# jeong0982/gkr

Hardware: AMD Instinct MI355X
Metric: BN254-Fr sumcheck field-ops/sec @ 2^20 vars (higher is better)
Workload: dtype u32x8

## Files before the change

### gkr_amd/_native.py

```python

import ctypes
import os

_HERE = os.path.dirname(os.path.abspath(__file__))
LIB_PATH = os.environ.get("GKR_AMD_LIB") or os.path.join(_HERE, "lib", "libgkr_amd.so")

GKR_OK = 0
GKR_ERR_INVALID = 1
GKR_ERR_NON_CANONICAL = 2
GKR_ERR_NO_DEVICE = 3
GKR_ERR_HIP = 4
GKR_ERR_NOMEM = 5
GKR_ERR_DEGENERATE = 6
GKR_ERR_UNSUPPORTED = 7

GKR_VERIFY_OK, GKR_VERIFY_SHAPE, GKR_VERIFY_NON_CANONICAL = 0, 1, 2
GKR_VERIFY_ROUND_SUM, GKR_VERIFY_CHALLENGE, GKR_VERIFY_EVALUATION = 4, 5, 10

GKR_TRANSCRIPT_DEVICE = 0
GKR_TRANSCRIPT_HOST = 1

SYMBOLS = [
    "gkr_strerror", "gkr_version", "gkr_ctx_create", "gkr_ctx_create_multi", "gkr_ctx_device_count", "gkr_ctx_destroy", "gkr_last_error",
    "gkr_ctx_set_transcript", "gkr_ctx_set_host_threads", "gkr_ctx_set_option", "gkr_ctx_get_option", "gkr_option_count", "gkr_option_name", "gkr_option_doc", "gkr_option_env", "gkr_host_help_while", "gkr_host_accounting", "gkr_host_accounting_read", "gkr_prove_many", "gkr_ctx_device_name", "gkr_ctx_profile", "gkr_ctx_profile_get", "gkr_ctx_profile_samples",
    "gkr_ctx_profile_reset", "gkr_mimc7_multi_hash", "gkr_mimc7_hash", "gkr_mimc7_constant",
    "gkr_selftest_mul", "gkr_selftest_wide_sum", "gkr_selftest_fold", "gkr_selftest_dot", "gkr_selftest_hash8", "gkr_selftest_host_pass", "gkr_selftest_host_prod_pass", "gkr_selftest_host_tail", "gkr_selftest_pass_schedule", "gkr_selftest_line_restriction", "gkr_selftest_seg_item", "gkr_devtest_field", "gkr_devtest_lazy", "gkr_devtest_reduce", "gkr_devtest_lanes", "gkr_sumcheck_mle", "gkr_sumcheck_mle_batch_device",
    "gkr_mle_eval_batch_device", "gkr_sumcheck_mle_verify_batch_device", "gkr_sumcheck_mle_verify",
    "gkr_sumcheck_layer", "gkr_sumcheck_layer_sharded", "gkr_sumcheck_layer_device", "gkr_resident_layer_create", "gkr_resident_layer_sumcheck", "gkr_resident_layer_sumcheck_wdev", "gkr_resident_layer_free", "gkr_exchange_limbs", "gkr_resident_layer_sumcheck_dev", "gkr_exchange_limbs_mle", "gkr_sumcheck_mle_sharded_dev", "gkr_exchange_rccl_unique_id", "gkr_exchange_rccl_create", "gkr_exchange_rccl_dev",
    "gkr_exchange_rccl_calls", "gkr_exchange_rccl_destroy", "gkr_exchange_rccl_error", "gkr_fr_widen", "gkr_fr_narrow", "gkr_predicate_tables", "gkr_layer_eval", "gkr_proof_sizes", "gkr_prove", "gkr_prove_batch",
    "gkr_layer_from_wires", "gkr_values_from_terms", "gkr_terms_from_coeffs", "gkr_prove_wires", "gkr_verify",
    "gkr_verify_prepare", "gkr_verify_prepared", "gkr_verify_circuit_free", "gkr_verify_device", "gkr_mimc7_multi_hash_device",
    "gkr_circom_meta", "gkr_circom_input_json", "gkr_circom_verifier_source", "gkr_circom_inject",
    "gkr_r1cs_parse", "gkr_r1cs_build", "gkr_r1cs_info", "gkr_r1cs_export", "gkr_r1cs_serialize", "gkr_r1cs_free",
    "gkr_wtns_parse", "gkr_wtns_serialize", "gkr_r1cs_compile", "gkr_layered_count", "gkr_layered_circuit",
    "gkr_layered_input_layer", "gkr_layered_input_values", "gkr_layered_free",
    "gkr_device_alloc", "gkr_device_free", "gkr_device_upload", "gkr_device_download",
    "gkr_device_fill_table", "gkr_device_fill_shard", "gkr_device_synchronize", "gkr_ubench_ceilings", "gkr_ubench_host_hash",
    "gkr_layer_session_open", "gkr_layer_session_open_tables", "gkr_layer_session_dep", "gkr_layer_session_rounds",
    "gkr_layer_session_sums", "gkr_layer_session_bind", "gkr_layer_session_tail", "gkr_layer_session_close",
    "gkr_mle_session_open", "gkr_mle_session_sums", "gkr_mle_session_bind", "gkr_mle_session_value",
    "gkr_mle_session_close", "gkr_device_tables_differ",
]


class CircuitDesc(ctypes.Structure):
    _fields_ = [
        ("depth", ctypes.c_uint32),
        ("k", ctypes.POINTER(ctypes.c_uint32)),
        ("gate_type", ctypes.POINTER(ctypes.c_void_p)),
        ("left", ctypes.POINTER(ctypes.c_void_p)),
        ("right", ctypes.POINTER(ctypes.c_void_p)),
    ]


class ProofBuf(ctypes.Structure):
    _fields_ = [(n, ctypes.c_void_p) for n in
                ("sumcheck_coeffs", "sumcheck_len", "sumcheck_r", "q", "q_len", "z", "r", "d_coeffs", "input_coeffs")]


class ProveItem(ctypes.Structure):
    _fields_ = [("circuit", ctypes.c_void_p), ("input_values", ctypes.c_void_p), ("batch", ctypes.c_int),
                ("require_zero_output", ctypes.c_int), ("outs", ctypes.c_void_p), ("status", ctypes.c_int)]


ALLREDUCE_DEV_FN = ctypes.CFUNCTYPE(ctypes.c_int, ctypes.c_void_p, ctypes.c_size_t, ctypes.c_void_p)


class ExchangeDev(ctypes.Structure):
    _fields_ = [("fn", ALLREDUCE_DEV_FN), ("user", ctypes.c_void_p), ("d_limbs", ctypes.c_void_p), ("capacity", ctypes.c_size_t)]


class R1csInfo(ctypes.Structure):
    _fields_ = [("n_wires", ctypes.c_uint32), ("n_pub_out", ctypes.c_uint32), ("n_pub_in", ctypes.c_uint32),
                ("n_prv_in", ctypes.c_uint32), ("n_labels", ctypes.c_uint64), ("n_constraints", ctypes.c_size_t),
                ("n_terms", ctypes.c_size_t)]


class ProofSizes(ctypes.Structure):
    _fields_ = [(n, ctypes.c_size_t) for n in ("rounds", "q_slots", "z_values", "d_coeffs", "input_coeffs")]


_lib = None


def lib():
    global _lib
    if _lib is None:
        if not os.path.exists(LIB_PATH):
            raise ImportError(
                "gkr_amd: %s is missing -- build it with `make -C gkr_amd/csrc` "
                "(or __graft_entry__.build()); there is no fallback path" % LIB_PATH)
        L = ctypes.CDLL(LIB_PATH)
        L.gkr_strerror.restype = ctypes.c_char_p
        L.gkr_version.restype = ctypes.c_char_p
        L.gkr_last_error.restype = ctypes.c_char_p
        L.gkr_last_error.argtypes = [ctypes.c_void_p]
        L.gkr_resident_layer_free.restype = None
        L.gkr_resident_layer_free.argtypes = [ctypes.c_void_p, ctypes.c_void_p]
        L.gkr_exchange_limbs.restype = ctypes.c_size_t
        L.gkr_exchange_limbs.argtypes = [ctypes.c_int]
        L.gkr_host_help_while.restype = ctypes.c_long
        L.gkr_host_help_while.argtypes = [ctypes.c_void_p]
        L.gkr_host_accounting.restype = ctypes.c_int
        L.gkr_host_accounting.argtypes = [ctypes.c_int]
        L.gkr_host_accounting_read.restype = ctypes.c_int
        L.gkr_host_accounting_read.argtypes = [ctypes.POINTER(ctypes.c_double), ctypes.c_size_t]
        L.gkr_ctx_destroy.restype = None
        L.gkr_ctx_destroy.argtypes = [ctypes.c_void_p]
        for fn in (L.gkr_layer_session_close, L.gkr_mle_session_close, L.gkr_verify_circuit_free):
            fn.restype = None
            fn.argtypes = [ctypes.c_void_p, ctypes.c_void_p]
        for fn in (L.gkr_r1cs_free, L.gkr_layered_free):
            fn.restype = None
            fn.argtypes = [ctypes.c_void_p]
        _lib = L
    return _lib
```

### gkr_amd/csrc/capi_internal.h

```cpp
#pragma once
#include <hip/hip_runtime.h>
#include <sched.h>
#include <stdio.h>
#include <stdlib.h>
#include <string.h>

#include <algorithm>
#include <chrono>
#include <condition_variable>
#include <map>
#include <memory>
#include <mutex>
#include <string>
#include <thread>
#include <vector>

#include "../../include/gkr_amd.h"
#include "fr64.h"
#include "host_cpus.h"
#include "hostpool.h"
#include "kernels.h"
#include "options.h"
#include "gate_seg.h"
#include "keccak.h"
// ... 426 lines not shown
    std::atomic<uint64_t> pieces{0}, piece_ns{0}, piece_pass_ns{0}, lanes[17] = {};
    std::atomic<bool> on{false};
};
inline HostAccountTotals& host_account_totals() {
    static HostAccountTotals t;
    return t;
}
inline bool accounting_on() { return host_account_totals().on.load(std::memory_order_relaxed); }
inline void account_piece(int transcripts, double pass_us, double total_us) {
    HostAccountTotals& t = host_account_totals();
    t.pieces.fetch_add(1, std::memory_order_relaxed);
    t.piece_ns.fetch_add((uint64_t)(total_us * 1e3), std::memory_order_relaxed);
    t.piece_pass_ns.fetch_add((uint64_t)(pass_us * 1e3), std::memory_order_relaxed);
    t.lanes[transcripts < 1 ? 1 : (transcripts > 16 ? 16 : transcripts)].fetch_add(1, std::memory_order_relaxed);
}
inline double now_us_dbg() { return std::chrono::duration<double, std::micro>(std::chrono::steady_clock::now().time_since_epoch()).count(); }

inline bool help_enabled() {
    static const bool on = !gkr::process_switch("GKR_NO_HELP");
    return on;
}
static void run_pieces(gkr::SpinPool* pool, const std::function<bool()>* work, bool several, int priority = 0) {
    auto run = [&] {
        if (pool)
            pool->run_now(work);
        else
            while ((*work)()) {
            }
    };
    const bool dbg = gkr::debug_timing() || accounting_on();
    const double t0 = dbg ? now_us_dbg() : 0.0;
    if (several && help_enabled()) {
        gkr::HelpBoard::Posted posted(work, priority);
        run();
    } else {
        run();
    }
    if (dbg) t_account.own_pieces_us += now_us_dbg() - t0;
}

template <typename Rec>
inline int wait_records(gkr_ctx* ctx, const volatile Rec* recs, int count, uint32_t ticket) {
    const auto t0 = std::chrono::steady_clock::now();
    const bool help = help_enabled();
    auto last_progress = t0;
    for (int b = 0; b < count; ++b) {
        uint32_t spins = 0, helped = 0;
        while (__atomic_load_n(&recs[b].seq, __ATOMIC_ACQUIRE) != ticket) {
            const bool dbg = gkr::debug_timing() || accounting_on();
            const double th0 = dbg ? now_us_dbg() : 0.0;
            const bool did_help = help && gkr::HelpBoard::instance().help();
            if (!did_help) GKR_CPU_RELAX();
            if (dbg) (did_help ? t_account.helped_us : t_account.spin_us) += now_us_dbg() - th0;
            if (did_help ? (++helped & 0x3F) == 0 : (++spins & 0xFFFF) == 0) {
                hipError_t q = hipStreamQuery(ctx->stream);
                if (q != hipSuccess && q != hipErrorNotReady) return ctx->hip_fail(q, "stream failed while waiting for a round");
                if (std::chrono::steady_clock::now() - last_progress > std::chrono::seconds(30)) {
                    if (q == hipSuccess && __atomic_load_n(&recs[b].seq, __ATOMIC_ACQUIRE) == ticket) break;
                    return ctx->fail(GKR_ERR_HIP, "timed out waiting for the device to publish a round");
                }
            }
        }
        if (spins | helped) last_progress = std::chrono::steady_clock::now();
    }
    return GKR_OK;
}

constexpr int kMaxGroups = 32;
constexpr int kMleShardTailLog2 = 6;

#define WS(ctx, slot, type, count, ptr) \
    HIP_TRY(ctx, (ctx)->workspace(slot, (size_t)(count) * sizeof(type), reinterpret_cast<void**>(&(ptr))))

inline int mle_pass_rounds(int m, int n, int jmax) {
    int j = m < jmax ? m : jmax;
    if (((size_t)1 << m) > gkr::kSmallPassEntries && m != n && j > m - 6) j = m - 6;
    if (jmax > 3 && (m - j == 10 || m - j == 11) && m - 12 >= 1) j = m - 12;
    return j < 1 ? 1 : j;
}

inline void write_round_output(gkr_fr* out_coeffs, uint32_t* out_len, gkr_fr* out_r, size_t row, const void* c0, const void* c1, uint32_t ln,
                               const void* r) {
    memset(&out_coeffs[row * 2], 0, 32);
    if (ln == 2) memcpy(&out_coeffs[row * 2], c1, 32);
    memcpy(&out_coeffs[row * 2 + 1], c0, 32);
    out_len[row] = ln;
    memcpy(&out_r[row], r, 32);
}
struct GroupHandoff {
    int b0 = 0, nb = 0;
    int state = 0;
    uint32_t ticket = 0;
    std::atomic<uint64_t> claim{0};
    std::atomic<int> done{0};
    template <typename Rec>
    bool records_landed(const Rec* rec) const {
        for (int i = nb - 1; i >= 0; --i)
            if (__atomic_load_n(&rec[b0 + i].seq, __ATOMIC_ACQUIRE) != ticket) return false;
        return true;
    }
    void open(uint32_t generation) {
        done.store(0, std::memory_order_relaxed);
        claim.store((uint64_t)generation << 32, std::memory_order_release);
        state = 1;
    }
    uint32_t open_generation() const {
        const uint64_t c = claim.load(std::memory_order_acquire);
        return (uint32_t)c < (uint32_t)nb ? (uint32_t)(c >> 32) : 0u;
    }
    bool try_claim(uint32_t chunk, uint32_t* first, uint32_t* take, uint32_t* generation = nullptr) {
        uint64_t c = claim.load(std::memory_order_acquire);
        while ((c >> 32) != 0 && (uint32_t)c < (uint32_t)nb) {
            const uint32_t left = (uint32_t)nb - (uint32_t)c, t = left < chunk ? left : chunk;
            if (!claim.compare_exchange_weak(c, c + t, std::memory_order_acq_rel)) continue;
            *first = (uint32_t)c;
            *take = t;
            if (generation) *generation = (uint32_t)(c >> 32);
            return true;
        }
        return false;
    }
    void finish(uint32_t count) { done.fetch_add((int)count, std::memory_order_release); }
    bool all_done() {
        if (done.load(std::memory_order_acquire) != nb) return false;
        claim.store(0, std::memory_order_release);
        return true;
    }
};
struct HandoffWatch {
    gkr_ctx* ctx;
    hipStream_t s;
    std::string unit;
    std::chrono::steady_clock::time_point t0 = std::chrono::steady_clock::now();
    uint32_t idle = 0;
    int progressed() {
        idle = 0;
        t0 = std::chrono::steady_clock::now();
        if (hipError_t le = hipGetLastError(); le != hipSuccess) return ctx->hip_fail(le, ("launch of a sumcheck " + unit).c_str());
        return GKR_OK;
    }
    int idled() {
        GKR_CPU_RELAX();
        if ((++idle & 0xFFFF) != 0) return GKR_OK;
        const hipError_t q = hipStreamQuery(s);
        if (q != hipSuccess && q != hipErrorNotReady) return ctx->hip_fail(q, ("stream failed during a sumcheck " + unit).c_str());
        if (std::chrono::steady_clock::now() - t0 > std::chrono::seconds(60))
            return ctx->fail(GKR_ERR_HIP, "timed out waiting for the device to publish a " + unit);
        return GKR_OK;
    }
};

void host_pass_scalar(const uint64_t* sums, size_t sums_row_words, int count, int J, const uint32_t* final_len, uint64_t (*c0)[16][4],
                      uint64_t (*c1)[16][4], uint64_t (*r)[16][4], uint32_t (*len)[16], uint64_t* weights, size_t w_row_words);
struct MleTailArgs {
    int n_total = 0, round_offset = 0;
    const uint32_t* dep_last = nullptr;
};
int run_mle_batch_passes(gkr_ctx* ctx, const Fr* d_tables, int n, int batch, gkr_fr* out_coeffs, uint32_t* out_len, gkr_fr* out_r,
                         const MleTailArgs* tail = nullptr);
int run_mle_batch(gkr_ctx* ctx, const Fr* d_tables, int n, int batch, gkr_fr* out_coeffs, uint32_t* out_len, gkr_fr* out_r);
void host_tail_pass(gkr::h64::F* tables, size_t stride, uint32_t m, uint32_t jp, const gkr::h64::F* weights, uint32_t J, gkr::h64::F* rec);
void host_tail_pass_scalar(gkr::h64::F* tables, size_t stride, uint32_t m, uint32_t jp, const gkr::h64::F* weights, uint32_t J, gkr::h64::F* rec);
void host_prod_pass_scalar(const uint64_t* recs, size_t rec_row_words, int count, int J, const uint32_t (*vec_len)[16], uint64_t (*c2)[16][4],
                           uint64_t (*lin)[16][4], uint64_t (*c0)[16][4], uint64_t (*r)[16][4], uint64_t* weights, size_t w_row_words);
struct LayerShardArgs {
    uint64_t gate_base = 0, gate_count = 0;
    gkr_allreduce_fn allreduce = nullptr;
    void* user = nullptr;
    const gkr_exchange_dev* dev = nullptr;
};
struct LayerGroup {
    const gkr::GateSet* d_sets = nullptr;
    gkr::GatePlanCounts plan_counts{};
};
int run_layer_batch(gkr_ctx* ctx, int batch, int k_i, int k, const uint8_t* d_gt, const uint32_t* d_l, const uint32_t* d_r, const gkr_fr* z,
                    const Fr* d_W, gkr_fr* const* out_coeffs, uint32_t* const* out_len, gkr_fr* const* out_r, const LayerShardArgs* shard = nullptr,
                    GateLists* cached = nullptr, const LayerGroup* group = nullptr);
int build_cached_gate_lists(gkr_ctx* ctx, int k_i, int k, const uint8_t* d_gt, const uint32_t* d_l, const uint32_t* d_r, GateLists* cached);
int check_layer_args(gkr_ctx* ctx, int k_i, int k_next, const uint8_t* gt, const uint32_t* l, const uint32_t* r, const gkr_fr* z);
int upload_gates(gkr_ctx* ctx, size_t gates, const uint8_t* gt, const uint32_t* l, const uint32_t* r, DevBuf<uint8_t>& dgt, DevBuf<uint32_t>& dl,
                 DevBuf<uint32_t>& dr);
int run_layer_dense(gkr_ctx* ctx, int batch, int k_i, int k, const uint8_t* d_gt, const uint32_t* d_l, const uint32_t* d_r, const gkr_fr* z,
                    const Fr* d_W, gkr_fr* const* out_coeffs, uint32_t* const* out_len, gkr_fr* const* out_r);
bool verify_device_hash_wanted(size_t rows);
int verify_hash_rows_device(gkr_ctx* ctx, const uint32_t* d_rows, const uint32_t* d_len, size_t n, gkr::VerifyHashSlot* d_slots, hipStream_t s);
void mobius_msb(std::vector<gkr::h64::F>& c, int k);
void line_restriction(const std::vector<gkr::h64::F>& vals, const std::vector<gkr::h64::F>& coeffs, int k, const gkr_fr* b, const gkr_fr* c,
                      gkr_fr* out, uint32_t* out_len);
int check_circuit(gkr_ctx* ctx, const gkr_circuit_desc* c);

}
```

### gkr_amd/csrc/capi_mle_passes.hip

```cpp
#include "capi_internal.h"

namespace gkr_host {

void host_pass_scalar(const uint64_t* sums, size_t sums_row_words, int count, int J, const uint32_t* final_len,
                             uint64_t (*c0)[16][4], uint64_t (*c1)[16][4], uint64_t (*r)[16][4], uint32_t (*len)[16],
                             uint64_t* weights, size_t w_row_words) {
    using gkr::h64::F;
    const F* cts = host_mimc_constants64();
    const F one_m = gkr::h64::to_mont(F{{1, 0, 0, 0}});
    for (int k = 0; k < count; ++k) {
        F S[gkr::kMleMaxSub], rm[gkr::kMlePassMaxRounds];
        memcpy(S, sums + (size_t)k * sums_row_words, sizeof(F) << J);
        for (int t = 0; t < J; ++t) {
            const int half = 1 << (J - t - 1);
            F lo = S[0], hi = S[half];
            for (int b = 1; b < half; ++b) {
                lo = gkr::h64::add(lo, S[b]);
                hi = gkr::h64::add(hi, S[half + b]);
            }
            const F d = gkr::h64::sub(hi, lo);
            const uint32_t ln = (final_len && t == J - 1) ? final_len[k] : (gkr::h64::is_zero(d) ? 1u : 2u);
            const F vec[2] = {d, lo};
            const F rc = host_multi_hash(vec + (2 - ln), (int)ln, cts);
            memcpy(c0[t][k], &lo, 32);
            memcpy(c1[t][k], &d, 32);
            memcpy(r[t][k], &rc, 32);
            len[t][k] = ln;
            rm[t] = gkr::h64::to_mont(rc);
            for (int b = 0; b < half; ++b) S[b] = gkr::h64::add(S[b], gkr::h64::mont_mul(gkr::h64::sub(S[half + b], S[b]), rm[t]));
        }
        if (!weights) continue;
        F* w = reinterpret_cast<F*>(weights + (size_t)k * w_row_words);
        F tmp[gkr::kMleMaxSub];
        tmp[0] = one_m;
        int cur = 1;
        for (int t = 0; t < J; ++t) {
            const F nr = gkr::h64::sub(one_m, rm[t]);
            for (int b = cur; b-- > 0;) {
                tmp[2 * b + 1] = gkr::h64::mont_mul(tmp[b], rm[t]);
                tmp[2 * b] = gkr::h64::mont_mul(tmp[b], nr);
            }
            cur <<= 1;
        }
        memcpy(w, tmp, sizeof(F) << J);
    }
}

struct MlePassTables {
    const Fr* input = nullptr;
    size_t in_stride = 0;
    Fr* work = nullptr;
    size_t work_len = 0;
    gkr::MleSubPartial* partials = nullptr;
    unsigned char* plans = nullptr;
    Fr* h_w = nullptr;
    gkr::MleHostRecSub* h_rec = nullptr;
    gkr::MleHostRecSub* rec = nullptr;
    uint32_t* arrivals = nullptr;
    Fr* h_tail = nullptr;
};
static int mle_pass_tables(gkr_ctx* ctx, const std::string& prefix, const Fr* input, size_t len, size_t work_len, int batch, MlePassTables& T) {
    T.input = input;
    T.in_stride = len;
    T.work_len = work_len;
    WS(ctx, (prefix + ".work").c_str(), Fr, (size_t)batch * (work_len ? work_len : 1), T.work);
    WS(ctx, (prefix + ".partials").c_str(), gkr::MleSubPartial, (size_t)batch * gkr::kMaxBlocksPerTable, T.partials);
    WS(ctx, (prefix + ".plans").c_str(), unsigned char, (size_t)batch * gkr::mle_fold_plan_bytes(), T.plans);
    HIP_TRY(ctx, ctx->pinned_host((prefix + ".rec").c_str(), sizeof(gkr::MleHostRecSub) * batch, reinterpret_cast<void**>(&T.h_rec)));
    HIP_TRY(ctx, ctx->pinned_host((prefix + ".w").c_str(), sizeof(Fr) * gkr::kMleMaxSub * batch, reinterpret_cast<void**>(&T.h_w)));
    T.rec = T.h_rec;
    return GKR_OK;
}

constexpr double kFusedPublishBytes = 64.0 * 1024 * 1024;
constexpr uint32_t kFusedPublishBlocks = 256;
constexpr size_t kArrivalCounters = 4096;
static int mle_arrival_counters(gkr_ctx* ctx, size_t len, MlePassTables& T) {
    if (gkr::opt(gkr::OPT_no_fused_reduce) != 0 || (double)len * 32.0 > kFusedPublishBytes) return GKR_OK;
    WS(ctx, "mlep.arrivals", uint32_t, kArrivalCounters, T.arrivals);
    if (ctx->mle_arrivals_zeroed != T.arrivals) {
        HIP_TRY(ctx, hipMemsetAsync(T.arrivals, 0, sizeof(uint32_t) * kArrivalCounters, ctx->stream));
        ctx->mle_arrivals_zeroed = T.arrivals;
    }
    return GKR_OK;
}
static bool fused_publish(const MlePassTables& T, int b0, int nb, uint32_t nblk, double bytes_read, uint32_t ticket, int jout, gkr::MlePublish& pub) {
    if (!T.arrivals || (size_t)(b0 + nb) > kArrivalCounters || bytes_read > kFusedPublishBytes || (uint64_t)nblk * nb > kFusedPublishBlocks || nblk > 128u)
        return false;
    pub.rec = T.rec + b0;
    pub.arrivals = T.arrivals + b0;
    pub.ticket = ticket;
    pub.jout = (uint32_t)jout;
    return true;
}

constexpr uint32_t kMleTailLog2 = 7;
struct MlePassPolicy {
    const char* row = nullptr;
    int plan_event = -1;
    Fr* export_tail = nullptr;
};
static void queue_sub_reduce(gkr_ctx* ctx, const MlePassTables& T, int b0, int nb, uint32_t nblk, int jout, uint32_t ticket, hipStream_t st) {
    Timed t(ctx, "mle_sub_reduce", 0.0, st, true);
    gkr::launch_mle_sub_reduce(T.partials + (size_t)b0 * gkr::kMaxBlocksPerTable, nblk, (uint32_t)jout, nb, T.rec + b0, ticket, st);
}
static void queue_pass0(gkr_ctx* ctx, const MlePassTables& T, int b0, int nb, int jout, uint32_t ticket, hipStream_t st, const MlePassPolicy& P) {
    const size_t len = T.in_stride;
    const Fr* src = T.input + (size_t)b0 * len;
    const double bytes = (double)nb * len * 32.0;
    if (len <= gkr::kSmallPassEntries) {
        Timed t(ctx, "mle_pass_small", bytes, st, true);
        gkr::launch_mle_multifold_small(0, src, len, nullptr, 0, (uint32_t)len, (uint32_t)jout, nb, T.h_w + (size_t)b0 * gkr::kMleMaxSub, T.rec + b0, ticket, st);
        return;
    }
    const uint32_t nblk = gkr::mle_pass_blocks((uint32_t)len, (uint32_t)jout, nb);
    gkr::MlePublish pub;
    const bool fused = fused_publish(T, b0, nb, nblk, bytes, ticket, jout, pub);
    {
        Timed t(ctx, P.row, bytes, st, fused);
        gkr::launch_mle_sub_sums(src, len, (uint32_t)len, nb, nblk, T.partials + (size_t)b0 * gkr::kMaxBlocksPerTable, st, fused ? &pub : nullptr);
    }
    if (!fused) queue_sub_reduce(ctx, T, b0, nb, nblk, jout, ticket, st);
}
static void queue_fold(gkr_ctx* ctx, const MlePassTables& T, int b0, int nb, bool from_input, int m_src, int jin, int jout, uint32_t ticket,
                       hipStream_t st, const MlePassPolicy& P) {
    const size_t src_len = (size_t)1 << m_src, S = src_len >> jin;
    const Fr* src = from_input ? T.input + (size_t)b0 * T.in_stride : T.work + (size_t)b0 * T.work_len;
    const size_t src_stride = from_input ? T.in_stride : T.work_len;
    Fr* dst = T.work + (size_t)b0 * T.work_len;
    const Fr* w = T.h_w + (size_t)b0 * gkr::kMleMaxSub;
    const double bytes = (double)nb * ((double)src_len + (double)S) * 32.0;
    if (S <= gkr::kSmallPassEntries) {
        Timed t(ctx, "mle_pass_small", bytes, st, true);
        gkr::launch_mle_multifold_small(jin, src, src_stride, dst, T.work_len, (uint32_t)S, (uint32_t)jout, nb, w, T.rec + b0, ticket, st, P.export_tail,
                                        1u << kMleTailLog2);
        return;
    }
    const uint32_t nblk = gkr::mle_multifold_blocks((uint32_t)S, (uint32_t)jout, nb);
    unsigned char* plan = T.plans + (size_t)b0 * gkr::mle_fold_plan_bytes();
    if (gkr::mle_multifold_uses_mfma((uint32_t)S, nblk)) {
        if (P.plan_event < 0) {
            gkr::launch_mle_fold_plan(jin, w, plan, nb, st);
        } else {
            {
                Timed t(ctx, "mle_fold_plan", 0.0, ctx->aux, true);
                gkr::launch_mle_fold_plan(jin, w, plan, nb, ctx->aux);
            }
            (void)hipEventRecord(ctx->aux_events[P.plan_event], ctx->aux);
            (void)hipStreamWaitEvent(st, ctx->aux_events[P.plan_event], 0);
        }
    }
    gkr::MlePublish pub;
    const bool fused = fused_publish(T, b0, nb, nblk, (double)nb * (double)src_len * 32.0, ticket, jout, pub);
    {
        Timed t(ctx, P.row, bytes, st, fused);
        gkr::launch_mle_multifold(jin, src, src_stride, dst, T.work_len, (uint32_t)S, nb, nblk, w, plan, T.partials + (size_t)b0 * gkr::kMaxBlocksPerTable, st,
                                  fused ? &pub : nullptr);
    }
    if (!fused) queue_sub_reduce(ctx, T, b0, nb, nblk, jout, ticket, st);
}

struct MleSchedule {
    int jmax = 0, j_first = 0;
    int n_dev = 0;
    int groups = 0, depth = 0;
    int bound[kMaxGroups + 1];
    uint32_t chunk[kMaxGroups];
    bool tail_on = false;
};
static MleSchedule mle_schedule(int n, int batch, int hash_threads, bool is_tail, const gkr::Options& o) {
    MleSchedule sc;
    const double len = (double)((size_t)1 << n);
    const int jcap = o.v[gkr::OPT_no_mfma_fold] ? 3 : gkr::kMlePassMaxRounds;
    const int jwant = o.v[gkr::OPT_rounds_per_pass] > 0 ? (int)o.v[gkr::OPT_rounds_per_pass] : jcap;
    sc.jmax = jwant > jcap ? jcap : jwant;
    sc.j_first = mle_pass_rounds(n, n, sc.jmax);
    const long long dp = o.v[gkr::OPT_device_hash_percent];
    const int dev_percent = dp < 0 ? 0 : (dp > 90 ? 90 : (int)dp);
    if (dev_percent > 0 && !is_tail && batch >= 64 && sc.j_first >= 1) {
        sc.n_dev = (int)((long long)batch * dev_percent / 100) & ~7;
        if (batch - sc.n_dev < 16) sc.n_dev = (batch - 16) & ~7;
        if (sc.n_dev < 8) sc.n_dev = 0;
    }
    const int host_batch = batch - sc.n_dev;
    const double batch_bytes = (double)host_batch * len * 32.0;
    int want_groups = (int)(batch_bytes / (4.0 * 1024 * 1024 * 1024));
    want_groups = want_groups < 4 ? 4 : (want_groups > 8 ? (batch_bytes > 96.0 * 1024 * 1024 * 1024 ? 16 : 8) : want_groups);
    const bool small_tables = n <= 17 && host_batch >= 256;
    if (small_tables) want_groups = 16;
    if (hash_threads <= 3 && host_batch >= 256 && want_groups < 16) want_groups = 16;
    int group_size = host_batch >= 128 ? (host_batch + want_groups - 1) / want_groups : (host_batch >= 16 ? (host_batch + 1) / 2 : host_batch);
    if (sc.n_dev && hash_threads <= 3 && host_batch >= 256) group_size = 64;
    if (o.v[gkr::OPT_group_size] > 0) group_size = (int)o.v[gkr::OPT_group_size];
    sc.groups = (host_batch + group_size - 1) / group_size;
    if (sc.groups > kMaxGroups) sc.groups = kMaxGroups;
    const long long forced = o.v[gkr::OPT_hash_chunk];
    for (int g = 0; g <= sc.groups; ++g) sc.bound[g] = sc.n_dev + (int)((long long)host_batch * g / sc.groups);
    for (int g = 0; g < sc.groups; ++g) {
        const int nb = sc.bound[g + 1] - sc.bound[g], per = (nb + hash_threads - 1) / hash_threads;
        sc.chunk[g] = forced == 8 || forced == 16 ? (uint32_t)forced : (nb >= 32 * hash_threads ? 16u : (uint32_t)(per <= 8 ? 8 : (per <= 16 ? per : 16)));
    }
    sc.depth = o.v[gkr::OPT_pass_queue_depth] > 0 ? (int)o.v[gkr::OPT_pass_queue_depth] : (small_tables ? 4 : 2);
    sc.tail_on = o.v[gkr::OPT_host_tail_log2] >= 0 && sc.n_dev == 0 && batch <= (o.v[gkr::OPT_host_tail_max_batch] > 0 ? o.v[gkr::OPT_host_tail_max_batch] : 8);
    return sc;
}

namespace {
struct PassGroup : GroupHandoff {
    int m = 0;
    int j = 0;
    int round0 = 0;
    int pass = 0, index = 0;
    hipStream_t chain = nullptr;
    bool on_host = false;
};
struct MlePassClock {
    const bool on = gkr::debug_timing();
    const std::chrono::steady_clock::time_point t0 = std::chrono::steady_clock::now();
    double a = 0, b = 0, c = 0, d = 0, e = 0;
    std::atomic<uint64_t> busy_ns{0};
    double us() const { return std::chrono::duration<double, std::micro>(std::chrono::steady_clock::now() - t0).count(); }
    void report(int threads) const {
        if (!on) return;
        fprintf(stderr,
                "[gkr timing] setup %.0f us, first launches %.0f, loop %.0f, end_session %.0f, sync %.0f, drain %.0f; hashing %.0f us "
                "over %d threads = %.0f%% of the loop\n",
                a, b - a, c - b, d - c, e - d, us() - e, busy_ns.load() * 1e-3, threads, busy_ns.load() * 1e-3 / ((c - b) * threads) * 100.0);
    }
};

struct MlePassRun {
    gkr_ctx* ctx;
    const int n, batch;
    const MleTailArgs* tail;
    gkr_fr* out_coeffs;
    uint32_t* out_len;
    gkr_fr* out_r;
    MleSchedule sc;
    MlePassTables T;
    hipStream_t s = nullptr, late = nullptr, chain = nullptr;
    std::vector<PassGroup> grp;
    std::vector<uint32_t> dep_last;
    int next_first = 0;
    gkr_fr *stage_c = nullptr, *stage_r = nullptr;
    uint32_t* stage_len = nullptr;
    MlePassClock clock;

    int rounds_for(int m) const { return mle_pass_rounds(m, n, sc.jmax); }
    void advance(PassGroup& G, int jin) {
        G.m -= jin;
        G.round0 += jin;
        G.j = rounds_for(G.m);
        G.ticket = ++ctx->ticket;
    }
    void launch_first(PassGroup& G) {
        G.ticket = ++ctx->ticket;
        MlePassPolicy P;
        P.row = G.chain ? "mle_sub_sums_dev" : "mle_sub_sums";
        queue_pass0(ctx, T, G.b0, G.nb, G.j, G.ticket, G.chain ? G.chain : s, P);
    }
    void launch_next_first() {
        if (next_first < sc.groups) launch_first(grp[next_first++]);
    }
    void launch_fold(PassGroup& G, int jin) {
        const int m_src = G.m;
        const bool from_input = m_src == n;
        hipStream_t st = G.chain ? G.chain : ((!from_input && m_src <= 16) ? late : s);
        advance(G, jin);
        MlePassPolicy P;
        P.row = G.chain ? "mle_multifold_dev" : (st == s ? "mle_multifold" : "mle_multifold_late");
        if (!gkr::opt(gkr::OPT_plan_main) && st == s && sc.groups != 1) P.plan_event = G.index;
        G.on_host = sc.tail_on && !G.chain && G.m <= (int)kMleTailLog2 && G.m - G.j > 0;
        if (G.on_host) P.export_tail = T.h_tail + ((size_t)G.b0 << kMleTailLog2);
        queue_fold(ctx, T, G.b0, G.nb, from_input, m_src, jin, G.j, G.ticket, st, P);
    }
    void host_fold(PassGroup& G, int jin) {
        using gkr::h64::F;
        advance(G, jin);
        const size_t S = (size_t)1 << G.m, nsub = (size_t)1 << G.j, sub = S >> G.j;
        for (int b = G.b0; b < G.b0 + G.nb; ++b) {
            F* tab = reinterpret_cast<F*>(T.h_tail + ((size_t)b << kMleTailLog2));
            const F* w = reinterpret_cast<const F*>(T.h_w + (size_t)b * gkr::kMleMaxSub);
            for (size_t i = 0; i < S; ++i) {
                gkr::h64::Wide acc = gkr::h64::wide_zero();
                for (size_t t = 0; t < ((size_t)1 << jin); ++t) gkr::h64::wide_mac(acc, tab[t * S + i], w[t]);
                tab[i] = gkr::h64::wide_reduce(acc);
            }
            F* sums = reinterpret_cast<F*>(T.h_rec[b].sums);
            for (size_t a = 0; a < nsub; ++a) {
                F v = tab[a * sub];
                for (size_t i = 1; i < sub; ++i) v = gkr::h64::add(v, tab[a * sub + i]);
                sums[a] = v;
            }
            __atomic_store_n(&T.h_rec[b].seq, G.ticket, __ATOMIC_RELEASE);
        }
    }
    void process_chunk(const PassGroup& G, int b_first, int count) {
        static const bool scalar_book = gkr::process_switch("GKR_HOST_PASS_SCALAR");
        const int J = G.j, n_out = tail ? tail->n_total : n, r_off = tail ? tail->round_offset : 0;
        uint64_t c0[gkr::kMlePassMaxRounds][16][4], c1[gkr::kMlePassMaxRounds][16][4], r[gkr::kMlePassMaxRounds][16][4];
        uint32_t ln[gkr::kMlePassMaxRounds][16], final_len[16];
        const bool final_pass = G.round0 + J == n;
        for (int i = 0; i < count; ++i) {
            if (G.round0 == 0) dep_last[b_first + i] = tail && tail->dep_last ? tail->dep_last[b_first + i] : T.h_rec[b_first + i].dep;
            final_len[i] = dep_last[b_first + i] ? 2u : 1u;
        }
        static_assert(sizeof(gkr::MleHostRecSub) % 8 == 0, "hand-off records are addressed in 64-bit words");
        const uint64_t* sums = reinterpret_cast<const uint64_t*>(T.h_rec[b_first].sums);
        uint64_t* weights = G.m - J > 0 ? reinterpret_cast<uint64_t*>(T.h_w + (size_t)b_first * gkr::kMleMaxSub) : nullptr;
        (host_ifma_ready() && count >= 3 && !scalar_book ? gkr::gkr_ifma_pass : host_pass_scalar)(
            sums, sizeof(gkr::MleHostRecSub) / 8, count, J, final_pass ? final_len : nullptr, c0, c1, r, ln, weights, 4 * gkr::kMleMaxSub);
        for (int i = 0; i < count; ++i)
            for (int t = 0; t < J; ++t)
                write_round_output(out_coeffs, out_len, out_r, (size_t)(b_first + i) * n_out + r_off + G.round0 + t, c0[t][i], c1[t][i], ln[t][i], r[t][i]);
    }
    bool try_work() {
        for (;;) {
            int best = -1;
            uint32_t best_gen = 0;
            for (int g = 0; g < sc.groups; ++g)
                if (const uint32_t gen = grp[g].open_generation(); gen && (best < 0 || gen < best_gen)) best = g, best_gen = gen;
            if (best < 0) return false;
            PassGroup& G = grp[best];
            uint32_t first, take;
            if (!G.try_claim(sc.chunk[best], &first, &take)) continue;
            const double t_in = clock.on ? clock.us() : 0.0;
            process_chunk(G, G.b0 + (int)first, (int)take);
            G.finish(take);
            if (clock.on) clock.busy_ns.fetch_add((uint64_t)((clock.us() - t_in) * 1e3), std::memory_order_relaxed);
            return true;
        }
    }
    int queue_device_chain() {
        const int n_dev = sc.n_dev;
        HIP_TRY(ctx, ctx->chain_stream(&chain));
        uint32_t* dep_dev = nullptr;
        WS(ctx, "mlep.dev_dep", uint32_t, (size_t)n_dev, dep_dev);
        HIP_TRY(ctx, ctx->pinned_host("mlep.stage_c", sizeof(gkr_fr) * 2 * (size_t)n_dev * n, reinterpret_cast<void**>(&stage_c)));
        HIP_TRY(ctx, ctx->pinned_host("mlep.stage_r", sizeof(gkr_fr) * (size_t)n_dev * n, reinterpret_cast<void**>(&stage_r)));
        HIP_TRY(ctx, ctx->pinned_host("mlep.stage_len", sizeof(uint32_t) * (size_t)n_dev * n, reinterpret_cast<void**>(&stage_len)));
        PassGroup dev;
        dev.nb = n_dev;
        dev.m = n;
        dev.j = sc.j_first;
        dev.index = sc.groups;
        dev.chain = chain;
        launch_first(dev);
        for (bool first = true;; first = false) {
            const int J = dev.j;
            {
                Timed t(ctx, "mle_pass_hash_dev", 0.0, chain);
                gkr::launch_mle_pass_hash_lanes(T.rec, (uint32_t)n_dev, (uint32_t)J, (uint32_t)dev.round0, (uint32_t)n, dev.round0 + J == n, first, ctx->d_cts,
                                                dep_dev, dev.m - J > 0 ? T.h_w : nullptr, reinterpret_cast<Fr*>(stage_c), stage_len,
                                                reinterpret_cast<Fr*>(stage_r), chain);
            }
            if (dev.m - J <= 0) return GKR_OK;
            launch_fold(dev, J);
        }
    }
    bool step(PassGroup& G, int& active) {
        if (G.state == 0 && G.records_landed(T.h_rec)) {
            G.open((uint32_t)++G.pass);
            return true;
        }
        if (G.state != 1 || !G.all_done()) return false;
        if (G.m - G.j > 0) {
            const bool first_fold = G.m == n;
            if (G.on_host)
                host_fold(G, G.j);
            else
                launch_fold(G, G.j);
            G.state = 0;
            if (first_fold) launch_next_first();
        } else {
            G.state = 2;
            --active;
            launch_next_first();
        }
        return true;
    }
    int loop() {
        int rc = GKR_OK, active = sc.groups;
        HandoffWatch watch{ctx, s, "pass"};
        while (active > 0 && rc == GKR_OK) {
            bool progress = false;
            for (int g = 0; g < next_first; ++g) progress |= step(grp[g], active);
            if (progress)
                rc = watch.progressed();
            else if (!try_work())
                rc = watch.idled();
        }
        return rc;
    }
};
}

int run_mle_batch_passes(gkr_ctx* ctx, const Fr* d_tables, int n, int batch, gkr_fr* out_coeffs, uint32_t* out_len, gkr_fr* out_r,
                         const MleTailArgs* tail) {
    MlePassRun R{ctx, n, batch, tail, out_coeffs, out_len, out_r};
    const size_t len = (size_t)1 << n;
    hipStream_t s = R.s = R.late = ctx->stream;
    gkr::SpinPool* pool = ctx->host_pool();
    const gkr::Options* o = gkr::current_options();
    const MleSchedule& sc = R.sc = mle_schedule(n, batch, pool->workers() + 1, tail != nullptr, o ? *o : gkr::default_options());
    if (int rc = mle_pass_tables(ctx, "mlep", d_tables, len, len >> sc.j_first, batch, R.T)) return rc;
    if (int rc = mle_arrival_counters(ctx, len, R.T)) return rc;
    HIP_TRY(ctx, ctx->aux_stream(sc.groups));
    if (sc.tail_on) HIP_TRY(ctx, ctx->pinned_host("mlep.tail", sizeof(Fr) * ((size_t)batch << kMleTailLog2), reinterpret_cast<void**>(&R.T.h_tail)));
    if (!gkr::opt(gkr::OPT_no_late_stream) && sc.groups > 1) HIP_TRY(ctx, ctx->late_stream(&R.late));
    R.dep_last = std::vector<uint32_t>(batch, 0);
    R.grp = std::vector<PassGroup>(sc.groups);
    for (int g = 0; g < sc.groups; ++g) {
        PassGroup& G = R.grp[g];
        G.index = g;
        G.b0 = sc.bound[g];
        G.nb = sc.bound[g + 1] - sc.bound[g];
        G.m = n;
        G.j = sc.j_first;
    }
    const std::function<bool()> try_work = [&R] { return R.try_work(); };
    R.clock.a = R.clock.us();
    gkr::SpinPool::Session session(pool, &try_work);
    R.launch_next_first();
    if (sc.n_dev)
        if (int rc = R.queue_device_chain()) return rc;
    while (R.next_first < sc.groups && R.next_first < sc.depth) R.launch_next_first();
    R.clock.b = R.clock.us();
    const int rc = R.loop();
    R.clock.c = R.clock.us();
    session.close();
    if (rc) {
        (void)hipStreamSynchronize(s);
        if (R.late != s) (void)hipStreamSynchronize(R.late);
        if (R.chain) (void)hipStreamSynchronize(R.chain);
        ctx->mle_arrivals_zeroed = nullptr;
        return rc;
    }
    R.clock.d = R.clock.us();
    HIP_TRY(ctx, hipGetLastError());
    HIP_TRY(ctx, hipStreamSynchronize(s));
    if (R.late != s) HIP_TRY(ctx, hipStreamSynchronize(R.late));
    if (sc.n_dev) {
        HIP_TRY(ctx, hipStreamSynchronize(R.chain));
        memcpy(out_coeffs, R.stage_c, sizeof(gkr_fr) * 2 * (size_t)sc.n_dev * n);
        memcpy(out_r, R.stage_r, sizeof(gkr_fr) * (size_t)sc.n_dev * n);
        memcpy(out_len, R.stage_len, sizeof(uint32_t) * (size_t)sc.n_dev * n);
    }
    R.clock.e = R.clock.us();
    if (ctx->pending.size() > 8192) ctx->drain_events();
    R.clock.report(pool->workers() + 1);
    return GKR_OK;
}

namespace {
struct MleShardRun {
    gkr_ctx* ctx;
    const gkr_exchange_dev* exchange;
    const int n, batch;
    gkr_fr* out_coeffs;
    uint32_t* out_len;
    gkr_fr* out_r;
    MlePassTables T;
    uint32_t* h_fail = nullptr;
    std::vector<uint32_t> dep_last;
    gkr::SpinPool* pool = nullptr;
    int rc = GKR_OK;
    uint32_t exchanges = 0;

    long long* limbs() const { return reinterpret_cast<long long*>(exchange->d_limbs); }
    void hook_failed(int arc) {
        if (arc && !rc) rc = ctx->fail(GKR_ERR_INVALID, "the device sum-over-ranks hook failed (status " + std::to_string(arc) + ")");
    }
    bool some_rank_failed() const { return __atomic_load_n(h_fail, __ATOMIC_ACQUIRE) != 0; }
    void exchange_sums(int J, uint32_t ticket) {
        hipStream_t s = ctx->stream;
        Timed t(ctx, "exchange", 0.0);
        gkr::launch_mle_xwiden(T.rec, (uint32_t)J, (uint32_t)batch, rc ? 1u : 0u, limbs(), s);
        const int arc = exchange->fn(exchange->user, (size_t)batch * (((size_t)1 << J) + 2) * 8, static_cast<void*>(s));
        gkr::launch_mle_xnarrow(limbs(), (uint32_t)J, (uint32_t)batch, T.h_rec, ticket, h_fail, s);
        ++exchanges;
        hook_failed(arc);
    }
    void gather_tail(const Fr* rest, size_t stride, int m, int lp, int shard, Fr* d_tail) {
        hipStream_t s = ctx->stream;
        Timed t(ctx, "exchange", 0.0);
        gkr::launch_mle_gather_widen(rest, stride, (uint32_t)m, (uint32_t)lp, (uint32_t)shard, rc ? 1u : 0u, (uint32_t)batch, limbs(), s);
        const int arc = exchange->fn(exchange->user, ((size_t)batch << (m + lp)) * 8 + 8, static_cast<void*>(s));
        gkr::launch_mle_gather_narrow(limbs(), (uint32_t)(m + lp), (uint32_t)batch, d_tail, h_fail, s);
        ++exchanges;
        hook_failed(arc);
    }
    void rounds_chunk(int first, int J, int round0) {
        const int count = batch - first < 16 ? batch - first : 16;
        uint64_t c0[gkr::kMlePassMaxRounds][16][4], c1[gkr::kMlePassMaxRounds][16][4], r[gkr::kMlePassMaxRounds][16][4];
        uint32_t ln[gkr::kMlePassMaxRounds][16];
        (host_ifma_ready() && count >= 3 ? gkr::gkr_ifma_pass : host_pass_scalar)(
            reinterpret_cast<const uint64_t*>(T.h_rec[first].sums), sizeof(gkr::MleHostRecSub) / 8, count, J, nullptr, c0, c1, r, ln,
            reinterpret_cast<uint64_t*>(T.h_w + (size_t)first * gkr::kMleMaxSub), 4 * gkr::kMleMaxSub);
        for (int i = 0; i < count; ++i) {
            if (round0 == 0) dep_last[first + i] = T.h_rec[first + i].dep;
            for (int t = 0; t < J; ++t)
                write_round_output(out_coeffs, out_len, out_r, (size_t)(first + i) * n + round0 + t, c0[t][i], c1[t][i], ln[t][i], r[t][i]);
        }
    }
    void host_rounds(int J, int round0) {
        std::atomic<int> next{0};
        const std::function<bool()> work_fn = [&]() -> bool {
            const int first = next.fetch_add(16, std::memory_order_relaxed);
            if (first < batch) rounds_chunk(first, J, round0);
            return first < batch;
        };
        gkr::SpinPool::Session session(pool, nullptr);
        run_pieces(pool, &work_fn, batch > 16);
    }
    void pass(bool pass0, bool from_input, int m_src, int jin, int J, int round0) {
        const uint32_t ticket = ++ctx->ticket;
        if (!rc) {
            MlePassPolicy P;
            P.row = pass0 ? "mle_sub_sums" : "mle_multifold";
            if (pass0)
                queue_pass0(ctx, T, 0, batch, J, ticket, ctx->stream, P);
            else
                queue_fold(ctx, T, 0, batch, from_input, m_src, jin, J, ticket, ctx->stream, P);
            if (hipError_t le = hipGetLastError(); le != hipSuccess) rc = ctx->hip_fail(le, "launch of a sumcheck pass");
        }
        exchange_sums(J, ticket);
        if (!rc) rc = wait_records(ctx, T.h_rec, batch, ticket);
        if (!rc && some_rank_failed()) rc = ctx->fail(GKR_ERR_HIP, "another rank failed during the sumcheck");
        if (!rc) host_rounds(J, round0);
    }
};
}

}

extern "C" {

size_t gkr_exchange_limbs_mle(int n, int log2_shards, int batch) {
    if (n < 2 || log2_shards < 0 || log2_shards > 16 || n - log2_shards < 1 || n - log2_shards > GKR_MAX_MLE_N || batch < 1) return 0;
    const int nl = n - log2_shards, t = nl < kMleShardTailLog2 ? nl : kMleShardTailLog2;
    const size_t per_pass = (size_t)batch * (gkr::kMleMaxSub + 2) * 8, gather = ((size_t)batch << (t + log2_shards)) * 8 + 8;
    return per_pass > gather ? per_pass : gather;
}

int gkr_sumcheck_mle_sharded_dev(gkr_ctx* ctx, const void* d_shards, int n, int log2_shards, int shard, int batch,
                                 const gkr_exchange_dev* exchange, gkr_fr* out_coeffs, uint32_t* out_len, gkr_fr* out_r,
                                 uint32_t* out_exchanges) {
    if (!ctx) return GKR_ERR_INVALID;
    if (!d_shards || !exchange || !exchange->fn || !exchange->d_limbs || !out_coeffs || !out_len || !out_r || batch < 1 || batch > 65535)
        return ctx->fail(GKR_ERR_INVALID, "null pointer or batch out of range [1, 65535]");
    const int lp = log2_shards, nl = n - lp;
    if (lp < 0 || lp > 16 || shard < 0 || shard >= (1 << lp)) return ctx->fail(GKR_ERR_INVALID, "shard must be in [0, 2^log2_shards), log2_shards in [0, 16]");
    if (n < 2 || nl < 1 || nl > GKR_MAX_MLE_N) return ctx->fail(GKR_ERR_INVALID, "n >= 2 and 1 <= n - log2_shards <= GKR_MAX_MLE_N needed");
    if (ctx->transcript != GKR_TRANSCRIPT_HOST) return ctx->fail(GKR_ERR_INVALID, "a sumcheck split over ranks needs the host transcript");
    if (exchange->capacity < gkr_exchange_limbs_mle(n, lp, batch)) return ctx->fail(GKR_ERR_INVALID, "the exchange buffer is smaller than gkr_exchange_limbs_mle(n, log2_shards, batch) int64");
    GKR_ENTER(ctx);
    hipStream_t s = ctx->stream;
    const size_t len = (size_t)1 << nl;
    const int t_stop = nl < kMleShardTailLog2 ? nl : kMleShardTailLog2;
    const int jmax = gkr::opt(gkr::OPT_no_mfma_fold) ? 3 : gkr::kMlePassMaxRounds;
// ... 50 lines not shown
```

### gkr_amd/csrc/gkr_capi.hip

```cpp
#include "capi_internal.h"


extern "C" {

const char* gkr_strerror(int status) {
    switch (status) {
        case GKR_OK: return "ok";
        case GKR_ERR_INVALID: return "invalid argument";
        case GKR_ERR_NON_CANONICAL: return "field element is not canonical (>= r)";
        case GKR_ERR_NO_DEVICE: return "no gfx950 device available";
        case GKR_ERR_HIP: return "HIP runtime error";
        case GKR_ERR_NOMEM: return "out of memory";
        case GKR_ERR_DEGENERATE: return "degenerate sumcheck (v == 0)";
        case GKR_ERR_UNSUPPORTED: return "R1CS shape the reference's compiler does not support";
        default: return "unknown status";
    }
}

const char* gkr_version(void) { return "gkr_amd 0.1 (gfx950)"; }

int gkr_ctx_create(int device_id, gkr_ctx** out) {
    if (!out) return GKR_ERR_INVALID;
    *out = nullptr;
    int count = 0;
// ... 196 lines not shown
int gkr_ctx_device_name(const gkr_ctx* ctx, char* buf, size_t len) {
    if (!ctx || !buf || !len) return GKR_ERR_INVALID;
    snprintf(buf, len, "%s", ctx->name);
    return GKR_OK;
}

int gkr_ctx_profile(gkr_ctx* ctx, int enable) {
    if (!ctx) return GKR_ERR_INVALID;
    ctx->profile = enable < 0 ? 0 : (enable > 2 ? 2 : enable);
    return GKR_OK;
}

int gkr_ctx_profile_get(gkr_ctx* ctx, const char* kernel, uint64_t* launches, double* total_ms, double* bytes) {
    if (!ctx || !kernel) return GKR_ERR_INVALID;
    ctx->drain_events();
    auto it = ctx->prof.find(kernel);
    ProfileRow r = it == ctx->prof.end() ? ProfileRow() : it->second;
    if (launches) *launches = r.launches;
    if (total_ms) *total_ms = r.total_ms;
    if (bytes) *bytes = r.bytes;
    return GKR_OK;
}

int gkr_ctx_profile_samples(gkr_ctx* ctx, const char* kernel, double* ms, double* bytes, size_t capacity, size_t* count) {
    if (!ctx || !kernel || !count) return GKR_ERR_INVALID;
    ctx->drain_events();
    auto it = ctx->prof.find(kernel);
    const size_t n = it == ctx->prof.end() ? 0 : it->second.samples.size();
    *count = n;
    for (size_t i = 0; i < n && i < capacity; ++i) {
        if (ms) ms[i] = it->second.samples[i].first;
        if (bytes) bytes[i] = it->second.samples[i].second;
    }
    return GKR_OK;
}

int gkr_ctx_profile_reset(gkr_ctx* ctx) {
    if (!ctx) return GKR_ERR_INVALID;
    ctx->drain_events();
    ctx->prof.clear();
    return GKR_OK;
}


int gkr_mimc7_multi_hash(const gkr_fr* arr, size_t n, const gkr_fr* key, gkr_fr* out) {
    if ((!arr && n) || !out) return GKR_ERR_INVALID;
    if (!all_canonical(arr, n) || (key && !all_canonical(key, 1))) return GKR_ERR_NON_CANONICAL;
    const Fr* cts = host_mimc_constants();
    Fr r = key ? gkr::to_mont(to_dev(*key)) : gkr::fr_zero();
    for (size_t i = 0; i < n; ++i) {
        Fr a = gkr::to_mont(to_dev(arr[i]));
        Fr h = gkr::mimc7_hash_mont(a, r, cts);
        r = gkr::fr_add(gkr::fr_add(r, a), h);
    }
    *out = to_abi(gkr::from_mont(r));
    return GKR_OK;
}

int gkr_mimc7_hash(const gkr_fr* x, const gkr_fr* k, gkr_fr* out) {
    if (!x || !k || !out) return GKR_ERR_INVALID;
    if (!all_canonical(x, 1) || !all_canonical(k, 1)) return GKR_ERR_NON_CANONICAL;
    Fr h = gkr::mimc7_hash_mont(gkr::to_mont(to_dev(*x)), gkr::to_mont(to_dev(*k)), host_mimc_constants());
    *out = to_abi(gkr::from_mont(h));
    return GKR_OK;
}

int gkr_mimc7_constant(int i, gkr_fr* out) {
    if (i < 0 || i >= gkr::kMimcRounds || !out) return GKR_ERR_INVALID;
    *out = to_abi(gkr::from_mont(host_mimc_constants()[i]));
    return GKR_OK;
}

int gkr_selftest_mul(const gkr_fr* a, const gkr_fr* b, gkr_fr* out) {
    if (!a || !b || !out) return GKR_ERR_INVALID;
    if (!all_canonical(a, 1) || !all_canonical(b, 1)) return GKR_ERR_NON_CANONICAL;
    *out = to_abi(gkr::fr_mul(to_dev(*a), to_dev(*b)));
    return GKR_OK;
}

int gkr_selftest_fold(const gkr_fr* lo, const gkr_fr* hi, const gkr_fr* r, gkr_fr* out) {
    if (!lo || !hi || !r || !out) return GKR_ERR_INVALID;
    if (!all_canonical(lo, 1) || !all_canonical(hi, 1) || !all_canonical(r, 1)) return GKR_ERR_NON_CANONICAL;
    const gkr::FixedMul T = gkr::make_fixed_mul(to_dev(*r));
    gkr::FixedMul T64;
    gkr::h64::F r64;
    memcpy(&r64, r, 32);
    gkr::h64::make_fixed_mul(r64, T64.w);
    if (memcmp(&T, &T64, sizeof T) != 0) return GKR_ERR_INVALID;
    const Fr single = gkr::fr_fold_fixed(to_dev(*lo), to_dev(*hi), T);
    Fr y0, y1;
    gkr::fr_fold_fixed2(to_dev(*lo), to_dev(*hi), to_dev(*hi), to_dev(*lo), T, y0, y1);
    if (!gkr::fr_eq(y0, single) || !gkr::fr_eq(y1, gkr::fr_fold_fixed(to_dev(*hi), to_dev(*lo), T))) return GKR_ERR_INVALID;
    *out = to_abi(single);
    return GKR_OK;
}

int gkr_selftest_pass_schedule(int n, int mfma, uint32_t* rounds, size_t capacity, size_t* passes) {
    if (n < 1 || n > 40 || !passes) return GKR_ERR_INVALID;
    const int jmax = mfma ? gkr::kMlePassMaxRounds : 3;
    size_t count = 0;
    for (int m = n; m > 0;) {
        const int j = mle_pass_rounds(m, n, jmax);
        if (rounds && count < capacity) rounds[count] = (uint32_t)j;
        ++count;
        m -= j;
    }
    *passes = count;
    return (rounds && count > capacity) ? GKR_ERR_NOMEM : GKR_OK;
}

int gkr_selftest_host_pass(const gkr_fr* sums, int count, int J, const uint32_t* final_len, gkr_fr* c0, gkr_fr* c1, uint32_t* len,
                           gkr_fr* r, gkr_fr* w, int* used_ifma) {
    using gkr::h64::F;
    if (!sums || !c0 || !c1 || !len || !r || !w || count < 1 || count > kHashChunkMax || J < 1 || J > gkr::kMlePassMaxRounds)
        return GKR_ERR_INVALID;
    static_assert(gkr::kMleMaxSub == 32 && kHashChunkMax == 16, "shapes of the self-test's arrays");
    if (!all_canonical(sums, (size_t)count * 32)) return GKR_ERR_NON_CANONICAL;
    if (final_len)
        for (int k = 0; k < count; ++k)
            if (final_len[k] != 1 && final_len[k] != 2) return GKR_ERR_INVALID;
    struct Out {
        uint64_t c0[gkr::kMlePassMaxRounds][16][4], c1[gkr::kMlePassMaxRounds][16][4], r[gkr::kMlePassMaxRounds][16][4];
        uint32_t len[gkr::kMlePassMaxRounds][16];
        std::vector<F> w;
    } a, b;
    a.w.assign((size_t)count * 32, F{{0, 0, 0, 0}});
    host_pass_scalar(reinterpret_cast<const uint64_t*>(sums), 4 * 32, count, J, final_len, a.c0, a.c1, a.r, a.len, &a.w[0].l[0], 4 * 32);
    const bool ifma = host_ifma_ready();
    if (used_ifma) *used_ifma = ifma ? 1 : 0;
    if (ifma) {
        b.w.assign((size_t)count * 32, F{{0, 0, 0, 0}});
        gkr::gkr_ifma_pass(reinterpret_cast<const uint64_t*>(sums), 4 * 32, count, J, final_len, b.c0, b.c1, b.r, b.len, &b.w[0].l[0], 4 * 32);
        for (int t = 0; t < J; ++t)
            for (int k = 0; k < count; ++k)
                if (memcmp(a.c0[t][k], b.c0[t][k], 32) || memcmp(a.c1[t][k], b.c1[t][k], 32) || memcmp(a.r[t][k], b.r[t][k], 32) ||
                    a.len[t][k] != b.len[t][k])
                    return GKR_ERR_INVALID;
        if (memcmp(a.w.data(), b.w.data(), sizeof(F) * a.w.size()) != 0) return GKR_ERR_INVALID;
    }
    for (int t = 0; t < J; ++t)
        for (int k = 0; k < count; ++k) {
            memcpy(&c0[(size_t)t * count + k], a.c0[t][k], 32);
            memcpy(&c1[(size_t)t * count + k], a.c1[t][k], 32);
            memcpy(&r[(size_t)t * count + k], a.r[t][k], 32);
            len[(size_t)t * count + k] = a.len[t][k];
        }
    for (size_t i = 0; i < a.w.size(); ++i) {
        const F wc = gkr::h64::from_mont(a.w[i]);
        memcpy(&w[i], &wc, 32);
    }
    return GKR_OK;
}

int gkr_selftest_host_prod_pass(const gkr_fr* recs, int count, int J, const uint32_t* vec_len, gkr_fr* c2, gkr_fr* lin, gkr_fr* c0,
                                gkr_fr* r, gkr_fr* w, int* used_ifma) {
    using gkr::h64::F;
    if (!recs || !vec_len || !c2 || !lin || !c0 || !r || !w || count < 1 || count > kHashChunkMax || J < 1 || J > gkr::kProdMaxJ)
        return GKR_ERR_INVALID;
    if (!all_canonical(recs, (size_t)count * gkr::kProdRecValues)) return GKR_ERR_NON_CANONICAL;
    uint32_t vl[gkr::kProdMaxJ][16] = {};
    for (int t = 0; t < J; ++t)
        for (int k = 0; k < count; ++k) {
            vl[t][k] = vec_len[(size_t)t * count + k];
            if (vl[t][k] != 2 && vl[t][k] != 3) return GKR_ERR_INVALID;
        }
    struct Out {
        uint64_t c2[gkr::kProdMaxJ][16][4], lin[gkr::kProdMaxJ][16][4], c0[gkr::kProdMaxJ][16][4], r[gkr::kProdMaxJ][16][4];
        F w[16][8];
    } a, b;
    memset(&a, 0, sizeof a);
    memset(&b, 0, sizeof b);
    host_prod_pass_scalar(reinterpret_cast<const uint64_t*>(recs), 4 * gkr::kProdRecValues, count, J, vl, a.c2, a.lin, a.c0, a.r, &a.w[0][0].l[0], 32);
    const bool ifma = host_ifma_ready();
    if (used_ifma) *used_ifma = ifma ? 1 : 0;
    if (ifma) {
        gkr::gkr_ifma_prod_pass(reinterpret_cast<const uint64_t*>(recs), 4 * gkr::kProdRecValues, count, J, vl, b.c2, b.lin, b.c0, b.r, &b.w[0][0].l[0], 32);
        for (int t = 0; t < J; ++t)
            for (int k = 0; k < count; ++k)
                if (memcmp(a.c2[t][k], b.c2[t][k], 32) || memcmp(a.lin[t][k], b.lin[t][k], 32) || memcmp(a.c0[t][k], b.c0[t][k], 32) ||
                    memcmp(a.r[t][k], b.r[t][k], 32))
                    return GKR_ERR_INVALID;
        for (int k = 0; k < count; ++k)
            if (memcmp(a.w[k], b.w[k], sizeof(F) << J) != 0) return GKR_ERR_INVALID;
    }
    for (int t = 0; t < J; ++t)
        for (int k = 0; k < count; ++k) {
            memcpy(&c2[(size_t)t * count + k], a.c2[t][k], 32);
            memcpy(&lin[(size_t)t * count + k], a.lin[t][k], 32);
            memcpy(&c0[(size_t)t * count + k], a.c0[t][k], 32);
            memcpy(&r[(size_t)t * count + k], a.r[t][k], 32);
        }
    for (int k = 0; k < count; ++k)
        for (int bb = 0; bb < 8; ++bb) {
            const F wc = bb < (1 << J) ? gkr::h64::from_mont(a.w[k][bb]) : F{{0, 0, 0, 0}};
            memcpy(&w[(size_t)k * 8 + bb], &wc, 32);
        }
    return GKR_OK;
}

int gkr_selftest_host_tail(const gkr_fr* tables, int m, int jp, const gkr_fr* weights, int J, gkr_fr* rec, int* used_ifma) {
    using gkr::h64::F;
    if (!tables || !rec || m < 0 || m > 12 || jp < 0 || jp > gkr::kProdMaxJ || jp > m || J < 1 || J > gkr::kProdMaxJ || J > m - jp || (jp && !weights))
        return GKR_ERR_INVALID;
    const size_t len = (size_t)1 << m;
    if (!all_canonical(tables, 3 * len) || (jp && !all_canonical(weights, (size_t)1 << jp))) return GKR_ERR_NON_CANONICAL;
    std::vector<F> t(3 * len);
    memcpy(t.data(), tables, sizeof(F) * 3 * len);
    for (size_t i = 0; i < len; ++i) t[i] = gkr::h64::to_mont(t[i]);
    F w[8] = {};
    for (int b = 0; jp && b < (1 << jp); ++b) {
        memcpy(&w[b], &weights[b], sizeof(F));
        w[b] = gkr::h64::to_mont(w[b]);
    }
    F out[gkr::kProdRecValues] = {};
    const bool ifma = host_ifma_ready();
    if (used_ifma) *used_ifma = ifma ? 1 : 0;
    if (ifma) {
        std::vector<F> t2(t);
        F out2[gkr::kProdRecValues] = {};
        gkr::gkr_ifma_tail_pass(&t2[0].l[0], len, (uint32_t)m, (uint32_t)jp, &w[0].l[0], (uint32_t)J, &out2[0].l[0]);
        host_tail_pass_scalar(t.data(), len, (uint32_t)m, (uint32_t)jp, w, (uint32_t)J, out);
        const size_t folded = (size_t)1 << (m - jp);
        for (int tb = 0; tb < 3; ++tb)
            if (memcmp(&t[(size_t)tb * len], &t2[(size_t)tb * len], folded * sizeof(F)) != 0) return GKR_ERR_INVALID;
        const int n = 1 << J;
        for (int a = 0; a < n; ++a) {
            if (memcmp(&out[a * 8], &out2[a * 8], sizeof(F) * n) != 0) return GKR_ERR_INVALID;
            if (memcmp(&out[64 + a], &out2[64 + a], sizeof(F)) != 0) return GKR_ERR_INVALID;
        }
    } else {
        host_tail_pass_scalar(t.data(), len, (uint32_t)m, (uint32_t)jp, w, (uint32_t)J, out);
    }
    memcpy(rec, out, sizeof out);
    return GKR_OK;
}

int gkr_selftest_hash8(const gkr_fr* vecs, const uint32_t* len, gkr_fr* out, int* used_ifma) {
    if (!vecs || !len || !out) return GKR_ERR_INVALID;
    if (!all_canonical(vecs, 24)) return GKR_ERR_NON_CANONICAL;
    for (int k = 0; k < 8; ++k)
        if (len[k] > 3) return GKR_ERR_INVALID;
    const bool ifma = host_ifma_ready();
    if (used_ifma) *used_ifma = ifma ? 1 : 0;
    if (ifma) {
        uint64_t v[8][3][4], o[8][4];
        memcpy(v, vecs, sizeof v);
        gkr::gkr_ifma_multi_hash8(v, len, 3, o);
        memcpy(out, o, sizeof o);
        uint64_t v16[16][3][4], o16[16][4];
        uint32_t len16[16];
        for (int k = 0; k < 8; ++k) {
            memcpy(v16[k], v[k], sizeof v[k]);
            memcpy(v16[15 - k], v[k], sizeof v[k]);
            len16[k] = len16[15 - k] = len[k];
        }
        gkr::gkr_ifma_multi_hash16(v16, len16, 3, o16);
        for (int k = 0; k < 8; ++k)
            if (memcmp(o16[k], o[k], 32) != 0 || memcmp(o16[15 - k], o[k], 32) != 0) return GKR_ERR_INVALID;
    } else {
        const gkr::h64::F* cts = host_mimc_constants64();
        for (int k = 0; k < 8; ++k) {
            gkr::h64::F v[3];
            memcpy(v, vecs + 3 * k, 96);
            const gkr::h64::F r = host_multi_hash(v + (3 - len[k]), (int)len[k], cts);
            memcpy(&out[k], &r, 32);
        }
    }
    return GKR_OK;
}

int gkr_ubench_host_hash(int len, double* us_per_hash_lanes16, double* us_per_hash_scalar) {
    if (len < 1 || len > 3 || !us_per_hash_lanes16 || !us_per_hash_scalar) return GKR_ERR_INVALID;
    uint64_t v16[16][3][4], o16[16][4];
    uint32_t len16[16];
    for (int k = 0; k < 16; ++k) {
        len16[k] = (uint32_t)len;
        for (int e = 0; e < 3; ++e)
            for (int j = 0; j < 4; ++j) v16[k][e][j] = j == 3 ? 0x0123456789abcdefull >> 4 : 0x9E3779B97F4A7C15ull * (uint64_t)(k * 12 + e * 4 + j + 1);
    }
    auto now = [] { return std::chrono::steady_clock::now(); };
    *us_per_hash_lanes16 = 0.0;
    if (host_ifma_ready()) {
        double best = 1e30;
        for (int rep = 0; rep < 5; ++rep) {
            const auto t0 = now();
            for (int i = 0; i < 64; ++i) {
                gkr::gkr_ifma_multi_hash16(v16, len16, 3, o16);
                memcpy(v16[i & 15][2], o16[(i + 1) & 15], 32);
            }
            const double us = std::chrono::duration<double, std::micro>(now() - t0).count() / (64.0 * 16.0);
            if (us < best) best = us;
        }
        *us_per_hash_lanes16 = best;
    }
    const gkr::h64::F* cts = host_mimc_constants64();
    gkr::h64::F v[3];
    memcpy(v, v16[0], 96);
    double best = 1e30;
    for (int rep = 0; rep < 5; ++rep) {
        const auto t0 = now();
        for (int i = 0; i < 32; ++i) v[2] = host_multi_hash(v + (3 - len), len, cts);
        const double us = std::chrono::duration<double, std::micro>(now() - t0).count() / 32.0;
        if (us < best) best = us;
    }
    *us_per_hash_scalar = best;
    return GKR_OK;
// ... 217 lines not shown
```

### gkr_amd/csrc/kernels.h

```cpp
#pragma once
#include <hip/hip_runtime.h>
#include <stddef.h>
#include <stdint.h>

#include "fr32.h"

namespace gkr {

constexpr uint32_t kMaxBlocksPerTable = 2048;
constexpr uint32_t kMaxLayerBlocks = 2048;

struct MlePartial {
    Acc<9> lo, hi;
    uint32_t dep, pad;
};

struct LayerBatch {
    uint32_t batch;
    uint32_t pstride;
    size_t tstride, wstride;
};
inline LayerBatch single_layer() { return LayerBatch{1u, 0u, 0, 0}; }

struct LayerPartial {
    Acc<9> c0, g1, c2;
    uint32_t pad;
};

struct MleHostRec {
    Fr c0, c1;
    uint32_t dep, seq;
    uint32_t pad[14];
};
struct LayerHostRec {
    Fr c0, g1, c2;
    uint32_t seq;
    uint32_t pad[7];
};
static_assert(sizeof(MleHostRec) == 128 && sizeof(LayerHostRec) == 128, "hand-off records are one 128-byte line");

constexpr int kProdMaxJ = 3;
constexpr int kProdRecValues = 72;
struct ProdPassRec {
    Fr v[kProdRecValues];
    uint32_t seq;
    uint32_t pad[7];
};
static_assert(sizeof(ProdPassRec) == kProdRecValues * 32 + 32, "product-pass record layout");
constexpr uint32_t kProdTile = 8, kProdTileWide = 32;
inline uint32_t prod_pass_tile(uint32_t S) { return S >= 1024u ? kProdTileWide : kProdTile; }
inline uint32_t prod_pass_blocks(uint32_t S) { return S <= kProdTile ? 1u : S / prod_pass_tile(S); }
inline uint32_t prod_pass_max_blocks(uint32_t k) {
    uint32_t m = 1;
    for (uint32_t l = 0; l < k; ++l) m = prod_pass_blocks(1u << l) > m ? prod_pass_blocks(1u << l) : m;
    return m;
}
inline size_t prod_pass_scratch_values(uint32_t k) { return ((size_t)prod_pass_max_blocks(k) + 64u) * kProdRecValues; }
constexpr uint32_t kProdFuseBlocks = 64;
constexpr uint32_t kProdFoldMinM = 17;
size_t prod_fold_plan_bytes();
void launch_prod_pass(Fr* W, Fr* X, Fr* Y, uint32_t m_in, uint32_t jp, const Fr* weights, uint32_t J, Fr* partials, uint32_t wstride,
                      ProdPassRec* rec, uint32_t ticket, uint32_t batch, hipStream_t s, uint32_t* arrivals = nullptr, void* fold_plans = nullptr,
                      Fr* tail = nullptr, uint32_t tail_stride = 0);
void launch_prod_c_setup(const Fr* Wb, uint32_t jp, const Fr* weights, const Fr* A, const Fr* M, Fr* X, Fr* Y, uint32_t k, uint32_t wstride,
                         uint32_t batch, hipStream_t s);

constexpr uint32_t kSmallFoldQuarter = 2048;
void launch_mle_fold_sum_small(const Fr* src, size_t src_stride, Fr* dst, size_t dst_stride, uint32_t q, uint32_t batch,
                               const FixedMul* rtab, MleHostRec* host_rec, uint32_t ticket, hipStream_t s);
void launch_mle_round_reduce(const MlePartial* partials, uint32_t nblk, uint32_t batch, MleHostRec* host_rec,
                             uint32_t ticket, hipStream_t s);

struct MleSubPartial {
    Acc<9> sum;
    uint32_t dep, pad[2];
};
constexpr int kMlePassMaxRounds = 5;
constexpr int kMleMaxSub = 1 << kMlePassMaxRounds;
struct MleHostRecSub {
    Fr sums[kMleMaxSub];
    uint32_t dep, seq;
    uint32_t pad[14];
};
static_assert(sizeof(MleHostRecSub) == 1088, "hand-off record layout");
struct MlePublish {
    MleHostRecSub* rec = nullptr;
    uint32_t* arrivals = nullptr;
    uint32_t ticket = 0, jout = 0;
};
constexpr uint32_t kSmallPassEntries = 512;
uint32_t mle_pass_blocks(uint32_t items, uint32_t jout, uint32_t batch);
uint32_t mle_multifold_blocks(uint32_t S, uint32_t jout, uint32_t batch);
bool mle_multifold_uses_mfma(uint32_t S, uint32_t nblk);
void launch_mle_sub_sums(const Fr* tables, size_t stride, uint32_t len, uint32_t batch, uint32_t nblk, MleSubPartial* partials,
                         hipStream_t s, const MlePublish* publish = nullptr);
void launch_mle_sub_reduce(const MleSubPartial* partials, uint32_t nblk, uint32_t jout, uint32_t batch, MleHostRecSub* host_rec,
                           uint32_t ticket, hipStream_t s);
size_t mle_fold_plan_bytes();
void launch_mle_fold_plan(int jin, const Fr* weights, void* plans, uint32_t batch, hipStream_t s);
void launch_mle_multifold(int jin, const Fr* src, size_t src_stride, Fr* dst, size_t dst_stride, uint32_t S, uint32_t batch,
                          uint32_t nblk, const Fr* weights, const void* plans, MleSubPartial* partials, hipStream_t s,
                          const MlePublish* publish = nullptr);
void launch_mle_pass_hash_lanes(const MleHostRecSub* rec, uint32_t count, uint32_t J, uint32_t round0, uint32_t n_out, bool final_pass,
                                bool first_pass, const Fr* cts, uint32_t* dep_last, Fr* weights, Fr* out_coeffs, uint32_t* out_len, Fr* out_r,
                                hipStream_t s);
void launch_mle_multifold_small(int jin, const Fr* src, size_t src_stride, Fr* dst, size_t dst_stride, uint32_t S, uint32_t jout,
                                uint32_t batch, const Fr* weights, MleHostRecSub* host_rec, uint32_t ticket, hipStream_t s, Fr* tail = nullptr, uint32_t tail_stride = 0);
void launch_layer_round_reduce(const LayerPartial* partials, uint32_t nblk, LayerHostRec* host_rec, uint32_t ticket,
                               LayerBatch lb, hipStream_t s);
void launch_fold_small(Fr* W, uint32_t hw, const FixedMul* rtab, LayerBatch lb, hipStream_t s);
struct GateSpan {
    uint64_t base, count;
};
uint32_t gate_lists_lds_blocks(uint64_t gates, uint32_t k);
size_t gate_lists_lds_scratch_words(uint64_t gates, uint32_t k);
inline size_t gate_list_words(uint64_t gates) { return 2 * (size_t)gates + 1; }
struct GateSegs {
    uint32_t shift = 0;
    uint32_t runs = 0;
    uint32_t run_base = 0;
    uint32_t bound = 0;
    uint32_t half_bound = 0;
    uint32_t groups = 0;
    uint32_t nb = 0;
    uint64_t packed_half = 0;
    uint32_t* words = nullptr;
    uint2* items() const { return reinterpret_cast<uint2*>(words); }
    uint32_t* order() const { return words + 2 * (size_t)bound; }
    uint32_t* bucket_begin() const { return order() + bound; }
    uint32_t* group_len() const { return bucket_begin() + 2 * (size_t)nb + 2; }
    uint32_t* group_off() const { return group_len() + 2 * (size_t)groups; }
    uint32_t* packed() const { return group_off() + 2 * (size_t)groups + 2; }
};
uint32_t gate_seg_shift(GateSpan span, uint32_t k_i, uint32_t k);
size_t gate_segs_words(GateSpan span, uint32_t k_i, uint32_t k);
size_t gate_segs_scratch_words(GateSpan span, uint32_t k_i, uint32_t k);
size_t gate_seg_partial_elems(GateSpan span, uint32_t k_i, uint32_t k);
void launch_gate_lists(GateSpan span, uint32_t k_i, uint32_t k, const uint8_t* gate_type, const uint32_t* left, const uint32_t* right,
                       uint32_t* counts, uint32_t* offsets, uint32_t* cursor, uint32_t* block_sums, uint32_t* list, uint32_t* bad,
                       uint32_t* lds_scratch, GateSegs* segs, uint32_t* seg_scratch, hipStream_t s);
struct GateSet {
    const uint32_t* offsets;
    const uint32_t* cursor;
    const uint32_t* list;
    const uint32_t* plan;
    const uint8_t* gate_type;
    const uint32_t* left;
    const uint32_t* right;
    uint64_t pad;
};
static_assert(sizeof(GateSet) == 64, "one cache line per proof");
void launch_gate_uv(GateSpan span, uint32_t k_i, uint32_t k, const uint32_t* offsets, const uint32_t* cursor, const uint32_t* list,
                    const Fr* e_hi, const Fr* e_lo_mont, uint32_t kl, const Fr* W, Fr* U, Fr* V, LayerBatch lb, const GateSegs* segs,
                    Fr* partials, hipStream_t s, const GateSet* sets = nullptr);
struct CPhaseFuse {
    const Fr* Wb = nullptr;
    const Fr* weights = nullptr;
    Fr* X = nullptr;
    Fr* Y = nullptr;
    uint32_t jp = 0;
};
bool launch_gate_rows(GateSpan span, uint32_t k_i, uint32_t k, const uint32_t* offsets, const uint32_t* cursor, const uint32_t* list,
                      const Fr* e_hi, const Fr* e_lo_mont, uint32_t kl, const Fr* eq_mont, Fr* A_row, Fr* M_row, LayerBatch lb,
                      const GateSegs* segs, Fr* partials, hipStream_t s, const CPhaseFuse* fuse = nullptr, const GateSet* sets = nullptr);
void launch_fill_table(Fr* table, size_t count, uint64_t seed, hipStream_t s);
void launch_fill_shard(Fr* shard_table, size_t count, uint32_t lp, uint32_t shard, uint64_t seed, hipStream_t s);
void launch_exchange_widen(const Fr* a, const Fr* b, uint32_t each, const uint32_t* flag, uint32_t local_flag, long long* limbs, hipStream_t s);
void launch_exchange_narrow(const long long* limbs, Fr* a, Fr* b, uint32_t each, uint32_t* flag_out, hipStream_t s);
void launch_ubench_copy(const void* in, void* out, size_t bytes, hipStream_t s);
void launch_ubench_read(const void* in, void* out, size_t bytes, hipStream_t s);
void launch_ubench_modmul(Fr* io, uint32_t entries_pow2, uint32_t waves, int reps, hipStream_t s);

uint32_t mle_blocks_per_table(uint32_t items, uint32_t batch);
void launch_mle_sum_first(const Fr* tables, size_t stride, uint32_t h, uint32_t batch, uint32_t nblk,
                          MlePartial* partials, hipStream_t s);
void launch_mle_fold_sum(const Fr* src, size_t src_stride, Fr* dst, size_t dst_stride, uint32_t q, uint32_t batch,
                         uint32_t nblk, const FixedMul* rtab, uint32_t r_stride, MlePartial* partials, hipStream_t s);
void launch_mle_round_hash(const MlePartial* partials, uint32_t nblk, uint32_t round, uint32_t n, uint32_t batch,
                           const Fr* cts, Fr* out_coeffs, uint32_t* out_len, Fr* out_r, FixedMul* rtab,
                           uint32_t* dep_last, hipStream_t s);

void launch_layer_eval(uint32_t gates, const uint8_t* gate_type, const uint32_t* left, const uint32_t* right,
                       const Fr* prev, Fr* out, uint32_t batch, uint32_t prev_stride, hipStream_t s, const GateSet* sets = nullptr);
void launch_copy_words(const void* src, void* dst, size_t words, hipStream_t s);
void launch_copy_rows(const void* src, size_t src_stride_words, void* dst, size_t dst_stride_words, uint32_t words, uint32_t rows, hipStream_t s);
void launch_eq_table(const Fr* points, uint32_t stride, uint32_t first, uint32_t nvars, Fr* out, bool montgomery, uint32_t batch,
                     hipStream_t s, const CPhaseFuse* wu_job = nullptr, Fr* wu_out = nullptr, uint32_t wstride = 0);
void launch_layer_prologue(const Fr* points, uint32_t k_i, uint32_t kh, uint32_t kl, Fr* e_hi, Fr* e_lo, const Fr* W, Fr* Wb, Fr* Wc,
                           uint32_t k, uint32_t* dep, uint32_t* host_dep, uint32_t batch, hipStream_t s, uint32_t* wide_bits = nullptr);
enum class LinePart { all, prepare, finish };
void launch_line_restriction(const Fr* W, uint32_t k, const Fr* bc, Fr* scratch, uint32_t* deg_scratch, Fr* bcm, Fr* out, uint32_t* out_len,
                             uint32_t batch, hipStream_t s, LinePart part = LinePart::all);

constexpr uint32_t kWideMinK = 13;
size_t gate_plan_words(uint64_t gates, uint32_t k);
size_t gate_plan_partial_elems(uint64_t gates, uint32_t k);
void launch_gate_plan(GateSpan span, uint32_t k, const uint32_t* offsets, const uint32_t* cursor, const uint32_t* list, uint32_t* plan, hipStream_t s);
struct GateEq {
    const Fr* E;
    const Fr* e_hi;
    const Fr* e_lo_mont;
    uint32_t kl;
};
constexpr uint32_t kGateEqTableMaxKi = 20;
struct GatePlanCounts {
    uint32_t hdr[2][8];
    bool known;
};
size_t gate_plan_arrive_words(uint64_t gates, uint32_t k);
void gate_plan_counts_offsets(uint64_t gates, uint32_t k, size_t* half1_word_offset);
void launch_gate_uv_wide(GateSpan span, uint32_t k_i, uint32_t k, const uint32_t* plan, const GateEq& eq, const Fr* W, Fr* U, Fr* V, LayerBatch lb, Fr* partials,
                         uint32_t* arrive, hipStream_t s, const GateSet* sets = nullptr, const GatePlanCounts* counts = nullptr);
struct WideCFuse {
    const Fr* wu = nullptr;
    Fr* X = nullptr;
    Fr* Y = nullptr;
};
void launch_gate_rows_wide(GateSpan span, uint32_t k_i, uint32_t k, const uint32_t* plan, const GateEq& eq, const Fr* eq_mont, Fr* A_row, Fr* M_row, LayerBatch lb,
                           Fr* partials, uint32_t* arrive, hipStream_t s, const GateSet* sets = nullptr, const GatePlanCounts* counts = nullptr,
                           const WideCFuse* fuse = nullptr);
void launch_eq_outer(const Fr* e_hi, const Fr* e_lo_mont, uint32_t k_i, uint32_t kl, Fr* E, uint32_t batch, hipStream_t s);
void launch_exclusive_scan(const uint32_t* in, uint32_t* out, uint32_t* block_sums, size_t n, hipStream_t s);
void launch_check_canonical(const Fr* t, size_t n, uint32_t* flag, hipStream_t s);
void launch_depends_wide(const Fr* W, uint32_t k, uint32_t* bits, uint32_t* dep, uint32_t* host_dep, uint32_t batch, hipStream_t s, bool bits_preset = false);
void launch_mobius(Fr* tables, uint32_t k, size_t stride, uint32_t batch, hipStream_t s);
void launch_line_setup_wide(const Fr* W, uint32_t k, Fr* scratch, uint32_t* maxdeg_scratch, uint32_t batch, hipStream_t s);

void launch_mle_xwiden(const MleHostRecSub* rec, uint32_t J, uint32_t batch, uint32_t local_fail, long long* limbs, hipStream_t s);
void launch_mle_xnarrow(const long long* limbs, uint32_t J, uint32_t batch, MleHostRecSub* host_rec, uint32_t ticket, uint32_t* fail_out,
                        hipStream_t s);
void launch_mle_gather_widen(const Fr* src, size_t stride, uint32_t t, uint32_t lp, uint32_t shard, uint32_t local_fail, uint32_t batch,
                             long long* limbs, hipStream_t s);
void launch_mle_gather_narrow(const long long* limbs, uint32_t tn, uint32_t batch, Fr* tail, uint32_t* fail_out, hipStream_t s);
void launch_to_mont(const Fr* in, Fr* out, uint32_t count, hipStream_t s);
void launch_depends(const Fr* W, uint32_t k, uint32_t* dep, uint32_t batch, hipStream_t s);
void launch_predicate_scatter(uint32_t k_i, uint32_t k_next, const uint8_t* gate_type, const uint32_t* left,
                              const uint32_t* right, const Fr* e_hi, const Fr* e_lo_mont, uint32_t kl,
                              unsigned long long* wideA, unsigned long long* wideM, uint32_t* bad, uint32_t log_p,
                              uint32_t shard, hipStream_t s);
void launch_to_mont_strided(const Fr* in, Fr* out, uint32_t count, uint32_t stride, uint32_t offset, hipStream_t s);
void launch_tables_differ(const Fr* a, const Fr* b, size_t count, uint32_t* flag, hipStream_t s);
void launch_fold_pair(const Fr* src, Fr* dst, const FixedMul* rtab, hipStream_t s);
void launch_predicate_sorted(uint32_t k_i, uint32_t k_next, const uint8_t* gate_type, const uint32_t* left,
                             const uint32_t* right, const Fr* e_hi, const Fr* e_lo_mont, uint32_t kl, uint32_t log_p,
                             uint32_t shard, size_t ncells, uint32_t* counts, uint32_t* offsets, uint32_t* cursor,
                             uint32_t* block_sums, uint32_t* list, uint32_t* bad, Fr* out_A, Fr* out_M, uint32_t batch,
                             hipStream_t s);
void launch_predicate_normalise(const unsigned long long* wide, Fr* out, size_t cells, hipStream_t s);

void launch_verify_pack(const uint8_t* gate_type, const uint32_t* left, const uint32_t* right, uint32_t gates, uint32_t k, uint2* packed,
                        uint32_t* bad, hipStream_t s);
struct VerifyLayer {
    const uint2* gates;
    const Fr* e_hi;
    const Fr* e_lo;
// ... 38 lines not shown
```

### gkr_amd/csrc/kernels.hip

```cpp
#include <hip/hip_runtime.h>
#include <stdlib.h>

#include <atomic>

#include "kernels.h"
#include "options.h"
#include "dev_util.h"
#include "gate_seg.h"
#include "mfma_fold.h"
#include "mfma_cross.h"
#include "mimc7.h"

namespace gkr {


__device__ __forceinline__ uint64_t mix64(uint64_t z) {
    z = (z ^ (z >> 30)) * 0xBF58476D1CE4E5B9ULL;
    z = (z ^ (z >> 27)) * 0x94D049BB133111EBULL;
    return z ^ (z >> 31);
}

__global__ void k_fill_table(Fr* table, size_t count, uint64_t seed) {
    for (size_t i = blockIdx.x * (size_t)blockDim.x + threadIdx.x; i < count; i += (size_t)gridDim.x * blockDim.x) {
        Fr f;
// ... 149 lines not shown
            Fr x[8];
#pragma unroll
            for (int b = 0; b < 8; ++b) x[b] = load_fr(s + (size_t)(q * 8 + b) * S + i);
            Lazy17 t;
            weighted_sum_s<8>(x, w + q * 8, t);
            y = fr_add(y, lazy_reduce_k8(t));
        }
        return y;
    }
}

__device__ __forceinline__ void mle_total_and_publish(const MleSubPartial* __restrict__ p, uint32_t nblk, uint32_t jout,
                                                      MleHostRecSub* __restrict__ r, uint32_t ticket) {
    __shared__ uint32_t s_pdep;
    __shared__ Acc<10> s_tot[kMleMaxSub], s_wave[16];
    const uint32_t T = blockDim.x, t = threadIdx.x, lane = t & 63u;
    const uint32_t nsub = 1u << jout, per = nblk > T ? nblk / T : 1u, eff = nblk / per, bps = (nblk >> jout) / per;
    if (t == 0) s_pdep = 0;
    __syncthreads();
    Acc<10> tot = acc_zero<10>();
    uint32_t dep = 0;
    if (t < eff) {
        for (uint32_t i = 0; i < per; ++i) {
            acc_add_acc(tot, p[(size_t)t * per + i].sum);
            dep |= p[(size_t)t * per + i].dep;
        }
    }
    if (__any(dep) && lane == 0) atomicOr(&s_pdep, 1u);
    const uint32_t seg = bps < 64u ? bps : 64u;
    for (uint32_t off = seg >> 1; off >= 1u; off >>= 1) {
        Acc<10> o;
#pragma unroll
        for (int l = 0; l < 10; ++l) o.l[l] = __shfl_down(tot.l[l], off, 64);
        acc_add_acc(tot, o);
    }
    if (bps <= 64u) {
        if (t < eff && (t & (seg - 1u)) == 0) s_tot[t / seg] = tot;
        __syncthreads();
    } else {
        if (t < eff && lane == 0) s_wave[t >> 6] = tot;
        __syncthreads();
        if (t < nsub) {
            Acc<10> a = acc_zero<10>();
            for (uint32_t w = 0; w < (bps >> 6); ++w) acc_add_acc(a, s_wave[t * (bps >> 6) + w]);
            s_tot[t] = a;
        }
    }
    if (t < nsub) r->sums[t] = acc_reduce(s_tot[t]);
    __syncthreads();
    if (t == 0) {
        r->dep = s_pdep;
        __hip_atomic_store(&r->seq, ticket, __ATOMIC_RELEASE, __HIP_MEMORY_SCOPE_SYSTEM);
    }
}

__device__ __forceinline__ void mle_publish_from_last_block(const MleSubPartial* __restrict__ partials, const MlePublish& pub) {
    __shared__ uint32_t s_last;
    const uint32_t b = blockIdx.y, nblk = gridDim.x;
    if (threadIdx.x == 0) {
        __threadfence();
        s_last = atomicAdd(pub.arrivals + b, 1u) == nblk - 1u ? 1u : 0u;
    }
    __syncthreads();
    if (!s_last) return;
    __threadfence();
    if (threadIdx.x == 0) pub.arrivals[b] = 0u;
    mle_total_and_publish(partials + (size_t)b * nblk, nblk, pub.jout, pub.rec + b, pub.ticket);
}

__global__ void __launch_bounds__(256) k_mle_sub_sums(const Fr* __restrict__ tables, size_t table_stride, uint32_t len,
                                                      MleSubPartial* __restrict__ partials, MlePublish pub) {
    __shared__ Acc<9> smem[4];
    __shared__ uint32_t s_dep;
    const Fr* t = tables + (size_t)blockIdx.y * table_stride;
    const uint32_t chunk = len / gridDim.x;
    const uint32_t begin = blockIdx.x * chunk, end = begin + chunk;
    Acc<9> acc[1] = {acc_zero<9>()};
    uint32_t dep = 0;
    if (threadIdx.x == 0) s_dep = 0;
    __syncthreads();
    for (uint32_t i = begin + threadIdx.x; i < end; i += blockDim.x) {
        const Fr x = load_fr(t + i);
        acc_add_fr(acc[0], x);
        uint32_t d = 0;
#pragma unroll
        for (int k = 0; k < 8; ++k) d |= x.l[k] ^ (uint32_t)__builtin_amdgcn_mov_dpp((int)x.l[k], 0xB1, 0xF, 0xF, true);
        dep |= d;
    }
    if (dep) atomicOr(&s_dep, 1u);
    block_sum<9, 1>(acc, smem);
    if (threadIdx.x == 0) {
        MleSubPartial* p = partials + (size_t)blockIdx.y * gridDim.x + blockIdx.x;
        p->sum = acc[0];
        p->dep = s_dep;
    }
    if (pub.arrivals) mle_publish_from_last_block(partials, pub);
}

template <int JIN>
__global__ void __launch_bounds__(256) k_mle_multifold(const Fr* __restrict__ src, size_t src_stride, Fr* __restrict__ dst,
                                                       size_t dst_stride, uint32_t S, const Fr* __restrict__ weights,
                                                       MleSubPartial* __restrict__ partials, MlePublish pub) {
    __shared__ Acc<9> smem[4];
    const Fr* s = src + (size_t)blockIdx.y * src_stride;
    Fr* d = dst + (size_t)blockIdx.y * dst_stride;
    const Fr* w = weights + (size_t)blockIdx.y * kMleMaxSub;
    const uint32_t chunk = S / gridDim.x;
    const uint32_t begin = blockIdx.x * chunk, end = begin + chunk;
    Acc<9> acc[1] = {acc_zero<9>()};
    for (uint32_t i = begin + threadIdx.x; i < end; i += blockDim.x) {
        const Fr y = multifold_entry<JIN>(s, S, i, w);
        store_fr(d + i, y);
        acc_add_fr(acc[0], y);
    }
    block_sum<9, 1>(acc, smem);
    if (threadIdx.x == 0) {
        MleSubPartial* p = partials + (size_t)blockIdx.y * gridDim.x + blockIdx.x;
        p->sum = acc[0];
        p->dep = 0;
    }
    if (pub.arrivals) mle_publish_from_last_block(partials, pub);
}

template <int JIN>
__global__ void __launch_bounds__(1024) k_mle_fold_plan(const Fr* __restrict__ weights, MfmaFoldPlan* __restrict__ plans) {
    __shared__ __attribute__((aligned(16))) unsigned char digits[32 * 32 * (1 << JIN)];
    mfma_plan_block<JIN>(weights + (size_t)blockIdx.x * kMleMaxSub, plans + blockIdx.x, digits);
}

template <int JIN>
__global__ void __launch_bounds__(256) k_mle_multifold_mfma(const Fr* __restrict__ src, size_t src_stride, Fr* __restrict__ dst,
                                                            size_t dst_stride, uint32_t S, const MfmaFoldPlan* __restrict__ plans,
                                                            MleSubPartial* __restrict__ partials, MlePublish pub) {
    __shared__ Acc<9> smem[4];
    __shared__ __attribute__((aligned(16))) unsigned char digits[JIN > 2 ? 32 * 32 * (1 << JIN) : 16];
    const Fr* s = src + (size_t)blockIdx.y * src_stride;
    Fr* d = dst + (size_t)blockIdx.y * dst_stride;
    const uint32_t chunk = S / gridDim.x;
    const uint32_t begin = blockIdx.x * chunk;
    Acc<9> acc[1] = {acc_zero<9>()};
    mfma_multifold_block<JIN>(s, d, S, plans + blockIdx.y, begin, begin + chunk, blockIdx.x * 5u + blockIdx.y * 3u, acc[0], digits);
    block_sum<9, 1>(acc, smem);
    if (threadIdx.x == 0) {
        MleSubPartial* p = partials + (size_t)blockIdx.y * gridDim.x + blockIdx.x;
        p->sum = acc[0];
        p->dep = 0;
    }
    if (pub.arrivals) mle_publish_from_last_block(partials, pub);
}

__global__ void __launch_bounds__(512) k_mle_sub_reduce(const MleSubPartial* __restrict__ partials, uint32_t nblk,
                                                        uint32_t jout, MleHostRecSub* __restrict__ host_rec, uint32_t ticket) {
    mle_total_and_publish(partials + (size_t)blockIdx.x * nblk, nblk, jout, host_rec + blockIdx.x, ticket);
}

__global__ void __launch_bounds__(256) k_mle_sums_small(const Fr* __restrict__ src, size_t src_stride, uint32_t S, uint32_t jout,
                                                        MleHostRecSub* __restrict__ host_rec, uint32_t ticket) {
    const uint32_t b = blockIdx.x;
    const Fr* tbl = src + (size_t)b * src_stride;
    const uint32_t sub = S >> jout, nsub = 1u << jout;
    MleHostRecSub* r = host_rec + b;
    uint32_t dep = 0;
    __shared__ Acc<9> s_part[256];
    const uint32_t tps = 256u >> jout, sb = threadIdx.x / tps, rr = threadIdx.x % tps;
    Acc<9> acc = acc_zero<9>();
    for (uint32_t i = rr; i < sub; i += tps) {
        const Fr x = load_fr(tbl + (size_t)sb * sub + i);
        acc_add_fr(acc, x);
        dep |= fr_eq(x, load_fr(tbl + (((size_t)sb * sub + i) ^ 1u))) ? 0u : 1u;
    }
    s_part[threadIdx.x] = acc;
    __syncthreads();
    for (uint32_t step = tps >> 1; step >= 1u; step >>= 1) {
        if (rr < step) {
            Acc<9> mine = s_part[threadIdx.x];
            acc_add_acc(mine, s_part[threadIdx.x + step]);
            s_part[threadIdx.x] = mine;
        }
        __syncthreads();
    }
    if (threadIdx.x < nsub) r->sums[threadIdx.x] = acc_reduce(s_part[threadIdx.x * tps]);
    dep = __syncthreads_or(dep);
    if (threadIdx.x == 0) {
        r->dep = dep ? 1u : 0u;
        __hip_atomic_store(&r->seq, ticket, __ATOMIC_RELEASE, __HIP_MEMORY_SCOPE_SYSTEM);
    }
}

__global__ void __launch_bounds__(1024) k_mle_multifold_small(const Fr* __restrict__ src, size_t src_stride, Fr* __restrict__ dst,
                                                              size_t dst_stride, uint32_t S, uint32_t jin, uint32_t jout,
                                                              const Fr* __restrict__ weights, MleHostRecSub* __restrict__ host_rec,
                                                              uint32_t ticket, Fr* __restrict__ tail, uint32_t tail_stride) {
    __shared__ Fr s_w[kMleMaxSub];
    __shared__ Fr s_y[1024];
    __shared__ Acc<9> s_part[kMleMaxSub];
    const uint32_t b = blockIdx.x;
    const Fr* s = src + (size_t)b * src_stride;
    Fr* d = dst + (size_t)b * dst_stride;
    const uint32_t nterm = 1u << jin;
    if (threadIdx.x < nterm * 8u)
        s_w[threadIdx.x >> 3].l[threadIdx.x & 7u] = reinterpret_cast<const uint32_t*>(weights + (size_t)b * kMleMaxSub)[threadIdx.x];
    __syncthreads();
    const uint32_t items = S << jin, per = items > 1024u ? items >> 10 : 1u, groups = nterm / per;
    const uint32_t i = threadIdx.x & (S - 1u), q = threadIdx.x / S;
    if (q < groups) {
        Lazy17 acc = lazy_zero();
        for (uint32_t t = 0; t < per; ++t) {
            const uint32_t term = q * per + t;
            lazy_mac_v(acc, load_fr(s + (size_t)term * S + i), s_w[term]);
        }
        s_y[q * S + i] = lazy_reduce(acc);
    }
    __syncthreads();
    Fr y;
    if (threadIdx.x < S) {
        Acc<9> tot = acc_zero<9>();
        for (uint32_t g = 0; g < groups; ++g) acc_add_fr(tot, s_y[g * S + threadIdx.x]);
        y = acc_reduce(tot);
        store_fr(d + threadIdx.x, y);
        if (tail) store_fr(tail + (size_t)b * tail_stride + threadIdx.x, y);
    }
    if (tail) __threadfence_system();
    __syncthreads();
    if (threadIdx.x < S) s_y[threadIdx.x] = y;
    __syncthreads();
    const uint32_t nsub = 1u << jout, sub = S >> jout;
    uint32_t tps = 1024u >> jout;
    if (tps > sub) tps = sub;
    const uint32_t sb = threadIdx.x / tps, rr = threadIdx.x % tps;
    MleHostRecSub* r = host_rec + b;
    const bool mine = sb < nsub;
    Acc<9> acc = acc_zero<9>();
    if (mine)
        for (uint32_t k = rr; k < sub; k += tps) acc_add_fr(acc, s_y[sb * sub + k]);
    const uint32_t within = tps < 64u ? tps : 64u;
    for (uint32_t off = within >> 1; off >= 1u; off >>= 1) {
        Acc<9> o;
#pragma unroll
        for (int l = 0; l < 9; ++l) o.l[l] = __shfl_down(acc.l[l], off, 64);
        acc_add_acc(acc, o);
    }
    if (tps > 64u) {
        __shared__ Acc<9> s_wave[16];
        if (mine && (threadIdx.x & 63u) == 0) s_wave[threadIdx.x >> 6] = acc;
        __syncthreads();
        if (threadIdx.x < nsub) {
            Acc<9> tot = acc_zero<9>();
            for (uint32_t w = 0; w < (tps >> 6); ++w) acc_add_acc(tot, s_wave[threadIdx.x * (tps >> 6) + w]);
            s_part[threadIdx.x] = tot;
        }
    } else if (mine && rr == 0) {
        s_part[sb] = acc;
    }
    __syncthreads();
    if (threadIdx.x < nsub) r->sums[threadIdx.x] = acc_reduce(s_part[threadIdx.x]);
    __syncthreads();
    if (threadIdx.x == 0) {
        r->dep = 0u;
        __hip_atomic_store(&r->seq, ticket, __ATOMIC_RELEASE, __HIP_MEMORY_SCOPE_SYSTEM);
    }
}

__global__ void __launch_bounds__(256) k_mle_fold_sum_small(const Fr* __restrict__ src, size_t src_stride,
                                                            Fr* __restrict__ dst, size_t dst_stride, uint32_t q,
                                                            const FixedMul* __restrict__ rtab,
                                                            MleHostRec* __restrict__ host_rec, uint32_t ticket) {
    __shared__ Acc<9> smem[4 * 2];
    const uint32_t b = blockIdx.x;
    const Fr* s = src + (size_t)b * src_stride;
    Fr* d = dst + (size_t)b * dst_stride;
    const FixedMul T = rtab[b];
    Acc<9> acc[2] = {acc_zero<9>(), acc_zero<9>()};
    for (uint32_t i = threadIdx.x; i < q; i += blockDim.x) {
        Fr x0 = load_fr(s + i), x1 = load_fr(s + i + 2 * (size_t)q);
        Fr x2 = load_fr(s + i + q), x3 = load_fr(s + i + 3 * (size_t)q);
        Fr y0 = fr_fold_fixed(x0, x1, T);
        Fr y1 = fr_fold_fixed(x2, x3, T);
        store_fr(d + i, y0);
        store_fr(d + i + q, y1);
        acc_add_fr(acc[0], y0);
        acc_add_fr(acc[1], y1);
    }
    block_sum<9, 2>(acc, smem);
    if (threadIdx.x == 0) {
        Fr c0 = acc_reduce(acc[0]);
        Fr c1 = fr_sub(acc_reduce(acc[1]), c0);
        MleHostRec* r = host_rec + b;
        r->c0 = c0;
        r->c1 = c1;
        r->dep = 0;
        __hip_atomic_store(&r->seq, ticket, __ATOMIC_RELEASE, __HIP_MEMORY_SCOPE_SYSTEM);
    }
}

__global__ void __launch_bounds__(64) k_mle_round_reduce(const MlePartial* __restrict__ partials, uint32_t nblk,
                                                         MleHostRec* __restrict__ host_rec, uint32_t ticket) {
    const uint32_t b = blockIdx.x;
    const MlePartial* p = partials + (size_t)b * nblk;
    Acc<10> lo = acc_zero<10>(), hi = acc_zero<10>();
    uint32_t dep = 0;
    for (uint32_t i = threadIdx.x; i < nblk; i += 64) {
        acc_add_acc(lo, p[i].lo);
        acc_add_acc(hi, p[i].hi);
        dep |= p[i].dep;
    }
    lo = wave_sum(lo);
// ... 1567 lines not shown
            uint32_t *cnt = seg_scratch, *off = cnt + a, *asums = off + a, *lh = asums + ablocks + 1, *ls = lh + b, *bsums = ls + b,
                     *csums = bsums + bblocks + 1;
            segs->shift = p.shift;
            segs->runs = p.runs;
            segs->run_base = p.run_base;
            segs->bound = p.bound;
            segs->half_bound = p.half_bound;
            segs->groups = p.groups;
            segs->nb = 1u << k;
            segs->packed_half = p.packed_half;
            const dim3 sg((unsigned)((a + 255) / 256));
            hipLaunchKernelGGL(k_seg_count, sg, dim3(256), 0, s, starts, hist, lblocks, p.m, p.runs, p.nseg, cnt);
            hipLaunchKernelGGL(k_scan_blocks, dim3(ablocks), dim3(256), 0, s, cnt, off, asums, a);
            hipLaunchKernelGGL(k_scan_sums, dim3(1), dim3(1024), 0, s, asums, ablocks);
            hipLaunchKernelGGL(k_scan_add, dim3(ablocks), dim3(256), 0, s, off, (uint32_t*)nullptr, asums, a);
            hipLaunchKernelGGL(k_seg_fill, sg, dim3(256), 0, s, starts, hist, lblocks, p.m, p.runs, p.nseg, off, segs->items(), segs->bucket_begin());
            const uint32_t per = (p.bound + p.len_blocks - 1) / p.len_blocks;
            hipLaunchKernelGGL(k_seg_len_hist, dim3(p.len_blocks), dim3(256), 0, s, segs->items(), segs->bucket_begin(), 1u << k, per, lh);
            hipLaunchKernelGGL(k_scan_blocks, dim3(bblocks), dim3(256), 0, s, lh, ls, bsums, b);
            hipLaunchKernelGGL(k_scan_sums, dim3(1), dim3(1024), 0, s, bsums, bblocks);
            hipLaunchKernelGGL(k_scan_add, dim3(bblocks), dim3(256), 0, s, ls, (uint32_t*)nullptr, bsums, b);
            hipLaunchKernelGGL(k_seg_len_fill, dim3(p.len_blocks), dim3(256), 0, s, segs->items(), segs->bucket_begin(), 1u << k, per, ls, segs->order());
            const size_t c = 2 * (size_t)p.groups + 1;
            const uint32_t cblocks = (uint32_t)((c + kScanPerBlock - 1) / kScanPerBlock);
            hipLaunchKernelGGL(k_seg_group_len, dim3((unsigned)((c + 255) / 256)), dim3(256), 0, s, segs->items(), segs->order(), segs->bucket_begin(),
                               1u << k, p.groups, segs->group_len());
            hipLaunchKernelGGL(k_scan_blocks, dim3(cblocks), dim3(256), 0, s, segs->group_len(), segs->group_off(), csums, c);
            hipLaunchKernelGGL(k_scan_sums, dim3(1), dim3(1024), 0, s, csums, cblocks);
            hipLaunchKernelGGL(k_scan_add, dim3(cblocks), dim3(256), 0, s, segs->group_off(), (uint32_t*)nullptr, csums, c);
            hipLaunchKernelGGL(k_seg_pack, dim3((2 * p.groups + 3) / 4), dim3(256), 0, s, segs->items(), segs->order(), segs->bucket_begin(), 1u << k, p.groups,
                               segs->group_len(), segs->group_off(), list, list + gate_list_words(gates), (uint32_t)span.base, p.shift,
                               segs->packed());
        }
        return;
    }
    const uint32_t gblocks = blocks_for(gates, 4096);
    const uint32_t sblocks = (uint32_t)((n + kScanPerBlock - 1) / kScanPerBlock);
    hipLaunchKernelGGL(k_gate_count, dim3(gblocks), dim3(256), 0, s, gates, k, gate_type, left, right, counts, bad);
    hipLaunchKernelGGL(k_scan_blocks, dim3(sblocks), dim3(256), 0, s, counts, offsets, block_sums, n);
    hipLaunchKernelGGL(k_scan_sums, dim3(1), dim3(1024), 0, s, block_sums, sblocks);
    hipLaunchKernelGGL(k_scan_add, dim3(sblocks), dim3(256), 0, s, offsets, cursor, block_sums, n);
    hipLaunchKernelGGL(k_gate_fill, dim3(gblocks), dim3(256), 0, s, gates, k, gate_type, left, right, cursor, list, list + gate_list_words(gates));
}

static uint32_t device_cus() {
    static std::atomic<uint32_t> cus[64];
    int dev = 0;
    if (hipGetDevice(&dev) != hipSuccess) return 256u;
    std::atomic<uint32_t>& slot = cus[dev & 63];
    uint32_t n = slot.load(std::memory_order_relaxed);
    if (!n) {
        hipDeviceProp_t prop;
        n = (hipGetDeviceProperties(&prop, dev) == hipSuccess && prop.multiProcessorCount >= 1) ? (uint32_t)prop.multiProcessorCount : 256u;
        slot.store(n, std::memory_order_relaxed);
    }
    return n;
}
template <bool ROWS, bool LDS_T>
static void launch_seg_pass_t(const GateSegs& g, uint32_t k, const Fr* e_lo_mont, const Fr* T, Fr* X, Fr* Y, LayerBatch lb, hipStream_t s) {
    const uint32_t tlen = 1u << k;
    const size_t lds = LDS_T ? (size_t)tlen * sizeof(Fr) : 0;
    static std::atomic<uint64_t> attr_set{0};
    int dev = 0;
    (void)hipGetDevice(&dev);
    if (LDS_T && !((attr_set.load(std::memory_order_relaxed) >> (dev & 63)) & 1u)) {
        if (hipFuncSetAttribute(reinterpret_cast<const void*>(&k_seg_pass<ROWS, LDS_T>), hipFuncAttributeMaxDynamicSharedMemorySize, 160 * 1024) != hipSuccess) {
            (void)hipGetLastError();
            launch_seg_pass_t<ROWS, false>(g, k, e_lo_mont, T, X, Y, lb, s);
            return;
        }
        attr_set.fetch_or((uint64_t)1 << (dev & 63), std::memory_order_relaxed);
    }
    const uint32_t blocks = LDS_T ? device_cus() : 4 * device_cus();
    hipLaunchKernelGGL((k_seg_pass<ROWS, LDS_T>), dim3(blocks, lb.batch), dim3(LDS_T ? 1024 : 256), lds, s, g.items(), g.order(), g.bucket_begin(),
                       g.nb, g.groups, g.group_len(), g.group_off(), g.packed(), e_lo_mont, g.shift, T, tlen,
                       (uint32_t)lb.wstride, X, Y, g.half_bound);
}
static void launch_seg_pass(bool rows, const GateSegs& g, uint32_t k, const Fr* e_lo_mont, const Fr* T, Fr* X, Fr* Y, LayerBatch lb, hipStream_t s) {
    const bool no_lds = opt(OPT_gate_segments_no_lds) != 0;
    const bool lds_t = !no_lds && ((size_t)sizeof(Fr) << k) <= 128 * 1024;
    if (rows)
        lds_t ? launch_seg_pass_t<true, true>(g, k, e_lo_mont, T, X, Y, lb, s) : launch_seg_pass_t<true, false>(g, k, e_lo_mont, T, X, Y, lb, s);
    else
        lds_t ? launch_seg_pass_t<false, true>(g, k, e_lo_mont, T, X, Y, lb, s) : launch_seg_pass_t<false, false>(g, k, e_lo_mont, T, X, Y, lb, s);
}

void launch_exclusive_scan(const uint32_t* in, uint32_t* out, uint32_t* block_sums, size_t n, hipStream_t s) {
    const uint32_t sblocks = (uint32_t)((n + kScanPerBlock - 1) / kScanPerBlock);
    hipLaunchKernelGGL(k_scan_blocks, dim3(sblocks), dim3(256), 0, s, in, out, block_sums, n);
    hipLaunchKernelGGL(k_scan_sums, dim3(1), dim3(1024), 0, s, block_sums, sblocks);
    hipLaunchKernelGGL(k_scan_add, dim3(sblocks), dim3(256), 0, s, out, (uint32_t*)nullptr, block_sums, n);
}

static uint32_t bucket_threads(uint64_t gates, uint32_t k) { return (gates >> k) > 64u ? 256u : 64u; }

void launch_gate_uv(GateSpan span, uint32_t k_i, uint32_t k, const uint32_t* offsets, const uint32_t* cursor, const uint32_t* list,
                    const Fr* e_hi, const Fr* e_lo_mont, uint32_t kl, const Fr* W, Fr* U, Fr* V, LayerBatch lb, const GateSegs* segs,
                    Fr* partials, hipStream_t s, const GateSet* sets) {
    if (segs && segs->shift && partials && !sets) {
        Fr *X = partials, *Y = partials + (size_t)segs->half_bound * lb.batch;
        launch_seg_pass(false, *segs, k, e_lo_mont, W, X, Y, lb, s);
        hipLaunchKernelGGL(k_seg_combine, dim3(((1u << k) + 1u) / 2u, lb.batch), dim3(64), 0, s, segs->items(), segs->bucket_begin(), 0u, 1u << k, X, Y,
                           segs->half_bound, e_hi, k_i - segs->shift, segs->run_base, U, V, (uint32_t)lb.wstride, CPhaseFuse{});
        return;
    }
    hipLaunchKernelGGL(k_gate_uv, dim3(1u << k, lb.batch), dim3(bucket_threads(span.count, k)), 0, s, offsets, cursor, list,
                       list + gate_list_words(span.count), e_hi, e_lo_mont, kl, k_i - kl, W, U, V, (uint32_t)lb.wstride, (uint32_t)span.base, sets);
}

bool launch_gate_rows(GateSpan span, uint32_t k_i, uint32_t k, const uint32_t* offsets, const uint32_t* cursor, const uint32_t* list,
                      const Fr* e_hi, const Fr* e_lo_mont, uint32_t kl, const Fr* eq_mont, Fr* A_row, Fr* M_row, LayerBatch lb,
                      const GateSegs* segs, Fr* partials, hipStream_t s, const CPhaseFuse* fuse, const GateSet* sets) {
    if (segs && segs->shift && partials && !sets) {
        Fr *X = partials, *Y = partials + (size_t)segs->half_bound * lb.batch;
        launch_seg_pass(true, *segs, k, e_lo_mont, eq_mont, X, Y, lb, s);
        hipLaunchKernelGGL(k_seg_combine, dim3(((1u << k) + 1u) / 2u, lb.batch), dim3(64), 0, s, segs->items(), segs->bucket_begin(), 1u << k, 1u << k, X, Y,
                           segs->half_bound, e_hi, k_i - segs->shift, segs->run_base, A_row, M_row, (uint32_t)lb.wstride, fuse ? *fuse : CPhaseFuse{});
        return fuse != nullptr;
    }
    hipLaunchKernelGGL(k_gate_rows, dim3(1u << k, lb.batch), dim3(bucket_threads(span.count, k)), 0, s, offsets, cursor, list,
                       list + gate_list_words(span.count), e_hi, e_lo_mont, kl, k_i - kl, eq_mont, A_row, M_row, k, (uint32_t)lb.wstride,
                       (uint32_t)span.base, sets);
    return false;
}

void launch_predicate_normalise(const unsigned long long* wide, Fr* out, size_t cells, hipStream_t s) {
    hipLaunchKernelGGL(k_predicate_normalise, dim3(blocks_for(cells, 4096)), dim3(256), 0, s, wide, out, cells);
}

void launch_mle_fold_sum_small(const Fr* src, size_t src_stride, Fr* dst, size_t dst_stride, uint32_t q, uint32_t batch,
                               const FixedMul* rtab, MleHostRec* host_rec, uint32_t ticket, hipStream_t s) {
    hipLaunchKernelGGL(k_mle_fold_sum_small, dim3(batch), dim3(256), 0, s, src, src_stride, dst, dst_stride, q, rtab,
                       host_rec, ticket);
}

uint32_t mle_pass_blocks(uint32_t items, uint32_t jout, uint32_t batch) {
    uint32_t want = mle_blocks_per_table(items, batch);
    uint32_t b = 1u << jout;
    while (b < want && b * 2 <= items && b * 2 <= kMaxBlocksPerTable) b <<= 1;
    if (b > items) b = items;
    return b;
}

void launch_mle_sub_sums(const Fr* tables, size_t stride, uint32_t len, uint32_t batch, uint32_t nblk, MleSubPartial* partials,
                         hipStream_t s, const MlePublish* publish) {
    hipLaunchKernelGGL(k_mle_sub_sums, dim3(nblk, batch), dim3(256), 0, s, tables, stride, len, partials, publish ? *publish : MlePublish{});
}

void launch_mle_sub_reduce(const MleSubPartial* partials, uint32_t nblk, uint32_t jout, uint32_t batch, MleHostRecSub* host_rec,
                           uint32_t ticket, hipStream_t s) {
    hipLaunchKernelGGL(k_mle_sub_reduce, dim3(batch), dim3(512), 0, s, partials, nblk, jout, host_rec, ticket);
}

bool mle_multifold_uses_mfma(uint32_t S, uint32_t nblk) {
    const bool off = opt(OPT_no_mfma_fold) != 0;
    return !off && nblk > 0 && S % nblk == 0 && (S / nblk) % 64u == 0;
}

size_t mle_fold_plan_bytes() { return sizeof(MfmaFoldPlan); }

void launch_mle_fold_plan(int jin, const Fr* weights, void* plans, uint32_t batch, hipStream_t s) {
    MfmaFoldPlan* pl = static_cast<MfmaFoldPlan*>(plans);
    if (jin == 1)
        hipLaunchKernelGGL(k_mle_fold_plan<1>, dim3(batch), dim3(64), 0, s, weights, pl);
    else if (jin == 2)
        hipLaunchKernelGGL(k_mle_fold_plan<2>, dim3(batch), dim3(128), 0, s, weights, pl);
    else if (jin == 3)
        hipLaunchKernelGGL(k_mle_fold_plan<3>, dim3(batch), dim3(256), 0, s, weights, pl);
    else if (jin == 4)
        hipLaunchKernelGGL(k_mle_fold_plan<4>, dim3(batch), dim3(512), 0, s, weights, pl);
    else
        hipLaunchKernelGGL(k_mle_fold_plan<5>, dim3(batch), dim3(1024), 0, s, weights, pl);
}

void launch_mle_multifold(int jin, const Fr* src, size_t src_stride, Fr* dst, size_t dst_stride, uint32_t S, uint32_t batch,
                          uint32_t nblk, const Fr* weights, const void* plans, MleSubPartial* partials, hipStream_t s,
                          const MlePublish* publish) {
    dim3 grid(nblk, batch);
    const MlePublish pub = publish ? *publish : MlePublish{};
    if (mle_multifold_uses_mfma(S, nblk)) {
        const MfmaFoldPlan* pl = static_cast<const MfmaFoldPlan*>(plans);
        if (jin == 1)
            hipLaunchKernelGGL(k_mle_multifold_mfma<1>, grid, dim3(256), 0, s, src, src_stride, dst, dst_stride, S, pl, partials, pub);
        else if (jin == 2)
            hipLaunchKernelGGL(k_mle_multifold_mfma<2>, grid, dim3(256), 0, s, src, src_stride, dst, dst_stride, S, pl, partials, pub);
        else if (jin == 3)
            hipLaunchKernelGGL(k_mle_multifold_mfma<3>, grid, dim3(256), 0, s, src, src_stride, dst, dst_stride, S, pl, partials, pub);
        else if (jin == 4)
            hipLaunchKernelGGL(k_mle_multifold_mfma<4>, grid, dim3(256), 0, s, src, src_stride, dst, dst_stride, S, pl, partials, pub);
        else
            hipLaunchKernelGGL(k_mle_multifold_mfma<5>, grid, dim3(256), 0, s, src, src_stride, dst, dst_stride, S, pl, partials, pub);
        return;
    }
    if (jin == 1)
        hipLaunchKernelGGL(k_mle_multifold<1>, grid, dim3(256), 0, s, src, src_stride, dst, dst_stride, S, weights, partials, pub);
    else if (jin == 2)
        hipLaunchKernelGGL(k_mle_multifold<2>, grid, dim3(256), 0, s, src, src_stride, dst, dst_stride, S, weights, partials, pub);
    else
        hipLaunchKernelGGL(k_mle_multifold<3>, grid, dim3(256), 0, s, src, src_stride, dst, dst_stride, S, weights, partials, pub);
}

uint32_t mle_multifold_blocks(uint32_t S, uint32_t jout, uint32_t batch) {
    const bool off = opt(OPT_no_mfma_fold) != 0;
    if (off) return mle_pass_blocks(S, jout, batch);
    const uint32_t target = opt(OPT_fold_blocks) > 0 ? (uint32_t)opt(OPT_fold_blocks) : 65536u;
    const uint32_t mc = (uint32_t)opt(OPT_fold_min_chunk);
    const uint32_t min_chunk = mc >= 64u && (mc & (mc - 1u)) == 0 ? mc : 256u;
    uint32_t b = 1u << jout;
    while ((uint64_t)b * batch < target && S / (2u * b) >= min_chunk && 2u * b <= kMaxBlocksPerTable) b <<= 1;
    if (b > S) b = S;
    return b;
}

void launch_mle_multifold_small(int jin, const Fr* src, size_t src_stride, Fr* dst, size_t dst_stride, uint32_t S, uint32_t jout,
                                uint32_t batch, const Fr* weights, MleHostRecSub* host_rec, uint32_t ticket, hipStream_t s, Fr* tail, uint32_t tail_stride) {
    dim3 grid(batch);
    if (jin == 0)
        hipLaunchKernelGGL(k_mle_sums_small, grid, dim3(256), 0, s, src, src_stride, S, jout, host_rec, ticket);
    else
        hipLaunchKernelGGL(k_mle_multifold_small, grid, dim3(1024), 0, s, src, src_stride, dst, dst_stride, S, (uint32_t)jin, jout, weights,
                           host_rec, ticket, tail, tail_stride);
}

void launch_mle_round_reduce(const MlePartial* partials, uint32_t nblk, uint32_t batch, MleHostRec* host_rec,
                             uint32_t ticket, hipStream_t s) {
    hipLaunchKernelGGL(k_mle_round_reduce, dim3(batch), dim3(64), 0, s, partials, nblk, host_rec, ticket);
}


}
```

### gkr_amd/csrc/mfma_fold.h

```cpp
#pragma once
#include "fr32.h"

namespace gkr {

constexpr int kMfmaMaxJ = 5;

#if defined(__HIP_DEVICE_COMPILE__) || defined(__HIPCC__)

typedef int mf_v4i __attribute__((ext_vector_type(4)));
typedef int mf_v16i __attribute__((ext_vector_type(16)));
typedef uint32_t mf_v2u __attribute__((ext_vector_type(2)));
typedef uint32_t mf_v4u __attribute__((ext_vector_type(4)));

__constant__ const uint32_t kMfmaColumnBias[kMfmaMaxJ][32] = {
    {0x2000f3, 0x2000a9, 0x2000e0, 0x2000af, 0x2000bc, 0x2000a4, 0x20007a, 0x20007a, 0x200093, 0x20009f, 0x200035,
     0x2000d6, 0x200006, 0x200035, 0x20007d, 0x20004d, 0x2000d7, 0x20003f, 0x2000fc, 0x200030, 0x20009b, 0x200087,
     0x200017, 0x2000d2, 0x200026, 0x200072, 0x2000b6, 0x200064, 0x200095, 0x20002d, 0x2000e0, 0x200006},
    {0x4000e6, 0x400053, 0x4000c1, 0x40005f, 0x400079, 0x400049, 0x4000f5, 0x4000f4, 0x400026, 0x40003f, 0x40006b,
     0x4000ac, 0x40000d, 0x40006a, 0x4000fa, 0x40009a, 0x4000ae, 0x40007f, 0x4000f8, 0x400061, 0x400036, 0x40000f,
     0x40002f, 0x4000a4, 0x40004d, 0x4000e4, 0x40006c, 0x4000c9, 0x40002a, 0x40005b, 0x4000c0, 0x40000d},
    {0x8000cc, 0x8000a7, 0x800082, 0x8000bf, 0x8000f2, 0x800092, 0x8000ea, 0x8000e9, 0x80004d, 0x80007e, 0x8000d6,
     0x800058, 0x80001b, 0x8000d4, 0x8000f4, 0x800035, 0x80005d, 0x8000ff, 0x8000f0, 0x8000c3, 0x80006c, 0x80001e,
     0x80005e, 0x800048, 0x80009b, 0x8000c8, 0x8000d9, 0x800092, 0x800055, 0x8000b6, 0x800080, 0x80001b},
    {0x1000097, 0x100004f, 0x1000005, 0x100008f, 0x1000051, 0x1000030, 0x10000f3, 0x100008f, 0x100000a, 0x100008c, 0x10000f3,
     0x1000037, 0x10000ee, 0x10000bf, 0x10000b5, 0x1000043, 0x100005d, 0x10000a6, 0x1000060, 0x1000006, 0x1000023, 0x10000f7,
     0x100006b, 0x10000d8, 0x100000c, 0x10000f1, 0x1000081, 0x1000044, 0x1000038, 0x100001e, 0x100009d, 0x1000006},
    {0x200002e, 0x200009f, 0x200000a, 0x200001e, 0x20000a3, 0x2000060, 0x20000e6, 0x200001f, 0x2000015, 0x2000018, 0x20000e7,
     0x200006f, 0x20000dc, 0x200007f, 0x200006b, 0x2000087, 0x20000ba, 0x200004c, 0x20000c1, 0x200000c, 0x2000046, 0x20000ee,
     0x20000d7, 0x20000b0, 0x2000019, 0x20000e2, 0x2000003, 0x2000089, 0x2000070, 0x200003c, 0x200003a, 0x200000d}};

__device__ __forceinline__ Fr mf_reduce_274(const uint32_t (&l)[9]) {
    constexpr uint32_t p[8] = GKR_MOD_LIMBS;
    constexpr uint32_t mu = 0xa948e8c4u;
    const uint64_t t1 = (uint64_t)l[7] * mu, t2 = (uint64_t)l[8] * mu;
    const uint32_t q = (uint32_t)((t2 + (t1 >> 32)) >> 29);
    uint32_t r[8];
    uint64_t prod = 0;
    uint32_t borrow = 0;
#pragma unroll
    for (int i = 0; i < 8; ++i) {
        prod += (uint64_t)q * p[i];
        const uint32_t s = (uint32_t)prod;
        prod >>= 32;
        const uint64_t d = (uint64_t)l[i] - s - borrow;
        r[i] = (uint32_t)d;
        borrow = (uint32_t)(d >> 63);
    }
    return cond_sub_mod(r);
}

struct alignas(16) MfmaFoldPlan {
    unsigned char digits[32 * 32 * (1 << kMfmaMaxJ)];
    int32_t start[2][16];
};

template <int JIN>
__device__ __forceinline__ void mfma_plan_block(const Fr* __restrict__ w_mont, MfmaFoldPlan* __restrict__ plan,
                                                unsigned char* lds ) {
    constexpr int NB = 1 << JIN;
    constexpr int K = 32 * NB;
    const uint32_t tid = threadIdx.x, lane = tid & 63u, c = lane & 31u, h = lane >> 5;
    __shared__ uint32_t w_lds[8 * NB];
    for (uint32_t i = tid; i < (uint32_t)(8 * NB); i += blockDim.x) w_lds[i] = reinterpret_cast<const uint32_t*>(w_mont)[i];
    __syncthreads();
    for (uint32_t row = tid; row < (uint32_t)K; row += blockDim.x) {
        const uint32_t b = row >> 5, j = row & 31u;
        Fr sh = fr_zero(), wb;
        sh.l[j >> 2] = 1u << (8u * (j & 3u));
#pragma unroll
        for (int i = 0; i < 8; ++i) wb.l[i] = w_lds[b * 8u + (uint32_t)i];
        const Fr R = mont_mul(wb, sh);
        uint32_t carry = 0;
        const uint32_t base = ((b * 2u + (j >> 4)) * 32u) * 16u + (j & 15u);
#pragma unroll
        for (int m = 0; m < 32; ++m) {
            uint32_t v = ((R.l[m >> 2] >> (8 * (m & 3))) & 0xffu) + carry;
            carry = (v + 128u) >> 8;
            lds[base + (uint32_t)m * 16u] = (unsigned char)v;
        }
    }
    __syncthreads();
    for (uint32_t i = tid; i < (uint32_t)(32 * K / 16); i += blockDim.x)
        reinterpret_cast<mf_v4u*>(plan->digits)[i] = reinterpret_cast<const mf_v4u*>(lds)[i];
    if (tid < 64u) {
        mf_v16i t = {0, 0, 0, 0, 0, 0, 0, 0, 0, 0, 0, 0, 0, 0, 0, 0};
        const mf_v4i x64 = {0x40404040, 0x40404040, 0x40404040, 0x40404040};
#pragma unroll
        for (int b = 0; b < NB; ++b) {
            const mf_v4i wf = *reinterpret_cast<const mf_v4i*>(lds + ((b * 2 + h) * 32 + c) * 16);
            t = __builtin_amdgcn_mfma_i32_32x32x32_i8(wf, x64, t, 0, 0, 0);
        }
        if (c == 0) {
#pragma unroll
            for (int r = 0; r < 16; ++r)
                plan->start[h][r] = 2 * t[r] + (int)kMfmaColumnBias[JIN - 1][(r & 3) + 8 * (r >> 2) + 4 * h];
        }
    }
}

__device__ __forceinline__ Fr mf_finish(const mf_v16i& a0, const mf_v16i& a1) {
    uint64_t ev[4], od[4];
#pragma unroll
    for (int g = 0; g < 4; ++g) {
        const uint64_t v0 = (uint64_t)(uint32_t)a0[4 * g] + ((uint64_t)(uint32_t)a0[4 * g + 1] << 8) +
                            ((uint64_t)(uint32_t)a0[4 * g + 2] << 16) + ((uint64_t)(uint32_t)a0[4 * g + 3] << 24);
        const uint64_t v1 = (uint64_t)(uint32_t)a1[4 * g] + ((uint64_t)(uint32_t)a1[4 * g + 1] << 8) +
                            ((uint64_t)(uint32_t)a1[4 * g + 2] << 16) + ((uint64_t)(uint32_t)a1[4 * g + 3] << 24);
        const mf_v2u lo = __builtin_amdgcn_permlane32_swap((uint32_t)v0, (uint32_t)v1, false, false);
        const mf_v2u hi = __builtin_amdgcn_permlane32_swap((uint32_t)(v0 >> 32), (uint32_t)(v1 >> 32), false, false);
        ev[g] = (uint64_t)lo.x | ((uint64_t)hi.x << 32);
        od[g] = (uint64_t)lo.y | ((uint64_t)hi.y << 32);
    }
    uint32_t l[9];
    uint64_t run = 0;
#pragma unroll
    for (int g = 0; g < 4; ++g) {
        run += ev[g];
        l[2 * g] = (uint32_t)run;
        run >>= 32;
        run += od[g];
        l[2 * g + 1] = (uint32_t)run;
        run >>= 32;
    }
    l[8] = (uint32_t)run;
    return mf_reduce_274(l);
}

template <int JIN, class Sink>
__device__ __forceinline__ void mfma_multifold_stream(const Fr* __restrict__ s, uint32_t S, const MfmaFoldPlan* __restrict__ plan,
                                                      uint32_t begin, uint32_t end, uint32_t rot, unsigned char* lds, Sink&& sink) {
    constexpr int NB = 1 << JIN;
    constexpr int KS = NB < 8 ? NB : 8;
    constexpr int NST = NB / KS;
    constexpr bool kRegs = NB <= 4;
    const uint32_t tid = threadIdx.x, lane = tid & 63u, c = lane & 31u, h = lane >> 5;
    mf_v4i wf[kRegs ? NB : 1];
    if constexpr (kRegs) {
#pragma unroll
        for (int b = 0; b < NB; ++b) wf[b] = *reinterpret_cast<const mf_v4i*>(plan->digits + ((b * 2 + h) * 32 + c) * 16);
    } else {
        for (uint32_t i = tid; i < (uint32_t)(32 * 32 * NB / 16); i += blockDim.x)
            reinterpret_cast<mf_v4u*>(lds)[i] = reinterpret_cast<const mf_v4u*>(plan->digits)[i];
        __syncthreads();
    }
    mf_v16i init;
#pragma unroll
    for (int r = 0; r < 16; ++r) init[r] = plan->start[h][r];

    const uint32_t wave = __builtin_amdgcn_readfirstlane(tid >> 6);
    auto load_stage = [&](uint32_t e0, int stage, mf_v4u (&x)[2][KS]) {
        const uint32_t voff = c * 32u + 16u * h;
        const Fr* tile = s + e0;
#pragma unroll
        for (int k = 0; k < KS; ++k) {
#if defined(MF_STREAM_PAD)
            const char* base = reinterpret_cast<const char*>(tile + (size_t)(stage * KS + k) * (S + MF_STREAM_PAD));
#else
            const char* base = reinterpret_cast<const char*>(tile + (size_t)(stage * KS + k) * S);
#endif
#pragma unroll
            for (int t = 0; t < 2; ++t)
                x[t][k] = __builtin_nontemporal_load(reinterpret_cast<const mf_v4u*>(base + voff + 1024u * t));
        }
    };
    auto mac_stage = [&](int stage, const mf_v4u (&x)[2][KS], mf_v16i& a0, mf_v16i& a1) {
#pragma unroll
        for (int k = 0; k < KS; ++k) {
            mf_v4i w;
            if constexpr (kRegs)
                w = wf[stage * KS + k];
            else
                w = *reinterpret_cast<const mf_v4i*>(lds + (((stage * KS + k) * 2 + h) * 32 + c) * 16);
            const mf_v4u f0 = x[0][k] ^ 0x80808080u, f1 = x[1][k] ^ 0x80808080u;
            a0 = __builtin_amdgcn_mfma_i32_32x32x32_i8(w, (mf_v4i)f0, a0, 0, 0, 0);
            a1 = __builtin_amdgcn_mfma_i32_32x32x32_i8(w, (mf_v4i)f1, a1, 0, 0, 0);
        }
    };
    auto store_entry = [&](uint32_t e0, const mf_v16i& a0, const mf_v16i& a1) { sink(e0, h, c, mf_finish(a0, a1)); };

    const uint32_t span = end - begin;
    const uint32_t iters = (span + 255u) / 256u;
    const uint32_t woff = wave * 64u;
    if (woff >= span) return;
    uint32_t cur = rot % iters;
    auto next_pos = [&]() {
        cur = cur + 1u == iters ? 0u : cur + 1u;
        return begin + cur * 256u + woff;
    };
    mf_v4u xa[2][KS], xb[2][KS];
    uint32_t e0 = begin + cur * 256u + woff;
    load_stage(e0, 0, xa);
    if constexpr (NST == 1) {
        for (uint32_t it = 0; it < iters; it += 2u) {
            const bool more1 = it + 1u < iters;
            const uint32_t e1 = next_pos();
            if (more1) load_stage(e1, 0, xb);
            {
                mf_v16i a0 = init, a1 = init;
                mac_stage(0, xa, a0, a1);
                store_entry(e0, a0, a1);
            }
            __builtin_amdgcn_sched_barrier(0);
            if (!more1) break;
            const bool more2 = it + 2u < iters;
            e0 = next_pos();
            if (more2) load_stage(e0, 0, xa);
            {
                mf_v16i a0 = init, a1 = init;
                mac_stage(0, xb, a0, a1);
                store_entry(e1, a0, a1);
            }
            __builtin_amdgcn_sched_barrier(0);
        }
    } else {
        for (uint32_t it = 0; it < iters; ++it) {
            const bool more = it + 1u < iters;
            const uint32_t e1 = next_pos();
            mf_v16i a0 = init, a1 = init;
#pragma unroll
            for (int st = 0; st < NST; st += 2) {
                load_stage(e0, st + 1, xb);
                mac_stage(st, xa, a0, a1);
                __builtin_amdgcn_sched_barrier(0);
                if (st + 2 < NST)
                    load_stage(e0, st + 2, xa);
                else if (more)
                    load_stage(e1, 0, xa);
                mac_stage(st + 1, xb, a0, a1);
                __builtin_amdgcn_sched_barrier(0);
            }
            store_entry(e0, a0, a1);
            e0 = e1;
        }
    }
}

template <int JIN>
__device__ __forceinline__ void mfma_multifold_block(const Fr* __restrict__ s, Fr* __restrict__ d, uint32_t S,
                                                     const MfmaFoldPlan* __restrict__ plan, uint32_t begin, uint32_t end,
                                                     uint32_t rot, Acc<9>& acc_out, unsigned char* lds) {
    mfma_multifold_stream<JIN>(s, S, plan, begin, end, rot, lds, [&](uint32_t e0, uint32_t h, uint32_t c, const Fr& y) {
        mf_v4u* o = reinterpret_cast<mf_v4u*>(d + e0 + 32u * h + c);
        const mf_v4u y0 = {y.l[0], y.l[1], y.l[2], y.l[3]}, y1 = {y.l[4], y.l[5], y.l[6], y.l[7]};
        __builtin_nontemporal_store(y0, o);
        __builtin_nontemporal_store(y1, o + 1);
        acc_add_fr(acc_out, y);
    });
}

#endif

}
```

### gkr_amd/csrc/mimc_ifma.cpp

```cpp
#include <immintrin.h>
#include <stdint.h>
#include <string.h>

#include "mimc_ifma.h"

namespace gkr {
namespace ifma {

typedef unsigned __int128 u128;
static const uint64_t M52 = (1ULL << 52) - 1;

struct V {
    __m512i l[5];
};

static void to52(const uint64_t x[4], uint64_t o[5]) {
    o[0] = x[0] & M52;
    o[1] = ((x[0] >> 52) | (x[1] << 12)) & M52;
    o[2] = ((x[1] >> 40) | (x[2] << 24)) & M52;
    o[3] = ((x[2] >> 28) | (x[3] << 36)) & M52;
    o[4] = x[3] >> 16;
}
static void from52(const uint64_t l[5], uint64_t x[4]) {
    x[0] = l[0] | (l[1] << 52);
// ... 572 lines not shown
        }
        uint64_t* base = weights + (size_t)8 * w * w_row_words;
        for (int b = 0; b < cur; ++b) scatter8(wv[b], base + 4 * (size_t)b, off_w[w], valid[w]);
    }
}

template <int W>
static void prod_pass_w(const uint64_t* recs, size_t rec_row_words, int count, int J, const uint32_t (*vec_len)[16], uint64_t (*c2)[16][4],
                        uint64_t (*lin)[16][4], uint64_t (*c0)[16][4], uint64_t (*r)[16][4], uint64_t* weights, size_t w_row_words) {
    const V r2 = splat(g_r2_52), one = splat(g_one52);
    V zero;
    for (int i = 0; i < 5; ++i) zero.l[i] = _mm512_setzero_si512();
    V M[W][64], SY[W][8], rm[3][W];
    __m512i off_in[W], off_out[W], off_w[W];
    __mmask8 valid[W];
    int cnt[W];
    const int n = 1 << J;
    for (int w = 0; w < W; ++w) {
        cnt[w] = count - 8 * w < 0 ? 0 : (count - 8 * w > 8 ? 8 : count - 8 * w);
        valid[w] = (__mmask8)((1u << cnt[w]) - 1);
        off_in[w] = lane_offsets(rec_row_words, cnt[w]);
        off_out[w] = lane_offsets(4, cnt[w]);
        off_w[w] = lane_offsets(w_row_words, cnt[w]);
        const uint64_t* base = recs + (size_t)(cnt[w] ? 8 * w : 0) * rec_row_words;
        for (int a = 0; a < n; ++a) {
            for (int b = 0; b < n; ++b) M[w][a * 8 + b] = gather8(base + 4 * (size_t)(a * 8 + b), off_in[w]);
            SY[w][a] = gather8(base + 4 * (size_t)(64 + a), off_in[w]);
        }
    }
    for (int t = 0; t < J; ++t) {
        const int half = 1 << (J - t - 1);
        V vc2[W], vlin[W], vc0[W], a[W], acc[W], h[W];
        __mmask8 three[W];
        unsigned any_three = 0;
        for (int w = 0; w < W; ++w) {
            V p00 = M[w][0], p01 = M[w][half], p10 = M[w][half * 8], p11 = M[w][half * 8 + half], s0 = SY[w][0], s1 = SY[w][half];
            for (int x = 1; x < half; ++x) {
                p00 = add_mod(p00, M[w][x * 8 + x]);
                p01 = add_mod(p01, M[w][x * 8 + half + x]);
                p10 = add_mod(p10, M[w][(half + x) * 8 + x]);
                p11 = add_mod(p11, M[w][(half + x) * 8 + half + x]);
                s0 = add_mod(s0, SY[w][x]);
                s1 = add_mod(s1, SY[w][half + x]);
            }
            vc0[w] = add_mod(p00, s0);
            const V g1 = add_mod(p11, s1);
            vc2[w] = sub_mod(add_mod(p11, p00), add_mod(p10, p01));
            vlin[w] = sub_mod(sub_mod(g1, vc0[w]), vc2[w]);
            three[w] = 0;
            for (int k = 0; k < cnt[w]; ++k)
                if (vec_len[t][8 * w + k] == 3) three[w] |= (__mmask8)(1u << k);
            any_three |= three[w];
            scatter8(vc2[w], &c2[t][8 * w][0], off_out[w], valid[w]);
            scatter8(vlin[w], &lin[t][8 * w][0], off_out[w], valid[w]);
            scatter8(vc0[w], &c0[t][8 * w][0], off_out[w], valid[w]);
            acc[w] = zero;
        }
        if (any_three) {
            for (int w = 0; w < W; ++w) a[w] = mont_mul(vc2[w], r2);
            mimc7_hash_w<W>(a, acc, h);
            for (int w = 0; w < W; ++w) {
                const V nr = add_mod(add_mod(acc[w], a[w]), h[w]);
                for (int i = 0; i < 5; ++i) acc[w].l[i] = _mm512_mask_blend_epi64(three[w], acc[w].l[i], nr.l[i]);
            }
        }
        for (int w = 0; w < W; ++w) a[w] = mont_mul(vlin[w], r2);
        mimc7_hash_w<W>(a, acc, h);
        for (int w = 0; w < W; ++w) acc[w] = add_mod(add_mod(acc[w], a[w]), h[w]);
        for (int w = 0; w < W; ++w) a[w] = mont_mul(vc0[w], r2);
        mimc7_hash_w<W>(a, acc, h);
        for (int w = 0; w < W; ++w) {
            rm[t][w] = add_mod(add_mod(acc[w], a[w]), h[w]);
            scatter8(mont_mul(rm[t][w], one), &r[t][8 * w][0], off_out[w], valid[w]);
            const V x = rm[t][w];
            for (int ra = 0; ra < half; ++ra)
                for (int cb = 0; cb < 2 * half; ++cb)
                    M[w][ra * 8 + cb] = add_mod(M[w][ra * 8 + cb], mont_mul(sub_mod(M[w][(half + ra) * 8 + cb], M[w][ra * 8 + cb]), x));
            for (int ra = 0; ra < half; ++ra)
                for (int cb = 0; cb < half; ++cb)
                    M[w][ra * 8 + cb] = add_mod(M[w][ra * 8 + cb], mont_mul(sub_mod(M[w][ra * 8 + half + cb], M[w][ra * 8 + cb]), x));
            for (int ra = 0; ra < half; ++ra) SY[w][ra] = add_mod(SY[w][ra], mont_mul(sub_mod(SY[w][half + ra], SY[w][ra]), x));
        }
    }
    if (!weights) return;
    for (int w = 0; w < W; ++w) {
        if (!cnt[w]) continue;
        V* wv = M[w];
        wv[0] = splat(g_r256_52);
        int cur = 1;
        for (int t = 0; t < J; ++t) {
            for (int b = cur; b-- > 0;) {
                const V hi = mont_mul(wv[b], rm[t][w]);
                wv[2 * b + 1] = hi;
                wv[2 * b] = sub_mod(wv[b], hi);
            }
            cur <<= 1;
        }
        uint64_t* base = weights + (size_t)8 * w * w_row_words;
        for (int b = 0; b < cur; ++b) scatter8(wv[b], base + 4 * (size_t)b, off_w[w], valid[w]);
    }
}

}

void gkr_ifma_prod_pass(const uint64_t* recs, size_t rec_row_words, int count, int J, const uint32_t (*vec_len)[16], uint64_t (*c2)[16][4],
                        uint64_t (*lin)[16][4], uint64_t (*c0)[16][4], uint64_t (*r)[16][4], uint64_t* weights, size_t w_row_words) {
    if (count > 8)
        ifma::prod_pass_w<2>(recs, rec_row_words, count, J, vec_len, c2, lin, c0, r, weights, w_row_words);
    else
        ifma::prod_pass_w<1>(recs, rec_row_words, count, J, vec_len, c2, lin, c0, r, weights, w_row_words);
}

void gkr_ifma_tail_pass(uint64_t* tables, size_t stride, uint32_t m, uint32_t jp, const uint64_t* weights, uint32_t J, uint64_t* rec) {
    using namespace ifma;
    const uint32_t mf = m - jp, len = 1u << mf, nsub = 1u << J, S = len >> J;
    const V c264 = splat(g_r264_52);
    if (jp) {
        V w[8];
        for (uint32_t b = 0; b < (1u << jp); ++b) {
            uint64_t l[5];
            to52(weights + 4 * b, l);
            w[b] = mont_mul(splat(l), c264);
        }
        for (int t = 0; t < 3; ++t) {
            uint64_t* T = tables + (size_t)t * stride * 4;
            for (uint32_t i = 0; i < len; i += 8) {
                const int count = len - i < 8 ? (int)(len - i) : 8;
                const __m512i off = lane_offsets(4, count);
                V acc = mont_mul(gather8(T + (size_t)i * 4, off), w[0]);
                for (uint32_t b = 1; b < (1u << jp); ++b) acc = add_mod(acc, mont_mul(gather8(T + (((size_t)b << mf) + i) * 4, off), w[b]));
                scatter8(acc, T + (size_t)i * 4, off, (__mmask8)((1u << count) - 1u));
            }
        }
    }
    const uint64_t *W = tables, *X = tables + stride * 4, *Y = tables + 2 * stride * 4;
    const __m512i sub_off = lane_offsets((size_t)S * 4, (int)nsub);
    const __mmask8 sub_lanes = (__mmask8)((1u << nsub) - 1u);
    const __m512i rec_off = lane_offsets(4, (int)nsub);
    uint64_t zero52[5] = {0, 0, 0, 0, 0};
    for (uint32_t a = 0; a < nsub; ++a) {
        V acc = splat(zero52);
        for (uint32_t i = 0; i < S; ++i) {
            uint64_t l[5];
            to52(W + ((size_t)a * S + i) * 4, l);
            acc = add_mod(acc, mont_mul(splat(l), gather8(X + (size_t)i * 4, sub_off)));
        }
        scatter8(mont_mul(acc, c264), rec + (size_t)a * 8 * 4, rec_off, sub_lanes);
    }
    V ysum = splat(zero52);
    for (uint32_t i = 0; i < S; ++i) ysum = add_mod(ysum, gather8(Y + (size_t)i * 4, sub_off));
    scatter8(ysum, rec + 64 * 4, rec_off, sub_lanes);
}

void gkr_ifma_pass(const uint64_t* sums, size_t sums_row_words, int count, int J, const uint32_t* final_len, uint64_t (*c0)[16][4],
                   uint64_t (*c1)[16][4], uint64_t (*r)[16][4], uint32_t (*len)[16], uint64_t* weights, size_t w_row_words) {
    if (count > 8)
        ifma::pass_w<2>(sums, sums_row_words, count, J, final_len, c0, c1, r, len, weights, w_row_words);
    else
        ifma::pass_w<1>(sums, sums_row_words, count, J, final_len, c0, c1, r, len, weights, w_row_words);
}

bool gkr_ifma_available() {
#if defined(__x86_64__)
    return __builtin_cpu_supports("avx512f") && __builtin_cpu_supports("avx512ifma");
#else
    return false;
#endif
}

void gkr_ifma_init(const uint64_t (*cts_canonical)[4]) { ifma::init_constants(cts_canonical); }

void gkr_ifma_multi_hash8(const uint64_t (*vec)[3][4], const uint32_t* len, int slots, uint64_t (*out)[4]) {
    using namespace ifma;
    const V r2 = splat(g_r2_52), one = splat(g_one52);
    V r;
    for (int i = 0; i < 5; ++i) r.l[i] = _mm512_setzero_si512();
    for (int s = 0; s < slots; ++s) {
        uint64_t in[8][4];
        __mmask8 active = 0;
        for (int k = 0; k < 8; ++k) {
            memcpy(in[k], vec[k][s], 32);
            if ((uint32_t)(slots - s) <= len[k]) active |= (__mmask8)(1u << k);
        }
        if (!active) continue;
        const V a = mont_mul(load8(in), r2);
        const V h = mimc7_hash(a, r);
        const V nr = add_mod(add_mod(r, a), h);
        for (int i = 0; i < 5; ++i) r.l[i] = _mm512_mask_blend_epi64(active, r.l[i], nr.l[i]);
    }
    store8(mont_mul(r, one), out);
}

void gkr_ifma_multi_hash16(const uint64_t (*vec)[3][4], const uint32_t* len, int slots, uint64_t (*out)[4]) {
    ifma::multi_hash_w<2>(vec, len, slots, out);
}

}
```

### gkr_amd/csrc/mimc_ifma.h

```cpp
#pragma once
#include <stdint.h>

namespace gkr {
bool gkr_ifma_available();
void gkr_ifma_init(const uint64_t (*cts_canonical)[4]);
void gkr_ifma_multi_hash8(const uint64_t (*vec)[3][4], const uint32_t* len, int slots, uint64_t (*out)[4]);
void gkr_ifma_multi_hash16(const uint64_t (*vec)[3][4], const uint32_t* len, int slots, uint64_t (*out)[4]);
void gkr_ifma_pass(const uint64_t* sums, size_t sums_row_words, int count, int J, const uint32_t* final_len, uint64_t (*c0)[16][4],
                   uint64_t (*c1)[16][4], uint64_t (*r)[16][4], uint32_t (*len)[16], uint64_t* weights, size_t w_row_words);
void gkr_ifma_prod_pass(const uint64_t* recs, size_t rec_row_words, int count, int J, const uint32_t (*vec_len)[16], uint64_t (*c2)[16][4],
                        uint64_t (*lin)[16][4], uint64_t (*c0)[16][4], uint64_t (*r)[16][4], uint64_t* weights, size_t w_row_words);
void gkr_ifma_tail_pass(uint64_t* tables, size_t stride, uint32_t m, uint32_t jp, const uint64_t* weights, uint32_t J, uint64_t* rec);
}
```

### gkr_amd/csrc/options.h

```cpp
#pragma once
#include <stdlib.h>
#include <string.h>

namespace gkr {

#define GKR_CONTEXT_OPTIONS(X)                                                                                                       \
                                                                  \
    X(rounds_per_pass, "rounds_per_pass", "GKR_ROUNDS_PER_PASS", 0, "rounds a pass of the plain sumcheck covers (0: 5; 3 without the MFMA fold)") \
    X(no_mfma_fold, "no_mfma_fold", "GKR_NO_MFMA_FOLD", 0, "fold passes on v_mad_u64_u32 instead of int8 MFMA")                      \
    X(no_fused_reduce, "no_fused_reduce", "GKR_NO_FUSED_REDUCE", 0, "latency-bound passes publish through k_mle_sub_reduce instead of from their last block") \
    X(hash_chunk, "hash_chunk", "GKR_HASH_CHUNK", 0, "8 or 16: sumchecks per host hash call (0: 16 when host threads are scarce)")    \
    X(device_hash_percent, "device_hash_percent", "GKR_DEVICE_HASH_PERCENT", 0, "share of a batch of >= 64 plain sumchecks hashed on the device (0..90)") \
    X(group_size, "group_size", "GKR_GROUP_SIZE", 0, "sumchecks per scheduling group of a batch (0: groups of ~4 GiB of tables)")     \
    X(pass_queue_depth, "pass_queue_depth", "GKR_PASS_QUEUE_DEPTH", 0, "groups whose pass 0 is queued up front (0: two)")           \
    X(no_late_stream, "no_late_stream", "GKR_NO_LATE_STREAM", 0, "a group's small late passes stay on the main stream")              \
    X(plan_main, "plan_main", "GKR_PLAN_MAIN", 0, "the fold plan (digit matrix) on the main stream instead of the side stream")       \
    X(mle_per_round, "mle_per_round", "GKR_MLE_PER_ROUND", 0, "one variable per pass (the first schedule; what the device transcript uses)") \
    X(fold_blocks, "fold_blocks", "GKR_FOLD_BLOCKS", 0, "target block count of a fold pass (0: 65536)")                              \
    X(fold_min_chunk, "fold_min_chunk", "GKR_FOLD_MIN_CHUNK", 0, "smallest chunk of entries per fold block (0: 256)")                \
    X(items_per_block, "items_per_block", "GKR_ITEMS_PER_BLOCK", 0, "entries per block of the first pass (0: 1024)")                 \
                                                                \
    X(predicate_atomics, "predicate_atomics", "GKR_PREDICATE_ATOMICS", 0, "dense predicate tables by widened-atomic scatter instead of the counting sort") \
    X(gate_groups_min_k, "gate_groups_min_k", "GKR_GATE_GROUPS_MIN_K", -1, "smallest k_next whose layers take the wide layers' item passes (-1: 13)") \
    X(no_fused_publish, "no_fused_publish", "GKR_NO_FUSED_PUBLISH", 0, "product passes publish through a second launch instead of from their last block") \
    X(gate_sort_global, "gate_sort_global", "GKR_GATE_SORT_GLOBAL", 0, "the gate lists' counting sort with global atomics where the LDS sort applies") \
    X(gate_segments_off, "gate_segments_off", "GKR_GATE_SEGMENTS_OFF", 0, "bucket kernels instead of the segment passes on large layers") \
    X(gate_segments_min_log2, "gate_segments_min_log2", "GKR_GATE_SEGMENTS_MIN_LOG2", 22, "smallest layer (log2 gates) that takes the segment passes") \
    X(gate_segment_log2, "gate_segment_log2", "GKR_GATE_SEGMENT_LOG2", 0, "log2 of the segments' mean length (0: 4)")              \
    X(gate_segments_no_lds, "gate_segments_no_lds", "GKR_GATE_SEGMENTS_NO_LDS", 0, "the segment pass gathers its table from L2 instead of LDS") \
    X(no_mfma_cross, "no_mfma_cross", "GKR_NO_MFMA_CROSS", 0, "wide layers' product passes over tables of 2^15 entries and more on v_mad_u64_u32 instead of int8 MFMA") \
    X(prod_cross_min_log2, "prod_cross_min_log2", "GKR_PROD_CROSS_MIN_LOG2", 0, "smallest tables (log2 entries, at least 13) whose cross sums of a product pass run on the matrix cores (0: 15)") \
    X(prod_fold_min_log2, "prod_fold_min_log2", "GKR_PROD_FOLD_MIN_LOG2", 0, "smallest tables (log2 entries) whose pending fold of a product pass runs on the matrix cores (0: 17)") \
    X(host_tail_log2, "host_tail_log2", "GKR_HOST_TAIL_LOG2", 0, "a phase's product passes over tables of 2^this entries and fewer run on the host (0: 6; -1: none; at most 12)") \
    X(host_tail_max_batch, "host_tail_max_batch", "GKR_HOST_TAIL_MAX_BATCH", 0, "largest batch (proofs advancing together) whose small product passes run on the host (0: 8)") \
    X(line_stepwise, "line_stepwise", "GKR_LINE_STEPWISE", 0, "q_i in its wide-layer form (one launch per variable) at every width")  \
    X(layer_no_fused, "layer_no_fused", "GKR_LAYER_NO_FUSED", 0, "device transcript: separate fold and sum kernels in the b-phase")   \
                                  \
    X(no_circuit_cache, "no_circuit_cache", "GKR_NO_CIRCUIT_CACHE", 0, "do not keep proven circuits' gate arrays and lists on the device between calls") \
    X(prove_many_pieces, "prove_many_pieces", "GKR_PROVE_MANY_PIECES", 0, "gkr_prove_many: cut the costliest items in two until there are this many")      \
    X(prove_many_lockstep, "prove_many_lockstep", "GKR_PROVE_MANY_LOCKSTEP", 1, "gkr_prove_many: items whose circuits share a k list advance in lockstep, one launch per pass for the group (0: one chain per item)") \
    X(lockstep_max_proofs, "lockstep_max_proofs", "GKR_LOCKSTEP_MAX_PROOFS", 0, "most proofs one lockstep group may hold (0: 32 -- beyond that independent chains overlap better)") \
                                                                \
    X(verify_workspace_mb, "verify_workspace_mb", "GKR_VERIFY_WORKSPACE_MB", 0, "gkr_verify_prepared / gkr_sumcheck_mle_verify*: MiB of device workspace a chunk of proofs may take (0: 2048; a chunk is never less than one proof)") \
    X(verify_device_hash_min, "verify_device_hash_min", "GKR_VERIFY_DEVICE_HASH_MIN", 0, "gkr_verify_prepared / gkr_sumcheck_mle_verify*: smallest number of round vectors in a chunk whose challenge hashes run on the device (0: the measured default, capi_verify.hip kVerifyDeviceHashMinRows; -1: never, the host threads hash; 1: always)") \
                         \
    X(mle_eval_mfma_min_n, "mle_eval_mfma_min_n", "GKR_MLE_EVAL_MFMA_MIN_N", 0, "gkr_mle_eval_batch_device / gkr_sumcheck_mle_verify*: smallest n whose tables are evaluated by the streaming matrix-core kernel (0: the default, kernels.h kMleEvalMfmaMinN; never below 11, where the kernel starts to apply; above 24: the one-block kernel up to n = 24, its largest)")

enum OptionId : int {
#define GKR_OPT_ENUM(id, name, env, def, doc) OPT_##id,
    GKR_CONTEXT_OPTIONS(GKR_OPT_ENUM)
#undef GKR_OPT_ENUM
        OPT_COUNT
};

struct OptionInfo {
    const char* name;
    const char* env;
    long long def;
    const char* doc;
};

inline const OptionInfo* option_table() {
    static const OptionInfo table[OPT_COUNT] = {
#define GKR_OPT_ROW(id, name, env, def, doc) {name, env, def, doc},
        GKR_CONTEXT_OPTIONS(GKR_OPT_ROW)
#undef GKR_OPT_ROW
    };
    return table;
}

struct Options {
    long long v[OPT_COUNT];
    static Options from_environment() {
        Options o;
        const OptionInfo* t = option_table();
        for (int i = 0; i < OPT_COUNT; ++i) {
            o.v[i] = t[i].def;
            if (const char* e = getenv(t[i].env)) {
                char* end = nullptr;
                const long long val = strtoll(e, &end, 0);
                o.v[i] = end != e ? val : 1;
            }
        }
        return o;
    }
};

inline int option_index(const char* name) {
    if (!name) return -1;
    const OptionInfo* t = option_table();
    for (int i = 0; i < OPT_COUNT; ++i)
        if (!strcmp(t[i].name, name) || !strcmp(t[i].env, name)) return i;
    return -1;
}

inline const Options*& current_options() {
    static thread_local const Options* cur = nullptr;
    return cur;
}
inline const Options& default_options() {
    static const Options d = Options::from_environment();
    return d;
}
inline long long opt(OptionId id) {
    const Options* o = current_options();
    return (o ? o : &default_options())->v[id];
}
struct OptionScope {
    const Options* prev;
    explicit OptionScope(const Options* o) : prev(current_options()) { current_options() = o; }
    ~OptionScope() { current_options() = prev; }
    OptionScope(const OptionScope&) = delete;
    OptionScope& operator=(const OptionScope&) = delete;
};

inline bool process_switch(const char* env) { return getenv(env) != nullptr; }
inline int process_int(const char* env, int def) {
    const char* e = getenv(env);
    return e ? atoi(e) : def;
}
inline bool debug_timing() {
    static const bool on = process_switch("GKR_DEBUG_TIMING");
    return on;
}

}
```

### include/gkr_amd.h

```cpp
#ifndef GKR_AMD_H
#define GKR_AMD_H

#include <stddef.h>
#include <stdint.h>

#ifdef __cplusplus
extern "C" {
#endif

typedef struct { uint64_t l[4]; } gkr_fr;

typedef struct gkr_ctx gkr_ctx;

#define GKR_MAX_K_NEXT 24
#define GKR_MAX_K_I 28
#define GKR_MAX_K_NEXT_DEVICE_TRANSCRIPT 14
#define GKR_MAX_MLE_N 30
#define GKR_MAX_BATCH 4096

enum {
    GKR_OK = 0,
    GKR_ERR_INVALID = 1,
    GKR_ERR_NON_CANONICAL = 2,
    GKR_ERR_NO_DEVICE = 3,
    GKR_ERR_HIP = 4,
    GKR_ERR_NOMEM = 5,
    GKR_ERR_DEGENERATE = 6,
    GKR_ERR_UNSUPPORTED = 7
};

enum {
    GKR_TRANSCRIPT_DEVICE = 0,
    GKR_TRANSCRIPT_HOST = 1
};

const char *gkr_strerror(int status);
const char *gkr_version(void);

int  gkr_ctx_create(int device_id, gkr_ctx **out);
int  gkr_ctx_create_multi(const int *device_ids, int n_devices, gkr_ctx **out);
int  gkr_ctx_device_count(const gkr_ctx *ctx);
void gkr_ctx_destroy(gkr_ctx *ctx);
const char *gkr_last_error(const gkr_ctx *ctx);
int  gkr_ctx_set_transcript(gkr_ctx *ctx, int mode);
int  gkr_ctx_set_host_threads(gkr_ctx *ctx, int threads);
int  gkr_ctx_set_option(gkr_ctx *ctx, const char *name, long long value);
int  gkr_ctx_get_option(const gkr_ctx *ctx, const char *name, long long *value);
int  gkr_option_count(void);
const char *gkr_option_name(int index);
const char *gkr_option_doc(int index);
const char *gkr_option_env(int index);
int  gkr_ctx_device_name(const gkr_ctx *ctx, char *buf, size_t len);
long gkr_host_help_while(const volatile int32_t *busy);
int  gkr_host_accounting(int enable);
int  gkr_host_accounting_read(double *out_us, size_t count);

int  gkr_ctx_profile(gkr_ctx *ctx, int enable);
int  gkr_ctx_profile_get(gkr_ctx *ctx, const char *kernel, uint64_t *launches, double *total_ms,
                         double *algorithmic_bytes);
int  gkr_ctx_profile_samples(gkr_ctx *ctx, const char *kernel, double *ms, double *bytes, size_t capacity, size_t *count);
int  gkr_ctx_profile_reset(gkr_ctx *ctx);

int  gkr_mimc7_multi_hash(const gkr_fr *arr, size_t n, const gkr_fr *key, gkr_fr *out);
int  gkr_mimc7_hash(const gkr_fr *x, const gkr_fr *k, gkr_fr *out);
int  gkr_mimc7_constant(int i, gkr_fr *out);
int  gkr_selftest_mul(const gkr_fr *a, const gkr_fr *b, gkr_fr *out);
int  gkr_selftest_wide_sum(const gkr_fr *vals, size_t n, gkr_fr *out);
int  gkr_selftest_hash8(const gkr_fr *vecs, const uint32_t *len, gkr_fr *out, int *used_ifma);
int  gkr_selftest_host_pass(const gkr_fr *sums, int count, int J, const uint32_t *final_len, gkr_fr *c0, gkr_fr *c1,
                            uint32_t *len, gkr_fr *r, gkr_fr *w, int *used_ifma);
int  gkr_selftest_host_tail(const gkr_fr *tables, int m, int jp, const gkr_fr *weights, int J, gkr_fr *rec, int *used_ifma);
int  gkr_selftest_host_prod_pass(const gkr_fr *recs, int count, int J, const uint32_t *vec_len, gkr_fr *c2, gkr_fr *lin,
                                 gkr_fr *c0, gkr_fr *r, gkr_fr *w, int *used_ifma);
int  gkr_selftest_dot(const gkr_fr *a, const gkr_fr *b, size_t n, gkr_fr *out);
int  gkr_selftest_pass_schedule(int n, int mfma, uint32_t *rounds, size_t capacity, size_t *passes);
int  gkr_selftest_line_restriction(int k, const gkr_fr *W, const gkr_fr *b, const gkr_fr *c, gkr_fr *out, uint32_t *out_len);
int  gkr_selftest_seg_item(const gkr_fr *e_lo, const gkr_fr *t, const uint8_t *is_mult, size_t n, const gkr_fr *e_hi, int rows,
                           gkr_fr *out0, gkr_fr *out1);
int  gkr_selftest_fold(const gkr_fr *lo, const gkr_fr *hi, const gkr_fr *r, gkr_fr *out);

enum {
    GKR_DEVTEST_FR_ADD = 0, GKR_DEVTEST_FR_SUB, GKR_DEVTEST_MONT_MUL, GKR_DEVTEST_FR_MUL, GKR_DEVTEST_TO_MONT,
    GKR_DEVTEST_FROM_MONT, GKR_DEVTEST_MUL_FIXED, GKR_DEVTEST_MUL_FIXED2, GKR_DEVTEST_FOLD_FIXED, GKR_DEVTEST_FOLD_FIXED2
};
enum {
    GKR_DEVTEST_LAZY_MAC_S = 0, GKR_DEVTEST_LAZY_MAC_V, GKR_DEVTEST_LAZY_MAC_SEL, GKR_DEVTEST_LAZY_MAC_V_HI,
    GKR_DEVTEST_LAZY_MAC2_S, GKR_DEVTEST_LAZY_MAC3_S, GKR_DEVTEST_LAZY_MAC4_S, GKR_DEVTEST_WEIGHTED_SUM_4,
    GKR_DEVTEST_WEIGHTED_SUM_8, GKR_DEVTEST_ACC_SUM
};
enum {
    GKR_DEVTEST_RED_FULL = 0, GKR_DEVTEST_RED_K8, GKR_DEVTEST_RED_PARTIAL32
};
enum {
    GKR_DEVTEST_MF_REDUCE_274 = 0, GKR_DEVTEST_CROSS_REDUCE, GKR_DEVTEST_LAZY_REDUCE, GKR_DEVTEST_LAZY_REDUCE_K8,
    GKR_DEVTEST_LAZY_REDUCE_PARTIAL32, GKR_DEVTEST_LAZY_ADD_HI, GKR_DEVTEST_ACC_ADD_FR9, GKR_DEVTEST_ACC_REDUCE9,
    GKR_DEVTEST_ADD256, GKR_DEVTEST_SUB256, GKR_DEVTEST_COND_SUB_MOD
};
enum {
    GKR_DEVTEST_LANES_MONT_MUL = 0, GKR_DEVTEST_LANES_ADD3, GKR_DEVTEST_LANES_COND_SUB_P, GKR_DEVTEST_LANES_COND_SUB_2P,
    GKR_DEVTEST_LANES_RESOLVE, GKR_DEVTEST_LANES_PERMUTATION, GKR_DEVTEST_LANES_MULTI_HASH1, GKR_DEVTEST_LANES_MULTI_HASH2,
    GKR_DEVTEST_LANES_MULTI_HASH3, GKR_DEVTEST_LANES_GROUP_SUM
};
int  gkr_devtest_field(gkr_ctx *ctx, int op, const gkr_fr *a, const gkr_fr *b, const gkr_fr *r, size_t n, gkr_fr *out);
int  gkr_devtest_lazy(gkr_ctx *ctx, int op, int red, const gkr_fr *a, const gkr_fr *b, size_t rows, size_t len, gkr_fr *out);
int  gkr_devtest_reduce(gkr_ctx *ctx, int op, const uint32_t *limbs, size_t n, uint32_t *out);
int  gkr_devtest_lanes(gkr_ctx *ctx, int op, const gkr_fr *x, const gkr_fr *y, const gkr_fr *z, size_t n, gkr_fr *out);

int  gkr_sumcheck_mle(gkr_ctx *ctx, const gkr_fr *table, int n, gkr_fr *out_coeffs, uint32_t *out_len,
                      gkr_fr *out_r);

int  gkr_sumcheck_mle_batch_device(gkr_ctx *ctx, const void *d_tables, int n, int batch,
                                   gkr_fr *out_coeffs, uint32_t *out_len, gkr_fr *out_r);


int gkr_mle_eval_batch_device(gkr_ctx *ctx, const void *d_tables, int n, int batch, const gkr_fr *points, gkr_fr *out);

int gkr_sumcheck_mle_verify_batch_device(gkr_ctx *ctx, const void *d_tables, int n, int batch, const gkr_fr *claims,
                                         const gkr_fr *coeffs, const uint32_t *len, const gkr_fr *r,
                                         int *accept, uint32_t *failed_round, uint32_t *failed_check, gkr_fr *out_claims);

int gkr_sumcheck_mle_verify(gkr_ctx *ctx, const gkr_fr *table, int n, const gkr_fr *claim, const gkr_fr *coeffs,
                            const uint32_t *len, const gkr_fr *r, int *accept, uint32_t *failed_round, uint32_t *failed_check);

int  gkr_sumcheck_layer(gkr_ctx *ctx, int k_i, int k_next, const uint8_t *gate_type,
                        const uint32_t *left, const uint32_t *right, const gkr_fr *z,
                        const gkr_fr *W, gkr_fr *out_coeffs, uint32_t *out_len, gkr_fr *out_r);

typedef int (*gkr_allreduce_fn)(void *user, gkr_fr *values, size_t count);
int  gkr_sumcheck_layer_sharded(gkr_ctx *ctx, int k_i, int k_next, uint64_t gate_first, uint64_t gate_count,
                                const uint8_t *gate_type, const uint32_t *left, const uint32_t *right, const gkr_fr *z,
                                const gkr_fr *W, gkr_allreduce_fn allreduce, void *user, gkr_fr *out_coeffs,
                                uint32_t *out_len, gkr_fr *out_r);
int  gkr_sumcheck_layer_device(gkr_ctx *ctx, int k_i, int k_next, uint64_t gate_first, uint64_t gate_count,
                               const void *d_gate_type, const void *d_left, const void *d_right, const gkr_fr *z,
                               const gkr_fr *W, gkr_allreduce_fn allreduce, void *user, gkr_fr *out_coeffs,
                               uint32_t *out_len, gkr_fr *out_r);
typedef struct gkr_resident_layer gkr_resident_layer;
int  gkr_resident_layer_create(gkr_ctx *ctx, int k_i, int k_next, uint64_t gate_first, uint64_t gate_count,
                               const uint8_t *gate_type, const uint32_t *left, const uint32_t *right,
                               gkr_resident_layer **out);
int  gkr_resident_layer_sumcheck_wdev(gkr_ctx *ctx, gkr_resident_layer *layer, const gkr_fr *z, const void *d_W,
                                      gkr_fr *out_coeffs, uint32_t *out_len, gkr_fr *out_r);
int  gkr_resident_layer_sumcheck(gkr_ctx *ctx, gkr_resident_layer *layer, const gkr_fr *z, const gkr_fr *W,
                                 gkr_allreduce_fn allreduce, void *user, gkr_fr *out_coeffs, uint32_t *out_len,
                                 gkr_fr *out_r);
void gkr_resident_layer_free(gkr_ctx *ctx, gkr_resident_layer *layer);
typedef int (*gkr_allreduce_dev_fn)(void *user, size_t count, void *hip_stream);
typedef struct {
    gkr_allreduce_dev_fn fn;
    void *user;
    int64_t *d_limbs;
    size_t capacity;
} gkr_exchange_dev;
size_t gkr_exchange_limbs(int k_next);
int  gkr_resident_layer_sumcheck_dev(gkr_ctx *ctx, gkr_resident_layer *layer, const gkr_fr *z, const gkr_fr *W,
                                     const gkr_exchange_dev *exchange, gkr_fr *out_coeffs, uint32_t *out_len,
                                     gkr_fr *out_r);
#define GKR_RCCL_ID_BYTES 128
typedef struct gkr_rccl_exchange gkr_rccl_exchange;
int  gkr_exchange_rccl_unique_id(void *id_out );
int  gkr_exchange_rccl_create(int device_id, const void *unique_id, int rank, int nranks, size_t capacity_limbs,
                              gkr_rccl_exchange **out);
const gkr_exchange_dev *gkr_exchange_rccl_dev(const gkr_rccl_exchange *x);
uint64_t gkr_exchange_rccl_calls(const gkr_rccl_exchange *x);
void gkr_exchange_rccl_destroy(gkr_rccl_exchange *x);
const char *gkr_exchange_rccl_error(void);

size_t gkr_exchange_limbs_mle(int n, int log2_shards, int batch);
int  gkr_sumcheck_mle_sharded_dev(gkr_ctx *ctx, const void *d_shards, int n, int log2_shards, int shard, int batch,
                                  const gkr_exchange_dev *exchange, gkr_fr *out_coeffs, uint32_t *out_len, gkr_fr *out_r,
                                  uint32_t *out_exchanges);
int  gkr_fr_widen(const gkr_fr *values, size_t count, int64_t *limbs);
int  gkr_fr_narrow(const int64_t *limbs, size_t count, gkr_fr *values);

int  gkr_predicate_tables(gkr_ctx *ctx, int k_i, int k_next, const uint8_t *gate_type,
                          const uint32_t *left, const uint32_t *right, const gkr_fr *z,
                          gkr_fr *out_A, gkr_fr *out_M);

int  gkr_layer_eval(gkr_ctx *ctx, size_t gates, const uint8_t *gate_type, const uint32_t *left,
                    const uint32_t *right, const gkr_fr *prev, size_t n_prev, gkr_fr *out);

typedef struct {
    uint32_t depth;
    const uint32_t *k;
    const uint8_t *const *gate_type;
    const uint32_t *const *left;
    const uint32_t *const *right;
} gkr_circuit_desc;

typedef struct {
    gkr_fr *sumcheck_coeffs;
    uint32_t *sumcheck_len;
    gkr_fr *sumcheck_r;
    gkr_fr *q;
    uint32_t *q_len;
    gkr_fr *z;
    gkr_fr *r;
    gkr_fr *d_coeffs;
    gkr_fr *input_coeffs;
} gkr_proof_buf;

typedef struct {
    size_t rounds;
    size_t q_slots;
    size_t z_values;
    size_t d_coeffs;
    size_t input_coeffs;
} gkr_proof_sizes_t;

int  gkr_proof_sizes(const gkr_circuit_desc *circuit, gkr_proof_sizes_t *out);

int  gkr_prove(gkr_ctx *ctx, const gkr_circuit_desc *circuit, const gkr_fr *input_values,
               int require_zero_output, gkr_proof_buf *out);

int  gkr_prove_batch(gkr_ctx *ctx, const gkr_circuit_desc *circuit, const gkr_fr *input_values, int batch,
                     int require_zero_output, gkr_proof_buf *outs);

typedef struct {
    const gkr_circuit_desc *circuit;
    const gkr_fr *input_values;
    int batch;
    int require_zero_output;
    gkr_proof_buf *outs;
    int status;
} gkr_prove_item;
int  gkr_prove_many(gkr_ctx *ctx, gkr_prove_item *items, size_t n_items, int max_concurrent);
// ... 117 lines not shown
```

Measured before the change: 442.4 billion.

## Add deep first pass binding ten sumcheck rounds with one fold

Pass 0 of the plain MLE sumcheck can now cover ten rounds instead of five. A deep reduce publishes fine-grained partial sums, and the host splits those rounds into two five-round halves joined by a contraction step, with an AVX-512 IFMA variant and a scalar fallback. A new deep multifold kernel then binds all ten rounds in one pass over the input, and the deep reduce can go out on a separate publish stream. The aim is to replace two full-table read passes with one over the largest table, at the cost of more host arithmetic, extra pinned buffers and a host-to-device weight copy.

```diff
diff --git a/gkr_amd/_native.py b/gkr_amd/_native.py
--- a/gkr_amd/_native.py
+++ b/gkr_amd/_native.py
@@ -24,7 +24,7 @@
     "gkr_strerror", "gkr_version", "gkr_ctx_create", "gkr_ctx_create_multi", "gkr_ctx_device_count", "gkr_ctx_destroy", "gkr_last_error",
     "gkr_ctx_set_transcript", "gkr_ctx_set_host_threads", "gkr_ctx_set_option", "gkr_ctx_get_option", "gkr_option_count", "gkr_option_name", "gkr_option_doc", "gkr_option_env", "gkr_host_help_while", "gkr_host_accounting", "gkr_host_accounting_read", "gkr_prove_many", "gkr_ctx_device_name", "gkr_ctx_profile", "gkr_ctx_profile_get", "gkr_ctx_profile_samples",
     "gkr_ctx_profile_reset", "gkr_mimc7_multi_hash", "gkr_mimc7_hash", "gkr_mimc7_constant",
-    "gkr_selftest_mul", "gkr_selftest_wide_sum", "gkr_selftest_fold", "gkr_selftest_dot", "gkr_selftest_hash8", "gkr_selftest_host_pass", "gkr_selftest_host_prod_pass", "gkr_selftest_host_tail", "gkr_selftest_pass_schedule", "gkr_selftest_line_restriction", "gkr_selftest_seg_item", "gkr_devtest_field", "gkr_devtest_lazy", "gkr_devtest_reduce", "gkr_devtest_lanes", "gkr_sumcheck_mle", "gkr_sumcheck_mle_batch_device",
+    "gkr_selftest_mul", "gkr_selftest_wide_sum", "gkr_selftest_fold", "gkr_selftest_dot", "gkr_selftest_hash8", "gkr_selftest_host_pass", "gkr_selftest_host_prod_pass", "gkr_selftest_host_deep_pass", "gkr_selftest_host_tail", "gkr_selftest_pass_schedule", "gkr_selftest_line_restriction", "gkr_selftest_seg_item", "gkr_devtest_field", "gkr_devtest_lazy", "gkr_devtest_reduce", "gkr_devtest_lanes", "gkr_sumcheck_mle", "gkr_sumcheck_mle_batch_device",
     "gkr_mle_eval_batch_device", "gkr_sumcheck_mle_verify_batch_device", "gkr_sumcheck_mle_verify",
     "gkr_sumcheck_layer", "gkr_sumcheck_layer_sharded", "gkr_sumcheck_layer_device", "gkr_resident_layer_create", "gkr_resident_layer_sumcheck", "gkr_resident_layer_sumcheck_wdev", "gkr_resident_layer_free", "gkr_exchange_limbs", "gkr_resident_layer_sumcheck_dev", "gkr_exchange_limbs_mle", "gkr_sumcheck_mle_sharded_dev", "gkr_exchange_rccl_unique_id", "gkr_exchange_rccl_create", "gkr_exchange_rccl_dev",
     "gkr_exchange_rccl_calls", "gkr_exchange_rccl_destroy", "gkr_exchange_rccl_error", "gkr_fr_widen", "gkr_fr_narrow", "gkr_predicate_tables", "gkr_layer_eval", "gkr_proof_sizes", "gkr_prove", "gkr_prove_batch",
diff --git a/gkr_amd/csrc/capi_internal.h b/gkr_amd/csrc/capi_internal.h
--- a/gkr_amd/csrc/capi_internal.h
+++ b/gkr_amd/csrc/capi_internal.h
@@ -602,6 +602,8 @@
 
 void host_pass_scalar(const uint64_t* sums, size_t sums_row_words, int count, int J, const uint32_t* final_len, uint64_t (*c0)[16][4],
                       uint64_t (*c1)[16][4], uint64_t (*r)[16][4], uint32_t (*len)[16], uint64_t* weights, size_t w_row_words);
+void host_deep_contract_scalar(const uint64_t* fine, size_t fine_row_words, int count, int d2, const uint64_t* weights, size_t w_row_words,
+                               uint64_t* out, size_t out_row_words);
 struct MleTailArgs {
     int n_total = 0, round_offset = 0;
     const uint32_t* dep_last = nullptr;
diff --git a/gkr_amd/csrc/capi_mle_passes.hip b/gkr_amd/csrc/capi_mle_passes.hip
--- a/gkr_amd/csrc/capi_mle_passes.hip
+++ b/gkr_amd/csrc/capi_mle_passes.hip
@@ -46,6 +46,22 @@
     }
 }
 
+void host_deep_contract_scalar(const uint64_t* fine, size_t fine_row_words, int count, int d2, const uint64_t* weights, size_t w_row_words,
+                               uint64_t* out, size_t out_row_words) {
+    using gkr::h64::F;
+    const size_t nc = (size_t)1 << d2;
+    for (int k = 0; k < count; ++k) {
+        const F* s = reinterpret_cast<const F*>(fine + (size_t)k * fine_row_words);
+        const F* w = reinterpret_cast<const F*>(weights + (size_t)k * w_row_words);
+        F* o = reinterpret_cast<F*>(out + (size_t)k * out_row_words);
+        for (size_t c = 0; c < nc; ++c) {
+            gkr::h64::Wide acc = gkr::h64::wide_zero();
+            for (size_t b = 0; b < (size_t)gkr::kMleMaxSub; ++b) gkr::h64::wide_mac(acc, s[b * nc + c], w[b]);
+            o[c] = gkr::h64::wide_reduce(acc);
+        }
+    }
+}
+
 struct MlePassTables {
     const Fr* input = nullptr;
     size_t in_stride = 0;
@@ -58,6 +74,9 @@
     gkr::MleHostRecSub* rec = nullptr;
     uint32_t* arrivals = nullptr;
     Fr* h_tail = nullptr;
+    Fr* h_fine = nullptr;
+    Fr* h_w2 = nullptr;
+    Fr* d_w2 = nullptr;
 };
 static int mle_pass_tables(gkr_ctx* ctx, const std::string& prefix, const Fr* input, size_t len, size_t work_len, int batch, MlePassTables& T) {
     T.input = input;
@@ -72,6 +91,13 @@
     return GKR_OK;
 }
 
+static int mle_deep_tables(gkr_ctx* ctx, const std::string& prefix, int batch, MlePassTables& T) {
+    HIP_TRY(ctx, ctx->pinned_host((prefix + ".fine").c_str(), sizeof(Fr) * gkr::kMleDeepMaxSub * batch, reinterpret_cast<void**>(&T.h_fine)));
+    HIP_TRY(ctx, ctx->pinned_host((prefix + ".w2").c_str(), sizeof(Fr) * gkr::kMleMaxSub * batch, reinterpret_cast<void**>(&T.h_w2)));
+    WS(ctx, (prefix + ".dw2").c_str(), Fr, (size_t)batch * gkr::kMleMaxSub, T.d_w2);
+    return GKR_OK;
+}
+
 constexpr double kFusedPublishBytes = 64.0 * 1024 * 1024;
 constexpr uint32_t kFusedPublishBlocks = 256;
 constexpr size_t kArrivalCounters = 4096;
@@ -99,28 +125,72 @@
     const char* row = nullptr;
     int plan_event = -1;
     Fr* export_tail = nullptr;
+    hipStream_t publish = nullptr;
+    int publish_event = -1;
 };
 static void queue_sub_reduce(gkr_ctx* ctx, const MlePassTables& T, int b0, int nb, uint32_t nblk, int jout, uint32_t ticket, hipStream_t st) {
     Timed t(ctx, "mle_sub_reduce", 0.0, st, true);
     gkr::launch_mle_sub_reduce(T.partials + (size_t)b0 * gkr::kMaxBlocksPerTable, nblk, (uint32_t)jout, nb, T.rec + b0, ticket, st);
 }
-static void queue_pass0(gkr_ctx* ctx, const MlePassTables& T, int b0, int nb, int jout, uint32_t ticket, hipStream_t st, const MlePassPolicy& P) {
-    const size_t len = T.in_stride;
-    const Fr* src = T.input + (size_t)b0 * len;
+static void queue_sums(gkr_ctx* ctx, const MlePassTables& T, const Fr* src, size_t stride, size_t len, size_t one_block_max, int b0, int nb, int jout,
+                       uint32_t ticket, hipStream_t st, const char* row) {
     const double bytes = (double)nb * len * 32.0;
-    if (len <= gkr::kSmallPassEntries) {
+    if (len <= one_block_max) {
         Timed t(ctx, "mle_pass_small", bytes, st, true);
-        gkr::launch_mle_multifold_small(0, src, len, nullptr, 0, (uint32_t)len, (uint32_t)jout, nb, T.h_w + (size_t)b0 * gkr::kMleMaxSub, T.rec + b0, ticket, st);
+        gkr::launch_mle_multifold_small(0, src, stride, nullptr, 0, (uint32_t)len, (uint32_t)jout, nb, T.h_w + (size_t)b0 * gkr::kMleMaxSub, T.rec + b0, ticket, st);
         return;
     }
     const uint32_t nblk = gkr::mle_pass_blocks((uint32_t)len, (uint32_t)jout, nb);
     gkr::MlePublish pub;
     const bool fused = fused_publish(T, b0, nb, nblk, bytes, ticket, jout, pub);
     {
-        Timed t(ctx, P.row, bytes, st, fused);
-        gkr::launch_mle_sub_sums(src, len, (uint32_t)len, nb, nblk, T.partials + (size_t)b0 * gkr::kMaxBlocksPerTable, st, fused ? &pub : nullptr);
+        Timed t(ctx, row, bytes, st, fused);
+        gkr::launch_mle_sub_sums(src, stride, (uint32_t)len, nb, nblk, T.partials + (size_t)b0 * gkr::kMaxBlocksPerTable, st, fused ? &pub : nullptr);
     }
     if (!fused) queue_sub_reduce(ctx, T, b0, nb, nblk, jout, ticket, st);
+}
+static void queue_pass0(gkr_ctx* ctx, const MlePassTables& T, int b0, int nb, int jout, uint32_t ticket, hipStream_t st, const MlePassPolicy& P) {
+    queue_sums(ctx, T, T.input + (size_t)b0 * T.in_stride, T.in_stride, T.in_stride, gkr::kSmallPassEntries, b0, nb, jout, ticket, st, P.row);
+}
+static void queue_pass0_deep(gkr_ctx* ctx, const MlePassTables& T, int b0, int nb, int depth, uint32_t ticket, hipStream_t st, const MlePassPolicy& P) {
+    const size_t len = T.in_stride;
+    const uint32_t nblk = gkr::mle_pass_blocks((uint32_t)len, (uint32_t)depth, nb);
+    gkr::MleSubPartial* partials = T.partials + (size_t)b0 * gkr::kMaxBlocksPerTable;
+    {
+        Timed t(ctx, P.row, (double)nb * len * 32.0, st);
+        gkr::launch_mle_sub_sums(T.input + (size_t)b0 * len, len, (uint32_t)len, nb, nblk, partials, st, nullptr);
+    }
+    hipStream_t pub = P.publish ? P.publish : st;
+    if (pub != st) {
+        (void)hipEventRecord(ctx->aux_events[P.publish_event], st);
+        (void)hipStreamWaitEvent(pub, ctx->aux_events[P.publish_event], 0);
+    }
+    Timed t(ctx, "mle_sub_reduce", 0.0, pub, true);
+    gkr::launch_mle_deep_reduce(partials, nblk, (uint32_t)depth, nb, T.h_fine + (size_t)b0 * gkr::kMleDeepMaxSub, T.rec + b0, ticket, pub);
+}
+constexpr size_t kDeepSumsOneBlock = 4096;
+static void queue_fold_deep(gkr_ctx* ctx, const MlePassTables& T, int b0, int nb, int n, int depth, int jout, uint32_t ticket, hipStream_t st,
+                            const MlePassPolicy& P) {
+    const size_t out_len = (size_t)1 << (n - depth);
+    Fr* dst = T.work + (size_t)b0 * T.work_len;
+    unsigned char* plan = T.plans + (size_t)b0 * gkr::mle_fold_plan_bytes();
+    const size_t w_off = (size_t)b0 * gkr::kMleMaxSub;
+    hipStream_t side = P.plan_event < 0 ? st : ctx->aux;
+    {
+        Timed t(ctx, "mle_fold_plan", 0.0, side, true);
+        gkr::launch_mle_fold_plan(gkr::kMlePassMaxRounds, T.h_w + w_off, plan, nb, side);
+        (void)hipMemcpyAsync(T.d_w2 + w_off, T.h_w2 + w_off, sizeof(Fr) * gkr::kMleMaxSub * nb, hipMemcpyHostToDevice, side);
+    }
+    if (P.plan_event >= 0) {
+        (void)hipEventRecord(ctx->aux_events[P.plan_event], ctx->aux);
+        (void)hipStreamWaitEvent(st, ctx->aux_events[P.plan_event], 0);
+    }
+    {
+        Timed t(ctx, P.row, (double)nb * ((double)T.in_stride + (double)out_len) * 32.0, st);
+        gkr::launch_mle_multifold_deep(T.input + (size_t)b0 * T.in_stride, T.in_stride, dst, T.work_len, (uint32_t)(n - depth), (uint32_t)depth, nb, plan,
+                                       T.d_w2 + w_off, st);
+    }
+    queue_sums(ctx, T, dst, T.work_len, out_len, kDeepSumsOneBlock, b0, nb, jout, ticket, st, "mle_sub_sums_folded");
 }
 static void queue_fold(gkr_ctx* ctx, const MlePassTables& T, int b0, int nb, bool from_input, int m_src, int jin, int jout, uint32_t ticket,
                        hipStream_t st, const MlePassPolicy& P) {
@@ -167,7 +237,9 @@
     int bound[kMaxGroups + 1];
     uint32_t chunk[kMaxGroups];
     bool tail_on = false;
+    int deep = 0;
 };
+constexpr int kMleDeepMinN = 20, kMleDeepRounds = gkr::kMleDeepMaxRounds;
 static MleSchedule mle_schedule(int n, int batch, int hash_threads, bool is_tail, const gkr::Options& o) {
     MleSchedule sc;
     const double len = (double)((size_t)1 << n);
@@ -182,6 +254,14 @@
         if (batch - sc.n_dev < 16) sc.n_dev = (batch - 16) & ~7;
         if (sc.n_dev < 8) sc.n_dev = 0;
     }
+    const long long deep_opt = o.v[gkr::OPT_mle_deep_rounds];
+    const bool deep_ok = !is_tail && sc.n_dev == 0 && !o.v[gkr::OPT_no_mfma_fold] && sc.jmax == gkr::kMlePassMaxRounds;
+    if (deep_opt > gkr::kMlePassMaxRounds && deep_opt <= gkr::kMleDeepMaxRounds) {
+        if (deep_ok && n >= (int)deep_opt + 6) sc.deep = (int)deep_opt;
+    } else if (deep_opt == 0 && deep_ok && o.v[gkr::OPT_rounds_per_pass] == 0 && n >= kMleDeepMinN && hash_threads >= 4) {
+        sc.deep = kMleDeepRounds;
+    }
+    if (sc.deep) sc.j_first = sc.deep;
     const int host_batch = batch - sc.n_dev;
     const double batch_bytes = (double)host_batch * len * 32.0;
     int want_groups = (int)(batch_bytes / (4.0 * 1024 * 1024 * 1024));
@@ -251,13 +331,19 @@
         G.m -= jin;
         G.round0 += jin;
         G.j = rounds_for(G.m);
+        if (sc.deep && G.round0 == sc.deep && ((size_t)1 << G.m) <= kDeepSumsOneBlock) G.j = G.m < sc.jmax ? G.m : sc.jmax;
         G.ticket = ++ctx->ticket;
     }
     void launch_first(PassGroup& G) {
         G.ticket = ++ctx->ticket;
         MlePassPolicy P;
         P.row = G.chain ? "mle_sub_sums_dev" : "mle_sub_sums";
-        queue_pass0(ctx, T, G.b0, G.nb, G.j, G.ticket, G.chain ? G.chain : s, P);
+        if (sc.deep) {
+            if (chain) P.publish = chain, P.publish_event = sc.groups + G.index;
+            queue_pass0_deep(ctx, T, G.b0, G.nb, sc.deep, G.ticket, s, P);
+        } else {
+            queue_pass0(ctx, T, G.b0, G.nb, G.j, G.ticket, G.chain ? G.chain : s, P);
+        }
     }
     void launch_next_first() {
         if (next_first < sc.groups) launch_first(grp[next_first++]);
@@ -270,9 +356,13 @@
         MlePassPolicy P;
         P.row = G.chain ? "mle_multifold_dev" : (st == s ? "mle_multifold" : "mle_multifold_late");
         if (!gkr::opt(gkr::OPT_plan_main) && st == s && sc.groups != 1) P.plan_event = G.index;
-        G.on_host = sc.tail_on && !G.chain && G.m <= (int)kMleTailLog2 && G.m - G.j > 0;
+        const bool deep_fold = from_input && sc.deep;
+        G.on_host = sc.tail_on && !G.chain && !deep_fold && G.m <= (int)kMleTailLog2 && G.m - G.j > 0;
         if (G.on_host) P.export_tail = T.h_tail + ((size_t)G.b0 << kMleTailLog2);
-        queue_fold(ctx, T, G.b0, G.nb, from_input, m_src, jin, G.j, G.ticket, st, P);
+        if (deep_fold)
+            queue_fold_deep(ctx, T, G.b0, G.nb, n, sc.deep, G.j, G.ticket, st, P);
+        else
+            queue_fold(ctx, T, G.b0, G.nb, from_input, m_src, jin, G.j, G.ticket, st, P);
     }
     void host_fold(PassGroup& G, int jin) {
         using gkr::h64::F;
@@ -298,8 +388,8 @@
     void process_chunk(const PassGroup& G, int b_first, int count) {
         static const bool scalar_book = gkr::process_switch("GKR_HOST_PASS_SCALAR");
         const int J = G.j, n_out = tail ? tail->n_total : n, r_off = tail ? tail->round_offset : 0;
-        uint64_t c0[gkr::kMlePassMaxRounds][16][4], c1[gkr::kMlePassMaxRounds][16][4], r[gkr::kMlePassMaxRounds][16][4];
-        uint32_t ln[gkr::kMlePassMaxRounds][16], final_len[16];
+        uint64_t c0[gkr::kMleDeepMaxRounds][16][4], c1[gkr::kMleDeepMaxRounds][16][4], r[gkr::kMleDeepMaxRounds][16][4];
+        uint32_t ln[gkr::kMleDeepMaxRounds][16], final_len[16];
         const bool final_pass = G.round0 + J == n;
         for (int i = 0; i < count; ++i) {
             if (G.round0 == 0) dep_last[b_first + i] = tail && tail->dep_last ? tail->dep_last[b_first + i] : T.h_rec[b_first + i].dep;
@@ -307,9 +397,21 @@
         }
         static_assert(sizeof(gkr::MleHostRecSub) % 8 == 0, "hand-off records are addressed in 64-bit words");
         const uint64_t* sums = reinterpret_cast<const uint64_t*>(T.h_rec[b_first].sums);
-        uint64_t* weights = G.m - J > 0 ? reinterpret_cast<uint64_t*>(T.h_w + (size_t)b_first * gkr::kMleMaxSub) : nullptr;
-        (host_ifma_ready() && count >= 3 && !scalar_book ? gkr::gkr_ifma_pass : host_pass_scalar)(
-            sums, sizeof(gkr::MleHostRecSub) / 8, count, J, final_pass ? final_len : nullptr, c0, c1, r, ln, weights, 4 * gkr::kMleMaxSub);
+        const bool lanes = host_ifma_ready() && count >= 3 && !scalar_book;
+        const auto pass_fn = lanes ? gkr::gkr_ifma_pass : host_pass_scalar;
+        constexpr size_t w_row = 4 * gkr::kMleMaxSub;
+        if (J > gkr::kMlePassMaxRounds) {
+            const int JA = gkr::kMlePassMaxRounds, JB = J - JA;
+            alignas(64) uint64_t bound[16][w_row];
+            pass_fn(sums, sizeof(gkr::MleHostRecSub) / 8, count, JA, nullptr, c0, c1, r, ln, reinterpret_cast<uint64_t*>(T.h_w + (size_t)b_first * gkr::kMleMaxSub), w_row);
+            (lanes ? gkr::gkr_ifma_deep_contract : host_deep_contract_scalar)(
+                reinterpret_cast<const uint64_t*>(T.h_fine + (size_t)b_first * gkr::kMleDeepMaxSub), 4 * gkr::kMleDeepMaxSub, count, JB,
+                reinterpret_cast<const uint64_t*>(T.h_w + (size_t)b_first * gkr::kMleMaxSub), w_row, &bound[0][0], w_row);
+            pass_fn(&bound[0][0], w_row, count, JB, nullptr, c0 + JA, c1 + JA, r + JA, ln + JA, reinterpret_cast<uint64_t*>(T.h_w2 + (size_t)b_first * gkr::kMleMaxSub), w_row);
+        } else {
+            uint64_t* weights = G.m - J > 0 ? reinterpret_cast<uint64_t*>(T.h_w + (size_t)b_first * gkr::kMleMaxSub) : nullptr;
+            pass_fn(sums, sizeof(gkr::MleHostRecSub) / 8, count, J, final_pass ? final_len : nullptr, c0, c1, r, ln, weights, w_row);
+        }
         for (int i = 0; i < count; ++i)
             for (int t = 0; t < J; ++t)
                 write_round_output(out_coeffs, out_len, out_r, (size_t)(b_first + i) * n_out + r_off + G.round0 + t, c0[t][i], c1[t][i], ln[t][i], r[t][i]);
@@ -404,8 +506,11 @@
     const gkr::Options* o = gkr::current_options();
     const MleSchedule& sc = R.sc = mle_schedule(n, batch, pool->workers() + 1, tail != nullptr, o ? *o : gkr::default_options());
     if (int rc = mle_pass_tables(ctx, "mlep", d_tables, len, len >> sc.j_first, batch, R.T)) return rc;
+    if (sc.deep)
+        if (int rc = mle_deep_tables(ctx, "mlep", batch, R.T)) return rc;
     if (int rc = mle_arrival_counters(ctx, len, R.T)) return rc;
-    HIP_TRY(ctx, ctx->aux_stream(sc.groups));
+    HIP_TRY(ctx, ctx->aux_stream(sc.deep ? 2 * sc.groups : sc.groups));
+    if (sc.deep && sc.groups > 1) HIP_TRY(ctx, ctx->chain_stream(&R.chain));
     if (sc.tail_on) HIP_TRY(ctx, ctx->pinned_host("mlep.tail", sizeof(Fr) * ((size_t)batch << kMleTailLog2), reinterpret_cast<void**>(&R.T.h_tail)));
     if (!gkr::opt(gkr::OPT_no_late_stream) && sc.groups > 1) HIP_TRY(ctx, ctx->late_stream(&R.late));
     R.dep_last = std::vector<uint32_t>(batch, 0);
diff --git a/gkr_amd/csrc/gkr_capi.hip b/gkr_amd/csrc/gkr_capi.hip
--- a/gkr_amd/csrc/gkr_capi.hip
+++ b/gkr_amd/csrc/gkr_capi.hip
@@ -372,6 +372,98 @@
     return GKR_OK;
 }
 
+int gkr_selftest_host_deep_pass(const gkr_fr* fine, int count, int depth, gkr_fr* c0, gkr_fr* c1, uint32_t* len, gkr_fr* r, int* used_ifma) {
+    using gkr::h64::F;
+    constexpr int JA = gkr::kMlePassMaxRounds, DM = gkr::kMleDeepMaxRounds, NS = gkr::kMleDeepMaxSub;
+    if (!fine || !c0 || !c1 || !len || !r || count < 1 || count > kHashChunkMax || depth <= JA || depth > DM) return GKR_ERR_INVALID;
+    if (!all_canonical(fine, (size_t)count * NS)) return GKR_ERR_NON_CANONICAL;
+    const int JB = depth - JA;
+    const size_t nc = (size_t)1 << JB, nfine = (size_t)1 << depth;
+    const F* f = reinterpret_cast<const F*>(fine);
+    const F* cts = host_mimc_constants64();
+    const F one_m = gkr::h64::to_mont(F{{1, 0, 0, 0}});
+    struct Out {
+        uint64_t c0[DM][16][4], c1[DM][16][4], r[DM][16][4];
+        uint32_t len[DM][16];
+        std::vector<F> wa, wb;
+    } d, a, b;
+    std::vector<F> w_direct((size_t)count * nfine);
+    for (int k = 0; k < count; ++k) {
+        std::vector<F> S(f + (size_t)k * NS, f + (size_t)k * NS + nfine), w(nfine);
+        w[0] = one_m;
+        size_t cur = 1;
+        for (int t = 0; t < depth; ++t) {
+            const size_t half = nfine >> (t + 1);
+            F lo = S[0], hi = S[half];
+            for (size_t i = 1; i < half; ++i) {
+                lo = gkr::h64::add(lo, S[i]);
+                hi = gkr::h64::add(hi, S[half + i]);
+            }
+            const F dd = gkr::h64::sub(hi, lo);
+            const uint32_t ln = gkr::h64::is_zero(dd) ? 1u : 2u;
+            const F vec[2] = {dd, lo};
+            const F rc = host_multi_hash(vec + (2 - ln), (int)ln, cts);
+            memcpy(d.c0[t][k], &lo, 32);
+            memcpy(d.c1[t][k], &dd, 32);
+            memcpy(d.r[t][k], &rc, 32);
+            d.len[t][k] = ln;
+            const F rm = gkr::h64::to_mont(rc), nr = gkr::h64::sub(one_m, rm);
+            for (size_t i = 0; i < half; ++i) S[i] = gkr::h64::add(S[i], gkr::h64::mont_mul(gkr::h64::sub(S[half + i], S[i]), rm));
+            for (size_t i = cur; i-- > 0;) {
+                w[2 * i + 1] = gkr::h64::mont_mul(w[i], rm);
+                w[2 * i] = gkr::h64::mont_mul(w[i], nr);
+            }
+            cur <<= 1;
+        }
+        std::copy(w.begin(), w.end(), w_direct.begin() + (size_t)k * nfine);
+    }
+    std::vector<F> coarse((size_t)count * 32), bound((size_t)count * 32);
+    for (int k = 0; k < count; ++k)
+        for (size_t bb = 0; bb < 32; ++bb) {
+            F v = f[(size_t)k * NS + bb * nc];
+            for (size_t c = 1; c < nc; ++c) v = gkr::h64::add(v, f[(size_t)k * NS + bb * nc + c]);
+            coarse[(size_t)k * 32 + bb] = v;
+        }
+    auto staged = [&](Out& o, bool lanes) {
+        o.wa.assign((size_t)count * 32, F{{0, 0, 0, 0}});
+        o.wb.assign((size_t)count * 32, F{{0, 0, 0, 0}});
+        const auto pass_fn = lanes ? gkr::gkr_ifma_pass : host_pass_scalar;
+        pass_fn(&coarse[0].l[0], 4 * 32, count, JA, nullptr, o.c0, o.c1, o.r, o.len, &o.wa[0].l[0], 4 * 32);
+        (lanes ? gkr::gkr_ifma_deep_contract : host_deep_contract_scalar)(reinterpret_cast<const uint64_t*>(fine), 4 * (size_t)NS, count, JB, &o.wa[0].l[0],
+                                                                          4 * 32, &bound[0].l[0], 4 * 32);
+        pass_fn(&bound[0].l[0], 4 * 32, count, JB, nullptr, o.c0 + JA, o.c1 + JA, o.r + JA, o.len + JA, &o.wb[0].l[0], 4 * 32);
+    };
+    auto differs = [&](const Out& x) {
+        for (int t = 0; t < depth; ++t)
+            for (int k = 0; k < count; ++k)
+                if (memcmp(d.c0[t][k], x.c0[t][k], 32) || memcmp(d.c1[t][k], x.c1[t][k], 32) || memcmp(d.r[t][k], x.r[t][k], 32) || d.len[t][k] != x.len[t][k])
+                    return true;
+        for (int k = 0; k < count; ++k)
+            for (size_t bb = 0; bb < 32; ++bb)
+                for (size_t c = 0; c < nc; ++c) {
+                    const F prod = gkr::h64::mont_mul(x.wa[(size_t)k * 32 + bb], x.wb[(size_t)k * 32 + c]);
+                    if (memcmp(&prod, &w_direct[(size_t)k * nfine + bb * nc + c], 32)) return true;
+                }
+        return false;
+    };
+    staged(a, false);
+    if (differs(a)) return GKR_ERR_INVALID;
+    const bool ifma = host_ifma_ready();
+    if (used_ifma) *used_ifma = ifma ? 1 : 0;
+    if (ifma) {
+        staged(b, true);
+        if (differs(b)) return GKR_ERR_INVALID;
+    }
+    for (int t = 0; t < depth; ++t)
+        for (int k = 0; k < count; ++k) {
+            memcpy(&c0[(size_t)t * count + k], d.c0[t][k], 32);
+            memcpy(&c1[(size_t)t * count + k], d.c1[t][k], 32);
+            memcpy(&r[(size_t)t * count + k], d.r[t][k], 32);
+            len[(size_t)t * count + k] = d.len[t][k];
+        }
+    return GKR_OK;
+}
+
 int gkr_selftest_host_prod_pass(const gkr_fr* recs, int count, int J, const uint32_t* vec_len, gkr_fr* c2, gkr_fr* lin, gkr_fr* c0,
                                 gkr_fr* r, gkr_fr* w, int* used_ifma) {
     using gkr::h64::F;
diff --git a/gkr_amd/csrc/kernels.h b/gkr_amd/csrc/kernels.h
--- a/gkr_amd/csrc/kernels.h
+++ b/gkr_amd/csrc/kernels.h
@@ -101,6 +101,13 @@
 void launch_mle_multifold(int jin, const Fr* src, size_t src_stride, Fr* dst, size_t dst_stride, uint32_t S, uint32_t batch,
                           uint32_t nblk, const Fr* weights, const void* plans, MleSubPartial* partials, hipStream_t s,
                           const MlePublish* publish = nullptr);
+constexpr int kMleDeepMaxRounds = 10;
+constexpr int kMleDeepMaxSub = 1 << kMleDeepMaxRounds;
+void launch_mle_deep_reduce(const MleSubPartial* partials, uint32_t nblk, uint32_t depth, uint32_t batch, Fr* fine, MleHostRecSub* host_rec,
+                            uint32_t ticket, hipStream_t s);
+uint32_t mle_multifold_deep_blocks(uint32_t log2_out);
+void launch_mle_multifold_deep(const Fr* src, size_t src_stride, Fr* dst, size_t dst_stride, uint32_t log2_out, uint32_t depth, uint32_t batch,
+                               const void* plans, const Fr* outer, hipStream_t s);
 void launch_mle_pass_hash_lanes(const MleHostRecSub* rec, uint32_t count, uint32_t J, uint32_t round0, uint32_t n_out, bool final_pass,
                                 bool first_pass, const Fr* cts, uint32_t* dep_last, Fr* weights, Fr* out_coeffs, uint32_t* out_len, Fr* out_r,
                                 hipStream_t s);
diff --git a/gkr_amd/csrc/kernels.hip b/gkr_amd/csrc/kernels.hip
--- a/gkr_amd/csrc/kernels.hip
+++ b/gkr_amd/csrc/kernels.hip
@@ -325,6 +325,77 @@
 __global__ void __launch_bounds__(512) k_mle_sub_reduce(const MleSubPartial* __restrict__ partials, uint32_t nblk,
                                                         uint32_t jout, MleHostRecSub* __restrict__ host_rec, uint32_t ticket) {
     mle_total_and_publish(partials + (size_t)blockIdx.x * nblk, nblk, jout, host_rec + blockIdx.x, ticket);
+}
+
+__global__ void __launch_bounds__(1024) k_mle_deep_reduce(const MleSubPartial* __restrict__ partials, uint32_t nblk, uint32_t depth,
+                                                          Fr* __restrict__ fine, MleHostRecSub* __restrict__ host_rec, uint32_t ticket) {
+    __shared__ uint32_t s_pdep;
+    const uint32_t t = threadIdx.x, nfine = 1u << depth, bpf = nblk >> depth, d2 = depth - (uint32_t)kMlePassMaxRounds;
+    const MleSubPartial* p = partials + (size_t)blockIdx.x * nblk;
+    MleHostRecSub* r = host_rec + blockIdx.x;
+    if (t == 0) s_pdep = 0;
+    __syncthreads();
+    Acc<10> tot = acc_zero<10>();
+    uint32_t dep = 0;
+    if (t < nfine) {
+        for (uint32_t i = 0; i < bpf; ++i) {
+            acc_add_acc(tot, p[(size_t)t * bpf + i].sum);
+            dep |= p[(size_t)t * bpf + i].dep;
+        }
+        store_fr(fine + (size_t)blockIdx.x * kMleDeepMaxSub + t, acc_reduce(tot));
+    }
+    if (__any(dep) && (t & 63u) == 0) atomicOr(&s_pdep, 1u);
+    for (uint32_t off = (1u << d2) >> 1; off >= 1u; off >>= 1) {
+        Acc<10> o;
+#pragma unroll
+        for (int l = 0; l < 10; ++l) o.l[l] = __shfl_down(tot.l[l], off, 64);
+        acc_add_acc(tot, o);
+    }
+    if (t < nfine && (t & ((1u << d2) - 1u)) == 0) r->sums[t >> d2] = acc_reduce(tot);
+    __threadfence_system();
+    __syncthreads();
+    if (t == 0) {
+        r->dep = s_pdep;
+        __hip_atomic_store(&r->seq, ticket, __ATOMIC_RELEASE, __HIP_MEMORY_SCOPE_SYSTEM);
+    }
+}
+
+__global__ void __launch_bounds__(256) k_mle_multifold_deep(const Fr* __restrict__ src, size_t src_stride, Fr* __restrict__ dst,
+                                                            size_t dst_stride, uint32_t log2_out, uint32_t d2,
+                                                            const MfmaFoldPlan* __restrict__ plans, const Fr* __restrict__ outer) {
+    __shared__ __attribute__((aligned(16))) unsigned char digits[32 * 32 * (1 << kMfmaMaxJ)];
+    const Fr* s = src + (size_t)blockIdx.y * src_stride;
+    Fr* d = dst + (size_t)blockIdx.y * dst_stride;
+    const Fr* v = outer + (size_t)blockIdx.y * kMleMaxSub;
+    const uint32_t S2 = 1u << log2_out, S = S2 << d2, nmid = 1u << d2;
+    const uint32_t chunk = S2 / gridDim.x, begin = blockIdx.x * chunk;
+    const uint32_t c_first = (blockIdx.x * 5u + blockIdx.y * 3u) & (nmid - 1u), c_last = (c_first + nmid - 1u) & (nmid - 1u);
+    struct Route {
+        uint32_t iters, begin, woff, c_first, nmid, d2, log2_out;
+        bool idle;
+        __device__ __forceinline__ uint32_t at(uint32_t cur) const {
+            return (((cur + c_first) & (nmid - 1u)) << log2_out) + begin + (cur >> d2) * 256u + woff;
+        }
+    };
+    Lazy17 sum = lazy_zero();
+    mfma_multifold_walk<kMfmaMaxJ>(
+        s, S, plans + blockIdx.y, 0u, digits,
+        [&](uint32_t e0, uint32_t h, uint32_t c, const Fr& y) {
+            const uint32_t mid = e0 >> log2_out;
+            lazy_mac_s(sum, y, load_fr(v + mid));
+            if (mid == c_last) {
+                const Fr out = lazy_reduce(sum);
+                mf_v4u* o = reinterpret_cast<mf_v4u*>(d + (e0 & (S2 - 1u)) + 32u * h + c);
+                const mf_v4u y0 = {out.l[0], out.l[1], out.l[2], out.l[3]}, y1 = {out.l[4], out.l[5], out.l[6], out.l[7]};
+                __builtin_nontemporal_store(y0, o);
+                __builtin_nontemporal_store(y1, o + 1);
+                sum = lazy_zero();
+            }
+        },
+        [&](uint32_t wave) {
+            const uint32_t woff = wave * 64u;
+            return Route{((chunk + 255u) / 256u) << d2, begin, woff, c_first, nmid, d2, log2_out, woff >= chunk};
+        });
 }
 
 __global__ void __launch_bounds__(256) k_mle_sums_small(const Fr* __restrict__ src, size_t src_stride, uint32_t S, uint32_t jout,
@@ -2198,6 +2269,19 @@
     hipLaunchKernelGGL(k_mle_sub_reduce, dim3(batch), dim3(512), 0, s, partials, nblk, jout, host_rec, ticket);
 }
 
+void launch_mle_deep_reduce(const MleSubPartial* partials, uint32_t nblk, uint32_t depth, uint32_t batch, Fr* fine, MleHostRecSub* host_rec,
+                            uint32_t ticket, hipStream_t s) {
+    hipLaunchKernelGGL(k_mle_deep_reduce, dim3(batch), dim3(1024), 0, s, partials, nblk, depth, fine, host_rec, ticket);
+}
+
+uint32_t mle_multifold_deep_blocks(uint32_t log2_out) { return log2_out >= 8u ? 1u << (log2_out - 8u) : 1u; }
+
+void launch_mle_multifold_deep(const Fr* src, size_t src_stride, Fr* dst, size_t dst_stride, uint32_t log2_out, uint32_t depth, uint32_t batch,
+                               const void* plans, const Fr* outer, hipStream_t s) {
+    hipLaunchKernelGGL(k_mle_multifold_deep, dim3(mle_multifold_deep_blocks(log2_out), batch), dim3(256), 0, s, src, src_stride, dst, dst_stride,
+                       log2_out, depth - (uint32_t)kMlePassMaxRounds, static_cast<const MfmaFoldPlan*>(plans), outer);
+}
+
 bool mle_multifold_uses_mfma(uint32_t S, uint32_t nblk) {
     const bool off = opt(OPT_no_mfma_fold) != 0;
     return !off && nblk > 0 && S % nblk == 0 && (S / nblk) % 64u == 0;
diff --git a/gkr_amd/csrc/mfma_fold.h b/gkr_amd/csrc/mfma_fold.h
--- a/gkr_amd/csrc/mfma_fold.h
+++ b/gkr_amd/csrc/mfma_fold.h
@@ -126,9 +126,9 @@
     return mf_reduce_274(l);
 }
 
-template <int JIN, class Sink>
-__device__ __forceinline__ void mfma_multifold_stream(const Fr* __restrict__ s, uint32_t S, const MfmaFoldPlan* __restrict__ plan,
-                                                      uint32_t begin, uint32_t end, uint32_t rot, unsigned char* lds, Sink&& sink) {
+template <int JIN, class Sink, class Route>
+__device__ __forceinline__ void mfma_multifold_walk(const Fr* __restrict__ s, uint32_t S, const MfmaFoldPlan* __restrict__ plan, uint32_t rot,
+                                                    unsigned char* lds, Sink&& sink, Route&& route) {
     constexpr int NB = 1 << JIN;
     constexpr int KS = NB < 8 ? NB : 8;
     constexpr int NST = NB / KS;
@@ -178,17 +178,16 @@
     };
     auto store_entry = [&](uint32_t e0, const mf_v16i& a0, const mf_v16i& a1) { sink(e0, h, c, mf_finish(a0, a1)); };
 
-    const uint32_t span = end - begin;
-    const uint32_t iters = (span + 255u) / 256u;
-    const uint32_t woff = wave * 64u;
-    if (woff >= span) return;
+    const auto tiles = route(wave);
+    const uint32_t iters = tiles.iters;
+    if (tiles.idle) return;
     uint32_t cur = rot % iters;
     auto next_pos = [&]() {
         cur = cur + 1u == iters ? 0u : cur + 1u;
-        return begin + cur * 256u + woff;
+        return tiles.at(cur);
     };
     mf_v4u xa[2][KS], xb[2][KS];
-    uint32_t e0 = begin + cur * 256u + woff;
+    uint32_t e0 = tiles.at(cur);
     load_stage(e0, 0, xa);
     if constexpr (NST == 1) {
         for (uint32_t it = 0; it < iters; it += 2u) {
@@ -235,6 +234,22 @@
     }
 }
 
+struct MfmaChunkRoute {
+    uint32_t iters, begin, woff;
+    bool idle;
+    __device__ __forceinline__ uint32_t at(uint32_t cur) const { return begin + cur * 256u + woff; }
+};
+template <int JIN, class Sink>
+__device__ __forceinline__ void mfma_multifold_stream(const Fr* __restrict__ s, uint32_t S, const MfmaFoldPlan* __restrict__ plan,
+                                                      uint32_t begin, uint32_t end, uint32_t rot, unsigned char* lds, Sink&& sink) {
+    mfma_multifold_walk<JIN>(s, S, plan, rot, lds, sink, [&](uint32_t wave) {
+        const uint32_t span = end - begin;
+        const uint32_t iters = (span + 255u) / 256u;
+        const uint32_t woff = wave * 64u;
+        return MfmaChunkRoute{iters, begin, woff, woff >= span};
+    });
+}
+
 template <int JIN>
 __device__ __forceinline__ void mfma_multifold_block(const Fr* __restrict__ s, Fr* __restrict__ d, uint32_t S,
                                                      const MfmaFoldPlan* __restrict__ plan, uint32_t begin, uint32_t end,
diff --git a/gkr_amd/csrc/mimc_ifma.cpp b/gkr_amd/csrc/mimc_ifma.cpp
--- a/gkr_amd/csrc/mimc_ifma.cpp
+++ b/gkr_amd/csrc/mimc_ifma.cpp
@@ -748,6 +748,25 @@
     scatter8(ysum, rec + 64 * 4, rec_off, sub_lanes);
 }
 
+void gkr_ifma_deep_contract(const uint64_t* fine, size_t fine_row_words, int count, int d2, const uint64_t* weights, size_t w_row_words,
+                            uint64_t* out, size_t out_row_words) {
+    using namespace ifma;
+    const V c264 = splat(g_r264_52);
+    const size_t nc = (size_t)1 << d2;
+    for (int g = 0; g < count; g += 8) {
+        const int cnt = count - g < 8 ? count - g : 8;
+        const __m512i off_f = lane_offsets(fine_row_words, cnt), off_w = lane_offsets(w_row_words, cnt), off_o = lane_offsets(out_row_words, cnt);
+        const uint64_t* f = fine + (size_t)g * fine_row_words;
+        V w[32];
+        for (size_t b = 0; b < 32; ++b) w[b] = mont_mul(gather8(weights + (size_t)g * w_row_words + 4 * b, off_w), c264);
+        for (size_t c = 0; c < nc; ++c) {
+            V acc = mont_mul(gather8(f + 4 * c, off_f), w[0]);
+            for (size_t b = 1; b < 32; ++b) acc = add_mod(acc, mont_mul(gather8(f + 4 * (b * nc + c), off_f), w[b]));
+            scatter8(acc, out + (size_t)g * out_row_words + 4 * c, off_o, (__mmask8)((1u << cnt) - 1u));
+        }
+    }
+}
+
 void gkr_ifma_pass(const uint64_t* sums, size_t sums_row_words, int count, int J, const uint32_t* final_len, uint64_t (*c0)[16][4],
                    uint64_t (*c1)[16][4], uint64_t (*r)[16][4], uint32_t (*len)[16], uint64_t* weights, size_t w_row_words) {
     if (count > 8)
diff --git a/gkr_amd/csrc/mimc_ifma.h b/gkr_amd/csrc/mimc_ifma.h
--- a/gkr_amd/csrc/mimc_ifma.h
+++ b/gkr_amd/csrc/mimc_ifma.h
@@ -8,6 +8,8 @@
 void gkr_ifma_multi_hash16(const uint64_t (*vec)[3][4], const uint32_t* len, int slots, uint64_t (*out)[4]);
 void gkr_ifma_pass(const uint64_t* sums, size_t sums_row_words, int count, int J, const uint32_t* final_len, uint64_t (*c0)[16][4],
                    uint64_t (*c1)[16][4], uint64_t (*r)[16][4], uint32_t (*len)[16], uint64_t* weights, size_t w_row_words);
+void gkr_ifma_deep_contract(const uint64_t* fine, size_t fine_row_words, int count, int d2, const uint64_t* weights, size_t w_row_words,
+                            uint64_t* out, size_t out_row_words);
 void gkr_ifma_prod_pass(const uint64_t* recs, size_t rec_row_words, int count, int J, const uint32_t (*vec_len)[16], uint64_t (*c2)[16][4],
                         uint64_t (*lin)[16][4], uint64_t (*c0)[16][4], uint64_t (*r)[16][4], uint64_t* weights, size_t w_row_words);
 void gkr_ifma_tail_pass(uint64_t* tables, size_t stride, uint32_t m, uint32_t jp, const uint64_t* weights, uint32_t J, uint64_t* rec);
diff --git a/gkr_amd/csrc/options.h b/gkr_amd/csrc/options.h
--- a/gkr_amd/csrc/options.h
+++ b/gkr_amd/csrc/options.h
@@ -6,7 +6,8 @@
 
 #define GKR_CONTEXT_OPTIONS(X)                                                                                                       \
                                                                   \
-    X(rounds_per_pass, "rounds_per_pass", "GKR_ROUNDS_PER_PASS", 0, "rounds a pass of the plain sumcheck covers (0: 5; 3 without the MFMA fold)") \
+    X(rounds_per_pass, "rounds_per_pass", "GKR_ROUNDS_PER_PASS", 0, "rounds a pass of the plain sumcheck covers (0: 5; 3 without the MFMA fold; setting it keeps pass 0 out of its deep form)") \
+    X(mle_deep_rounds, "mle_deep_rounds", "GKR_MLE_DEEP_ROUNDS", 0, "rounds pass 0 of the plain sumcheck covers in its deep form, where one fold then binds them all (0: 10 from n = 20 on, with the host transcript, the MFMA fold, rounds_per_pass unset and four hashing threads or more; 5: never, the five-round schedule; 6..10: that depth wherever the fold leaves 64 entries or more)") \
     X(no_mfma_fold, "no_mfma_fold", "GKR_NO_MFMA_FOLD", 0, "fold passes on v_mad_u64_u32 instead of int8 MFMA")                      \
     X(no_fused_reduce, "no_fused_reduce", "GKR_NO_FUSED_REDUCE", 0, "latency-bound passes publish through k_mle_sub_reduce instead of from their last block") \
     X(hash_chunk, "hash_chunk", "GKR_HASH_CHUNK", 0, "8 or 16: sumchecks per host hash call (0: 16 when host threads are scarce)")    \
diff --git a/include/gkr_amd.h b/include/gkr_amd.h
--- a/include/gkr_amd.h
+++ b/include/gkr_amd.h
@@ -72,6 +72,8 @@
 int  gkr_selftest_host_tail(const gkr_fr *tables, int m, int jp, const gkr_fr *weights, int J, gkr_fr *rec, int *used_ifma);
 int  gkr_selftest_host_prod_pass(const gkr_fr *recs, int count, int J, const uint32_t *vec_len, gkr_fr *c2, gkr_fr *lin,
                                  gkr_fr *c0, gkr_fr *r, gkr_fr *w, int *used_ifma);
+int  gkr_selftest_host_deep_pass(const gkr_fr *fine, int count, int depth, gkr_fr *c0, gkr_fr *c1, uint32_t *len, gkr_fr *r,
+                                 int *used_ifma);
 int  gkr_selftest_dot(const gkr_fr *a, const gkr_fr *b, size_t n, gkr_fr *out);
 int  gkr_selftest_pass_schedule(int n, int mfma, uint32_t *rounds, size_t capacity, size_t *passes);
 int  gkr_selftest_line_restriction(int k, const gkr_fr *W, const gkr_fr *b, const gkr_fr *c, gkr_fr *out, uint32_t *out_len);
```

Result: slower. 408.6 billion (-7.6%).
